# autonomousvision/volsurfs

Hardware: AMD Instinct MI355X
Metric: Mrays/s (fwd+bwd) at 800x800, K=5 shells (higher is better)
Workload: dtype f16 (hash features, MLP on MFMA, composite: as the reference), f32 accumulate and I/O

## Files before the change

include/volsurfs_hip.h:

```cpp
#ifndef VOLSURFS_HIP_H
#define VOLSURFS_HIP_H

#include <stdint.h>

#ifdef __cplusplus
extern "C" {
#endif

#define VSA_OK 0
#define VSA_ERR_ARG (-1)
#define VSA_ERR_UNSUPPORTED (-2)

#define VSA_MAX_SHELLS 16

int vsa_version(void);

int vsa_composite_dense_fwd(const float* surfs_rgb, const float* surfs_alpha,
                            const float* rgb_bg, int bg_is_broadcast, float* out_rgb,
                            float* out_rgb_fg, float* out_bg_transmittance, float* out_weights,
                            float* out_surfs_rgb_h, float* out_surfs_alpha_h, int nr_rays,
                            int nr_shells, int carry_f16, void* stream);

int vsa_composite_dense_bwd(const float* surfs_rgb, const float* surfs_alpha,
                            const float* rgb_bg, int bg_is_broadcast, const float* g_rgb,
                            float* g_surfs_rgb, float* g_surfs_alpha, float* g_rgb_bg,
                            int nr_rays, int nr_shells, int carry_f16, void* stream);

int vsa_composite_dense_bwd_l1(const float* surfs_rgb, const float* surfs_alpha,
                               const float* rgb_bg, int bg_is_broadcast, const float* pred_rgb,
                               const float* gt_rgb, float loss_scale, float* g_surfs_rgb,
                               float* g_surfs_alpha, int nr_rays, int nr_shells, int carry_f16,
                               void* stream);

int vsa_composite_dense_fwd_bwd_l1(const float* surfs_rgb, const float* surfs_alpha,
                                   const float* rgb_bg, int bg_is_broadcast, const float* gt_rgb,
                                   float loss_scale, float* out_rgb, float* g_surfs_rgb,
                                   float* g_surfs_alpha, int nr_rays, int nr_shells, int carry_f16,
                                   void* stream);

long long vsa_reduce_scratch_bytes(void);
int vsa_count_hits(const int32_t* hit_slot, long long n, void* scratch, int64_t* out, void* stream);
int vsa_l1_mean(const float* pred, const float* gt, long long n, void* scratch, float* out, void* stream);

typedef struct vsa_bvh vsa_bvh;
int vsa_bvh_build(const float* verts, const int32_t* faces, int nr_verts, int nr_faces,
                  int leaf_size, vsa_bvh** out_bvh);
int vsa_bvh_sizes(const vsa_bvh* bvh, int* nr_nodes, int* nr_tris, int* max_depth);
int vsa_bvh_export(const vsa_bvh* bvh, float* nodes_out, float* tris_out, int node_base,
                   int tri_base);
int vsa_bvh_export_q(const vsa_bvh* bvh, uint32_t* qnodes_out, float* tris_out, int node_base,
                     int tri_base, float* frame_out);
int vsa_bvh_refit(vsa_bvh* bvh, const float* verts, int nr_verts);
int vsa_bvh_destroy(vsa_bvh* bvh);

typedef struct vsa_bvh_dev vsa_bvh_dev;
int vsa_bvh_dev_build(const float* verts, const int32_t* faces, int nr_verts, int nr_faces, int leaf_size,
                      void* stream, vsa_bvh_dev** out_bvh);
int vsa_bvh_dev_sizes(const vsa_bvh_dev* bvh, int* nr_nodes, int* nr_tris, int* max_depth);
int vsa_bvh_dev_export(const vsa_bvh_dev* bvh, float* nodes_out, uint32_t* qnodes_out, float* tris_out,
                       int node_base, int tri_base, float* frame_out, void* stream);
int vsa_bvh_dev_refit(vsa_bvh_dev* bvh, const float* verts, int nr_verts, void* stream);
int vsa_bvh_dev_destroy(vsa_bvh_dev* bvh);
int vsa_bvh_dev_build_ploc(const float* verts, const int32_t* faces, int nr_verts, int nr_faces, int leaf_size,
                           int radius, void* stream, vsa_bvh_dev** out_bvh);

int vsa_trace(const float* nodes, const float* tris, const int32_t* mesh_roots, int nr_meshes,
              int max_depth, const float* rays_o, const float* rays_d, int nr_rays, float t_min,
              float* hit_t, int32_t* hit_slot, float* hit_uv, void* stream);

int vsa_trace_q(const uint32_t* qnodes, const float* tris, const int32_t* mesh_roots,
                const float* mesh_frames, int nr_meshes, int max_depth, const float* rays_o,
                const float* rays_d, int nr_rays, float t_min, float* hit_t, int32_t* hit_slot,
                float* hit_uv, void* stream);
int vsa_trace_q_narrow(const uint32_t* qnodes, const float* tris, const int32_t* mesh_roots,
                       const float* mesh_frames, int nr_meshes, int max_depth, const float* rays_o,
                       const float* rays_d, int nr_rays, float t_min, float* hit_t, int32_t* hit_slot,
                       float* hit_uv, int rays_per_wave, void* stream);
long long vsa_trace_feedback_bytes(int nr_rays, int nr_meshes);
int vsa_trace_q_fb(const uint32_t* qnodes, const float* tris, const int32_t* mesh_roots,
                   const float* mesh_frames, int nr_meshes, int max_depth, const float* rays_o,
                   const float* rays_d, int nr_rays, float t_min, float* hit_t, int32_t* hit_slot,
                   float* hit_uv, void* feedback, long long feedback_bytes, int phase, void* stream);
int vsa_trace_coop_config(int chunk, int lanes, long long max_waves);
int vsa_trace_q_stats(const uint32_t* qnodes, const float* tris, const int32_t* mesh_roots,
                      const float* mesh_frames, int nr_meshes, int max_depth, const float* rays_o,
                      const float* rays_d, int nr_rays, float t_min, uint64_t* stats, void* stream);
int vsa_hit_attributes(const float* tris, const float* rays_o, const float* rays_d,
                       const float* hit_t, const int32_t* hit_slot, const float* hit_uv,
                       int nr_rays, uint8_t* is_hit, int32_t* tri_id, float* positions,
                       float* normals, float* barycentric, void* stream);

#define VSA_NT_MAX_LEVELS 16
#define VSA_NT_MAX_DEG 4
#define VSA_NT_WEIGHTS_PER_TEX 8192
#define VSA_NT_ROW_QUADS(d) ((d) == 0 ? 2 : ((d) == 1 ? 4 : 8))
#define VSA_NT_ALPHA_QUAD(d) ((d) == 0 ? 1 : ((d) == 1 ? 3 : ((d) == 2 ? 4 : 6)))

typedef struct vsa_nt_plan {
  int32_t nr_shells;
  int32_t rgb_degrees;
  int32_t alpha_degrees;
  int32_t inner_solid;
  int32_t with_alpha_decay;
  int32_t n_levels;
  int32_t tex_res[VSA_NT_MAX_DEG];
  float sh_lo[VSA_NT_MAX_DEG];
  float sh_span[VSA_NT_MAX_DEG];
  float level_scale[VSA_NT_MAX_LEVELS];
  int32_t level_res[VSA_NT_MAX_LEVELS];
  int32_t level_size[VSA_NT_MAX_LEVELS];
  int32_t level_offset[VSA_NT_MAX_LEVELS + 1];
  int64_t dom_off[VSA_MAX_SHELLS * VSA_NT_MAX_DEG + 1];
  int64_t slot_capacity;
  int32_t max_rays;
  int32_t anchor;
  int64_t row_base[VSA_MAX_SHELLS * VSA_NT_MAX_DEG + 1];
  void* balance;
  int32_t row_format;
  int32_t grads_zeroed;
  int32_t shared_rgb;
  int32_t shared_alpha;
} vsa_nt_plan;

long long vsa_nt_balance_bytes(void);
int vsa_nt_rebalance(const vsa_nt_plan* plan, void* stream);

int vsa_nt_mark(const vsa_nt_plan* plan, const int32_t* hit_slot, const float* hit_uv,
                const float* face_uvs, int nr_rays, float* tex_uv, uint8_t* marks, void* stream);

int vsa_nt_compact_frame(const vsa_nt_plan* plan, uint8_t* marks, int32_t* slot_of,
                         int32_t* texel_of_slot, float* slot_xy, int32_t* seg_start,
                         int32_t* block_scratch, void* stream);

int vsa_nt_encode_fwd(const vsa_nt_plan* plan, const void* tables_h, const float* slot_xy,
                      const int32_t* seg_start, void* features, void* stream);

int vsa_nt_mlp_fwd(const vsa_nt_plan* plan, const void* weights_h, const void* features,
                   const int32_t* seg_start, uint8_t* texels, void* pre_out, void* stream);

int vsa_nt_encode_mlp_fwd(const vsa_nt_plan* plan, const void* tables_h, const void* weights_h,
                          const float* slot_xy, const int32_t* seg_start, void* features,
                          uint8_t* texels, void* pre_out, void* stream);

int vsa_nt_mlp_bwd(const vsa_nt_plan* plan, const void* weights_h, void* features,
                   const int32_t* seg_start, uint16_t* grad_rows, float* grad_weights,
                   float* dfeat_abs_sum, float weight_grad_scale, void* stream);

int vsa_nt_shade_fwd(const vsa_nt_plan* plan, const int32_t* hit_slot, const float* tex_uv,
                     const float* rays_d, const float* tris, const int32_t* slot_of,
                     const int32_t* seg_start, const uint8_t* texels, int nr_rays,
                     float* surfs_rgb, float* surfs_alpha,
                     float* surfs_normals, float* coeffs_out, float* act_out, void* stream);

int vsa_nt_shade_bwd(const vsa_nt_plan* plan, const int32_t* hit_slot, const float* tex_uv,
                     const float* rays_d, const float* tris, const int32_t* slot_of,
                     const int32_t* seg_start, const uint8_t* texels, int nr_rays,
                     const float* g_surfs_rgb,
                     const float* g_surfs_alpha, float grad_scale, uint16_t* grad_rows,
                     const float* act_in, void* stream);

long long vsa_nt_planes_bytes(const vsa_nt_plan* plan);
int vsa_nt_export_planes(const vsa_nt_plan* plan, const int32_t* slot_of, const int32_t* seg_start,
                         const uint8_t* texels, uint8_t* planes, long long planes_bytes, void* stream);
int vsa_nt_import_planes(const vsa_nt_plan* plan, const uint8_t* planes, long long planes_bytes,
                         const int32_t* slot_of, const int32_t* seg_start, uint8_t* texels, void* stream);

int vsa_nt_encode_bwd(const vsa_nt_plan* plan, const void* dfeatures, const float* dfeat_abs_sum,
                      float grad_scale, const float* slot_xy, const int32_t* seg_start,
                      float* grad_tables, void* stream);

int vsa_nt_encode_bwd_range(const vsa_nt_plan* plan, const void* dfeatures,
                            const float* dfeat_abs_sum, float grad_scale, const float* slot_xy,
                            const int32_t* seg_start, float* grad_tables, int shell_begin,
                            int shell_end, void* stream);

typedef struct vsa_dp_flags vsa_dp_flags;
int vsa_dp_flags_create(int n, vsa_dp_flags** out);
int vsa_dp_flags_destroy(vsa_dp_flags* flags);
int vsa_dp_flags_read(const vsa_dp_flags* flags, uint32_t* host_out);

int vsa_nt_encode_bwd_phased(const vsa_nt_plan* plan, const void* dfeatures,
                             const float* dfeat_abs_sum, float grad_scale, const float* slot_xy,
                             const int32_t* seg_start, float* grad_tables, int n_phases,
                             const int32_t* phase_shell_end, vsa_dp_flags* flags, uint32_t* counters,
                             const uint32_t* epoch, int reserve_cus, void* stream);

int vsa_dp_signal(vsa_dp_flags* flags, int index, uint32_t* epoch, int advance_epoch, void* stream);

int vsa_dp_stream_wait(vsa_dp_flags* flags, int index, uint32_t value, int mode, void* stream);

#define VSA_GRID_MAX_LEVELS 32
typedef struct vsa_grid_plan {
  int32_t n_dims;
  int32_t n_levels;
  int32_t n_features;
  int32_t reserved0;
  float level_scale[VSA_GRID_MAX_LEVELS];
  int32_t level_res[VSA_GRID_MAX_LEVELS];
  int32_t level_size[VSA_GRID_MAX_LEVELS];
  int32_t level_offset[VSA_GRID_MAX_LEVELS + 1];
} vsa_grid_plan;

int vsa_grid_encode_fwd(const vsa_grid_plan* plan, const float* tables, const float* x,
                        int nr_points, float* out, void* stream);
int vsa_grid_encode_bwd(const vsa_grid_plan* plan, const float* x, const float* g_out,
                        int nr_points, float* grad_tables, void* stream);
int vsa_grid_encode_bwd_sliced(const vsa_grid_plan* plan, const float* x, const float* g_out,
                               int nr_points, float* grad_tables, float* workspace, void* stream);
int vsa_grid_encode_bwd_binned_workspace(const vsa_grid_plan* plan, int nr_points,
                                         long long* workspace_floats);
int vsa_grid_encode_bwd_binned(const vsa_grid_plan* plan, const float* x, const float* g_out,
                               int nr_points, float* grad_tables, float* workspace, void* stream);
int vsa_grid_encode_fwd_ld(const vsa_grid_plan* plan, const float* tables, const float* x,
                           int nr_points, float* out, int out_stride, int append_x, void* stream);
int vsa_grid_encode_bwd_ld(const vsa_grid_plan* plan, const float* x, const float* g_out,
                           int g_stride, int nr_points, float* grad_tables, void* stream);
int vsa_grid_encode_bwd_sliced_ld(const vsa_grid_plan* plan, const float* x, const float* g_out,
                                  int g_stride, int nr_points, float* grad_tables, float* workspace,
                                  void* stream);
int vsa_grid_encode_bwd_binned_ld(const vsa_grid_plan* plan, const float* x, const float* g_out,
                                  int g_stride, int nr_points, float* grad_tables, float* workspace,
                                  void* stream);
int vsa_sh_encode(const float* dirs, int nr_dirs, int degree, float* out, void* stream);

int vsa_field_head_fwd(const float* y1, int y1_stride, const float* dirs_enc, long long nr_points, int nr_feat,
                       int nr_dir, float* x2, float* density, void* stream);
int vsa_field_head_bwd(const float* y1, int y1_stride, const float* dx2, const float* d_density, long long nr_points,
                       int nr_feat, int nr_dir, float* dy1, void* stream);

#define VSA_MLP_MAX_LAYERS 6
typedef struct vsa_mlp_plan {
  int32_t n_layers;
  int32_t dims[VSA_MLP_MAX_LAYERS + 1];
  const float* w[VSA_MLP_MAX_LAYERS];
  const float* b[VSA_MLP_MAX_LAYERS];
} vsa_mlp_plan;
typedef struct vsa_mlp_grads {
  float* dw[VSA_MLP_MAX_LAYERS];
  float* db[VSA_MLP_MAX_LAYERS];
  int32_t accumulate;
} vsa_mlp_grads;

int vsa_mlp_workspace(const vsa_mlp_plan* plan, long long nr_points, long long* packed_floats,
                      long long* act_floats, long long* partial_floats);
int vsa_mlp_bwd_needs_act(const vsa_mlp_plan* plan, int x_stride, int dx_stride);
int vsa_mlp_fwd(const vsa_mlp_plan* plan, const float* x, int x_stride, int nr_points, float* y,
                int y_stride, float* z_ws, float* a_ws, float* packed_ws, void* stream);
int vsa_mlp_bwd(const vsa_mlp_plan* plan, const float* x, int x_stride, int nr_points,
                const float* dy, int dy_stride, const float* z_ws, float* dz_ws, const float* a_ws,
                float* packed_ws, float* partial_ws, float* dx, int dx_stride,
                const vsa_mlp_grads* grads, void* stream);

int vsa_mlp_fwd_grouped(const vsa_mlp_plan* plans, int nr_groups, const int* nr_points,
                        const float* x, int x_stride, float* y, int y_stride, float* z_ws,
                        float* a_ws, float* packed_ws, float* packed_bwd_ws, void* stream);
int vsa_mlp_bwd_grouped(const vsa_mlp_plan* plans, int nr_groups, const int* nr_points,
                        const float* x, int x_stride, const float* dy, int dy_stride,
                        const float* z_ws, float* dz_ws, const float* a_ws, float* packed_ws,
                        int packed_ready, float* partial_ws, float* dx, int dx_stride,
                        const vsa_mlp_grads* grads, void* stream);

typedef struct vsa_adam_tensor {
  float* param;
  float* grad;
  float* exp_avg;
  float* exp_avg_sq;
  void* param_f16;
  int64_t n;
} vsa_adam_tensor;

int vsa_adam_chunk_elems(void);
int vsa_adam_step(const vsa_adam_tensor* tensors_dev, const int32_t* chunks_dev, int nr_chunks,
                  float lr, float beta1, float beta2, float eps, int step, float grad_scale,
                  int zero_grads, void* stream);
int vsa_adam_step_shared(const vsa_adam_tensor* tensors_dev, const int32_t* chunks_dev, int nr_chunks,
                         float lr, float beta1, float beta2, float eps, int step, float grad_scale,
                         int zero_grads, int max_workgroups, void* stream);

int vsa_legacy_hit_prep(const float* rays_o, const float* rays_d, const float* hit_t, const int32_t* hit_slot,
                        const float* tris, const int64_t* hit_shell, const int64_t* hit_ray, int nr_hits, int nr_rays,
                        float* pts, float* dirs, float* normals, void* stream);
int vsa_legacy_shade_out_fwd(const float* y_rgb, int ld_rgb, const float* y_alpha, int ld_alpha, int alpha_first_row,
                             const int64_t* hit_shell, const int64_t* hit_ray, const float* dirs, const float* normals,
                             int nr_hits, int nr_rays,
                             int nr_shells, int with_alpha_decay, float* surfs_rgb, float* surfs_alpha,
                             float* surfs_normals, float* sig_rgb, float* sig_alpha, float* decay, void* stream);
int vsa_legacy_shade_out_bwd(const float* g_surfs_rgb, const float* g_surfs_alpha, const int64_t* hit_shell,
                             const int64_t* hit_ray, const float* sig_rgb, const float* sig_alpha, const float* decay, int nr_hits, int nr_shells,
                             int alpha_first_row, float* dy_rgb, int ld_rgb, float* dy_alpha, int ld_alpha, void* stream);

typedef struct vsa_permuto_plan {
  int32_t pos_dim;
  int32_t n_levels;
  int32_t n_features;
  int32_t capacity;
  float scale_factor[VSA_GRID_MAX_LEVELS][4];
  float random_shift[VSA_GRID_MAX_LEVELS][4];
} vsa_permuto_plan;

int vsa_permuto_encode_fwd(const vsa_permuto_plan* plan, const float* lattice_values,
                           const float* x, const float* window, int nr_points, float* out,
                           int out_stride, void* stream);
int vsa_permuto_encode_bwd(const vsa_permuto_plan* plan, const float* x, const float* window,
                           const float* g_out, int g_stride, int nr_points, float* grad_values,
                           void* stream);

int vsa_permuto_encode_fwd_grouped(const vsa_permuto_plan* plan_host, const vsa_permuto_plan* plans_dev,
                                   const float* const* lattice_values, int nr_groups,
                                   const int* nr_points, const float* x, const float* window,
                                   float* out, int out_stride, void* stream);
int vsa_permuto_encode_bwd_grouped(const vsa_permuto_plan* plan_host, const vsa_permuto_plan* plans_dev,
                                   int nr_groups, const int* nr_points, const float* x,
                                   const float* window, const float* g_out, int g_stride,
                                   float* const* grad_values, void* stream);

int vsa_packed_cumprod_fwd(const int32_t* start_end, const float* one_minus_alpha,
                           float* transmittance, float* bg_transmittance, int nr_rays,
                           void* stream);
int vsa_packed_cumprod_bwd(const int32_t* start_end, const float* g_bg_transmittance,
                           const float* one_minus_alpha, const float* bg_transmittance,
                           const float* cumsum_lv, float* g_one_minus_alpha, int nr_rays,
                           void* stream);
int vsa_packed_cumsum(const int32_t* start_end, const float* values, int inverse, float* out,
                      int nr_rays, void* stream);
int vsa_packed_integrate_fwd(const int32_t* start_end, const float* values, const float* weights,
                             float* out, int nr_rays, int dim, void* stream);
int vsa_packed_integrate_bwd(const int32_t* start_end, const float* g_out, const float* values,
                             const float* weights, float* g_values, float* g_weights,
                             int nr_rays, int dim, int bug_compat, void* stream);
int vsa_packed_composite_fwd(const int32_t* start_end, const float* density, const float* dt,
                             const float* rgb, float* pred_rgb, float* weights, int nr_rays,
                             void* stream);
int vsa_packed_composite_bwd(const int32_t* start_end, const float* density, const float* dt,
                             const float* rgb, const float* g_pred_rgb, float* g_rgb,
                             float* g_density, float* scratch, int nr_rays, int bug_compat,
                             void* stream);
int vsa_nerf_composite_fwd(const int32_t* start_end, const float* density, const float* dt,
                           const float* samples_z, const float* rgb, const float* rgb_bg, int bg_per_ray,
                           float* rgb_fg, float* rgb_out, float* weights_sum, float* depth, float* weights,
                           int nr_rays, void* stream);
int vsa_nerf_composite_bwd(const int32_t* start_end, const float* density, const float* dt,
                           const float* rgb, const float* rgb_bg, int bg_per_ray, const float* weights_sum,
                           const float* g_rgb, const float* g_weights_sum, float* g_density,
                           float* g_rgb_samples, float* g_rgb_bg, float* scratch, int nr_rays,
                           int bug_compat, void* stream);
int vsa_nerf_coarse_cdf(const int32_t* start_end, const float* density, const float* dt, float* cdf,
                        int nr_rays, void* stream);
int vsa_neus_composite_fwd(const int32_t* start_end, const float* sdf, const float* sdf_grad,
                           const float* dirs, const float* dt, const float* samples_z,
                           const float* normals, const float* rgb, const float* rgb_bg, int bg_per_ray,
                           double cos_anneal_ratio, double logistic_beta, float* rgb_fg, float* rgb_out,
                           float* weights_sum, float* depth, float* normals_out, float* weights,
                           float* alpha, int nr_rays, void* stream);
int vsa_neus_composite_bwd(const int32_t* start_end, const float* sdf, const float* sdf_grad,
                           const float* dirs, const float* dt, const float* rgb, const float* rgb_bg,
                           int bg_per_ray, double cos_anneal_ratio, double logistic_beta,
                           const float* weights_sum, const float* g_rgb, const float* g_weights_sum,
                           float* g_sdf, float* g_sdf_grad, float* g_rgb_samples, float* g_rgb_bg,
                           float* scratch, int nr_rays, int bug_compat, void* stream);
int vsa_sdf_coarse_cdf(const int32_t* start_end, const float* sdf, const float* dt, float logistic_beta,
                       float* cdf, int nr_rays, void* stream);
int vsa_offsets_composite_fwd(const int32_t* start_end, int nr_surfs, const float* sdfs, const float* sdfs_grad,
                              const float* normals, const float* rgb, const float* transparency, const float* dirs,
                              const float* dt, const float* samples_z, const float* rgb_bg, int bg_per_ray,
                              double cos_anneal_ratio, double logistic_beta, int with_alpha_decay,
                              double alpha_decay_factor, float* surfs_rgb, float* surfs_normals, float* surfs_depths,
                              float* surfs_weight_sum, float* surfs_alpha, float* surfs_transmittance,
                              float* surfs_blending_weights, float* rgb_fg, float* bg_transmittance, float* rgb_out,
                              float* alpha, int nr_rays, void* stream);
int vsa_offsets_composite_bwd(const int32_t* start_end, int nr_surfs, const float* sdfs, const float* sdfs_grad,
                              const float* normals, const float* rgb, const float* transparency, const float* dirs,
                              const float* dt, const float* rgb_bg, int bg_per_ray, double cos_anneal_ratio,
                              double logistic_beta, int with_alpha_decay, double alpha_decay_factor,
                              const float* surfs_rgb, const float* surfs_alpha, const float* surfs_transmittance,
                              const float* bg_transmittance, const float* g_rgb, float* g_sdfs, float* g_sdfs_grad,
                              float* g_rgb_samples, float* g_transparency, float* g_rgb_bg, float* scratch,
                              int nr_rays, int bug_compat, void* stream);
int vsa_sdfs_coarse_cdf(const int32_t* start_end, int nr_surfs, const float* sdfs, const float* dt,
                        float logistic_beta, float* cdf, int nr_rays, void* stream);
int vsa_packed_median_depth(const int32_t* start_end, const float* samples_z,
                            const float* weights, float threshold, float* out, int nr_rays,
                            int fallback_compat, void* stream);
int vsa_packed_update_dt(const int32_t* start_end, const float* ray_max_dt, const float* ray_exit,
                         const float* samples_z, int is_background, float* samples_dt,
                         int nr_rays, void* stream);
int vsa_sample_bg(const float* rays_o, const float* rays_d, const float* ray_t_start,
                  float ray_t_far, int nr_samples_per_ray, int jitter, uint64_t rng_state,
                  uint64_t rng_inc, float* ray_max_dt, float* samples_3d, float* samples_dirs,
                  float* samples_z, int32_t* ray_start_end_idx, int nr_rays, void* stream);
int vsa_contract_samples(const float* ray_o, const int32_t* start_end, const float* samples_3d,
                         const float* samples_z, float* out_samples_3d, float* out_samples_z,
                         int nr_rays, void* stream);

int vsa_packed_sum_over_rays(const int32_t* start_end, const float* values, float* sum_per_ray,
                             float* sum_per_sample, int nr_rays, int dim, void* stream);
int vsa_packed_sum_over_rays_bwd(const int32_t* start_end, const float* g_sum_per_ray,
                                 const float* g_sum_per_sample, float* g_values, int nr_rays,
                                 int dim, void* stream);
int vsa_packed_sdf2alpha(const int32_t* start_end, const float* samples_dt, const float* samples_sdf,
                         const float* logistic_beta, float* alpha, int nr_rays, void* stream);
int vsa_packed_compute_cdf(const int32_t* start_end, const float* weights, float* cdf, int nr_rays,
                           void* stream);

int vsa_sample_fg(const float* rays_o, const float* rays_d, const float* ray_t_entry,
                  const float* ray_t_exit, float min_dist_between_samples,
                  int min_nr_samples_per_ray, int max_nr_samples_per_ray, int jitter,
                  uint64_t rng_state, uint64_t rng_inc, float* ray_max_dt, int32_t* samples_idx,
                  float* samples_3d, float* samples_dirs, float* samples_z,
                  int32_t* ray_start_end_idx, int nr_rays, void* stream);
int vsa_pack_compact(const int32_t* start_end, const int32_t* out_start, const int32_t* samples_idx,
                     const float* samples_3d, const float* samples_dirs, const float* samples_z,
                     const float* samples_dt, const float* samples_values, int values_dim,
                     int32_t* out_idx, float* out_3d, float* out_dirs, float* out_z, float* out_dt,
                     float* out_values, int32_t* out_start_end, int nr_rays, void* stream);
int vsa_importance_sample(const float* rays_o, const float* rays_d, const int32_t* start_end,
                          const float* samples_z, const float* samples_cdf,
                          int nr_importance_samples, int jitter, uint64_t rng_state,
                          uint64_t rng_inc, float* out_3d, float* out_dirs, float* out_z,
                          int32_t* out_start_end, int nr_rays, void* stream);

int vsa_uncontract_samples(const float* ray_o, const int32_t* start_end, const float* samples_3d,
                           const float* samples_z, float* out_samples_3d, float* out_samples_z,
                           int nr_rays, void* stream);

int vsa_combine_packs(const int32_t* start_end_1, const int32_t* idx_1, const float* s3d_1,
                      const float* dirs_1, const float* z_1, const float* values_1,
                      const int32_t* start_end_2, const int32_t* idx_2, const float* s3d_2,
                      const float* dirs_2, const float* z_2, const float* values_2,
                      const int32_t* out_start, float min_dist_between_samples, int values_dim,
                      int32_t* out_idx, float* out_3d, float* out_dirs, float* out_z,
                      float* out_values, int32_t* out_start_end, int nr_rays, void* stream);

int vsa_intersect_primitive(const float* rays_o, const float* rays_d, int nr_rays, int kind,
                            float size, uint8_t* is_hit, float* t_near, float* t_far,
                            float* points_near, float* points_far, void* stream);

int vsa_camera_rays(const float* c2w, const float* intrinsics_inv, int height, int width,
                    int nr_rays_per_pixel, int jitter_pixels, uint64_t rng_state, uint64_t rng_inc,
                    float* rays_o, float* rays_d, float* points_2d, void* stream);

int vsa_reel_next_rays_batch(const float* c2w_all, const float* intrinsics_inv_all,
                             const float* rgb_all, const float* mask_all, int nr_cameras, int height,
                             int width, int batch_size, int nr_rays_per_pixel, int jitter_pixels,
                             uint64_t rng_state, uint64_t rng_inc, int32_t* camera_idx,
                             float* rays_o, float* rays_d, float* gt_rgb, float* gt_mask,
                             float* points_2d, void* stream);

typedef struct vsa_train_ctl {
  int32_t iter;
  int32_t nr_rays;
  int32_t capacity;
  int32_t adam_step;
  float loss_scale;
  float adam_lr;
  float loss;
  int32_t clamped;
  uint64_t rng_state, rng_inc;
  int64_t nr_hits;
  int32_t target_hits;
  int32_t nr_warmup;
  int32_t nr_milestones;
  int32_t milestone[8];
  float lr_stage[9];
  int32_t adam_pending;
  double lr_base;
  double loss_weight;
  int64_t sum_rays, sum_hits;
} vsa_train_ctl;

int vsa_train_ctl_tick(vsa_train_ctl* ctl, void* stream);

int vsa_reel_next_rays_batch_ctl(const float* c2w_all, const float* intrinsics_inv_all, const float* rgb_all,
                                 const float* mask_all, int nr_cameras, int height, int width, int capacity,
                                 int nr_rays_per_pixel, int jitter_pixels, const vsa_train_ctl* ctl,
                                 const float* dummy_o, const float* dummy_d, const float* dummy_rgb,
                                 int32_t* camera_idx, float* rays_o, float* rays_d, float* gt_rgb,
                                 float* gt_mask, float* points_2d, void* stream);

int vsa_composite_dense_fwd_bwd_l1_ctl(const float* surfs_rgb, const float* surfs_alpha, const float* rgb_bg,
                                       int bg_is_broadcast, const float* gt_rgb, const vsa_train_ctl* ctl,
                                       float* out_rgb, float* g_surfs_rgb, float* g_surfs_alpha, int capacity,
                                       int nr_shells, int carry_f16, void* stream);

int vsa_l1_mean_ctl(const float* pred, const float* gt, int capacity, void* scratch, vsa_train_ctl* ctl, void* stream);

int vsa_adam_step_ctl(const vsa_adam_tensor* tensors_dev, const int32_t* chunks_dev, int nr_chunks, float beta1,
                      float beta2, float eps, float grad_scale, int zero_grads, int max_workgroups,
                      const vsa_train_ctl* ctl, void* stream);

int vsa_tile_order(const float* src, float* dst, int height, int width, int channels, int inverse,
                   void* stream);
int vsa_tile_order_rays(const float* rays_o, const float* rays_d, const float* gt_rgb,
                        float* rays_o_tiled, float* rays_d_tiled, float* gt_rgb_tiled, int height,
                        int width, void* stream);


int vsa_occ_grid_points(const int32_t* point_indices, int nr_points, int nr_voxels_per_dim,
                        float extent_x, float extent_y, float extent_z, int centre_of_voxel, int jitter,
                        uint64_t rng_state, uint64_t rng_inc, float* out_points, void* stream);
int vsa_occ_update_values(const int32_t* point_indices, const float* values, int nr_points, float decay,
                          float* grid_values, void* stream);
int vsa_occ_update_occupancy_density(const int32_t* point_indices, int nr_points, int nr_voxels_per_dim,
                                     float extent_x, float extent_y, float extent_z,
                                     float occupancy_thresh, int check_neighbours,
                                     const float* grid_values, uint8_t* grid_occupancy, void* stream);
int vsa_occ_update_occupancy_sdf(const int32_t* point_indices, const float* logistic_beta, int nr_points,
                                 int nr_voxels_per_dim, float extent_x, float extent_y, float extent_z,
                                 float occupancy_thresh, const float* grid_values,
                                 uint8_t* grid_occupancy, void* stream);
int vsa_occ_check(const float* points, int nr_points, int nr_voxels_per_dim, float extent_x,
                  float extent_y, float extent_z, const float* grid_values,
                  const uint8_t* grid_occupancy, const uint8_t* grid_roi, uint8_t* out_occupancy,
                  float* out_values, void* stream);
int vsa_occ_rays_t_near_t_far(const float* rays_o, const float* rays_d, const float* ray_t_entry,
                              const float* ray_t_exit, int nr_rays, int nr_voxels_per_dim,
                              float extent_x, float extent_y, float extent_z,
                              const uint8_t* grid_occupancy, const uint8_t* grid_roi, float* out_t_near,
                              float* out_t_far, void* stream);
int vsa_occ_first_sample(const float* rays_o, const float* rays_d, const float* ray_t_entry,
                         const float* ray_t_exit, int nr_rays, int nr_voxels_per_dim, float extent_x,
                         float extent_y, float extent_z, const uint8_t* grid_occupancy,
                         const uint8_t* grid_roi, float* samples_3d, float* samples_dirs,
                         float* samples_z, float* samples_dt, int32_t* ray_start_end_idx, void* stream);
int vsa_occ_advance_samples(const float* samples_dirs, const float* samples_3d, int nr_points,
                            int nr_voxels_per_dim, float extent_x, float extent_y, float extent_z,
                            const uint8_t* grid_occupancy, const uint8_t* grid_roi,
                            float* new_samples_3d, uint8_t* is_within_bounds, void* stream);
int vsa_sample_fg_occupied(const float* rays_o, const float* rays_d, const float* ray_t_entry,
                           const float* ray_t_exit, float min_dist_between_samples,
                           int min_nr_samples_per_ray, int max_nr_samples_per_ray, int jitter_samples,
                           uint64_t rng_state, uint64_t rng_inc, int nr_voxels_per_dim, float extent_x,
                           float extent_y, float extent_z, const uint8_t* grid_occupancy,
                           const uint8_t* grid_roi, float* ray_max_dt, int32_t* samples_idx,
                           float* samples_3d, float* samples_dirs, float* samples_z,
                           int32_t* ray_start_end_idx, int nr_rays, void* stream);

long long vsa_image_metrics_workspace_bytes(int B, int H, int W, int pool, int pred_u8, int gt_u8);
int vsa_image_metrics(const void* pred, int pred_u8, const void* gt, int gt_u8, int B, int H, int W, int pool,
                      int quantize_pred, void* workspace, long long workspace_bytes, double* psnr_out,
                      double* ssim_out, void* stream);

long long vsa_isosurface_workspace_bytes(long long nx, long long ny, long long nz, int nr_levels);
int vsa_isosurface_count(const float* grid, long long nx, long long ny, long long nz, const float* levels,
                         int nr_levels, int inside_above, void* workspace, long long workspace_bytes,
                         long long* totals, void* stream);
int vsa_isosurface_emit(const float* grid, long long nx, long long ny, long long nz, const float* levels,
                        int nr_levels, int inside_above, const float* origin, const float* spacing, void* workspace,
                        long long workspace_bytes, const long long* totals, float* const* verts,
                        int32_t* const* faces, void* stream);
int vsa_mc_table(int8_t* out);

long long vsa_simplify_workspace_bytes(long long nr_verts, long long nr_faces);
int vsa_simplify(const float* verts, long long nr_verts, const int32_t* faces, long long nr_faces,
                 long long target_faces, void* workspace, long long workspace_bytes, float* out_verts,
                 int32_t* out_faces, long long* stats, float* stage_ms, void* stream);

#define VSA_ERR_ATLAS_FULL (-3)
long long vsa_atlas_workspace_bytes(long long nr_verts, long long nr_faces, int resolution);
int vsa_atlas(const float* verts, long long nr_verts, const int32_t* faces, long long nr_faces, int resolution,
              int padding, void* workspace, long long workspace_bytes, float* out_faces_uvs, int32_t* out_chart,
              long long* stats, float* scale, float* stage_ms, void* stream);
long long vsa_atlas_rasterize_workspace_bytes(long long nr_faces);
int vsa_atlas_rasterize(const float* faces_uvs, long long nr_faces, int resolution, void* workspace,
                        long long workspace_bytes, int32_t* out_face_id, int32_t* out_count, void* stream);

int vsa_st_begin(const float* points_near, int nr_rays, int nr_slots, float* pts, uint8_t* flags, int32_t* live,
                 float* dense, int32_t* count, void* stream);
int vsa_st_step(const int32_t* live_in, const int32_t* count_in, const float* sdf, int nr_columns,
                const int32_t* slot_cols, int nr_rays, const float* rays_d, float sdf_multiplier, float thresh,
                int kind, float size, float* pts, uint8_t* flags, uint8_t* keep, int32_t* block_counts,
                const float* dense_in, int32_t* live_out, float* dense_out, int32_t* count_out, int bound,
                void* stream);
int vsa_st_finish(const float* pts, const float* rays_o, int nr_rays, int nr_slots, const uint8_t* flags,
                  int unconverged_are_hits, float* z, uint8_t* hit, uint8_t* keep, int32_t* block_counts,
                  int32_t* hit_list, int32_t* hit_count, void* stream);
int vsa_st_scatter(const int32_t* ids, long long nr_ids, const float* src, int nr_channels, int nr_rays,
                   int nr_slots, float* dst, void* stream);
int vsa_st_blend(const float* surfs_rgb, const float* surfs_alpha, int nr_rays, int nr_surfs,
                 float* surfs_transmittance, float* surfs_blending_weights, float* rgb_fg, float* bg_transmittance,
                 void* stream);

long long vsa_tb_workspace_bytes(long long nr_faces, int resolution);
long long vsa_tb_max_chunks(int resolution, int nr_samples, long long chunk_rows);
int vsa_tb_samples(const float* faces_uvs, long long nr_faces, int resolution, int nr_samples,
                   unsigned long long seed, long long chunk_rows, void* workspace, long long workspace_bytes,
                   int32_t* owner, int32_t* ctl, int ctl_len, void* stream);
int vsa_tb_emit(const float* verts, const int32_t* faces, const float* faces_uvs, long long nr_faces, int resolution,
                int nr_samples, unsigned long long seed, const void* workspace, long long workspace_bytes,
                const int32_t* owner, int32_t* row_start, float* points, float* normals, void* stream);
int vsa_tb_resolve(const float* vals, int nr_channels, const int32_t* row_start, int texel_begin, int texel_end,
                   int resolution, float* texture, void* stream);
int vsa_tb_dilate(float* img, int height, int width, int nr_channels, int nr_iterations, int32_t* stamp,
                  int32_t* filled, void* stream);

int vsa_tsdf_fuse_lattice(const float* proj, const float* depth, int nr_views, int height, int width,
                          const float* axis, int n, float sdf_trunc, int uncontract, float* out_tsdf, void* stream);
int vsa_tsdf_fuse_points(const float* proj, const float* depth, const float* rgb_maps, int nr_views, int height,
                         int width, const float* points, long long nr_points, float sdf_trunc, int uncontract,
                         float* out_tsdf, float* out_rgb, void* stream);
int vsa_tsdf_uncontract_points(const float* points, long long nr_points, float max_range, float* out, void* stream);

long long vsa_mesh_clusters_workspace_bytes(long long nr_verts, long long nr_faces);
int vsa_mesh_clusters(const float* verts, long long nr_verts, const int32_t* faces, long long nr_faces,
                      void* workspace, long long workspace_bytes, int32_t* out_triangle_clusters,
                      int32_t* out_cluster_n_triangles, double* out_cluster_area, long long* out_nr_clusters,
                      float* stage_ms, void* stream);
int vsa_mesh_filter(const float* verts, long long nr_verts, const int32_t* faces, long long nr_faces, int mode,
                    const uint8_t* keep_mask, long long cluster_to_keep, long long min_cluster_faces,
                    int drop_unreferenced, int drop_degenerate, void* workspace, long long workspace_bytes,
                    float* out_verts, int32_t* out_faces, int32_t* out_vertex_map, int32_t* out_face_map,
                    long long* stats, float* stage_ms, void* stream);
int vsa_mesh_compact_rows(const void* rows, long long nr_rows, int row_words, const int32_t* map, void* out,
                          void* stream);

int vsa_face_view_counts(const uint32_t* qnodes, const float* tris, const int32_t* mesh_roots,
                         const float* mesh_frames, int nr_meshes, int max_depth,
                         const float* c2w_all, const float* intrinsics_inv_all,
                         int nr_views, int height, int width, int supersample, float t_min,
                         const long long* face_base, uint32_t* counts,
                         void* stream);
int vsa_face_view_counts_tile(int tile);
int vsa_face_ring_dilate(const int32_t* faces, long long nr_faces, long long nr_verts, uint8_t* keep,
                         int rings, uint8_t* vert_scratch, void* stream);

#ifdef __cplusplus
}
#endif
#endif
```

volsurfs_amd/composite.py:

```python
import torch

from . import _lib


class _CompositeDense(torch.autograd.Function):
    @staticmethod
    def forward(ctx, surfs_rgb, surfs_alpha, rgb_bg, carry_f16):
        N, K, _ = surfs_rgb.shape
        surfs_rgb = _lib.check_f32(surfs_rgb.contiguous(), N, K, 3)
        surfs_alpha = _lib.check_f32(surfs_alpha.contiguous().view(N, K), N, K)
        rgb_bg = rgb_bg.contiguous()
        bcast = rgb_bg.shape[0] == 1 and N != 1
        _lib.check_f32(rgb_bg, 1 if bcast else N, 3)
        dev = surfs_rgb.device
        out_rgb = torch.empty(N, 3, device=dev)
        out_fg = torch.empty(N, 3, device=dev)
        out_bgT = torch.empty(N, 1, device=dev)
        out_w = torch.empty(N, K, 1, device=dev)
        out_rgb_h = torch.empty(N, K, 3, device=dev)
        out_alpha_h = torch.empty(N, K, 1, device=dev)
        _lib.call("vsa_composite_dense_fwd", surfs_rgb, surfs_alpha, rgb_bg, bcast, out_rgb,
                  out_fg, out_bgT, out_w, out_rgb_h, out_alpha_h, N, K, int(carry_f16),
                  _lib.stream_ptr())
        ctx.save_for_backward(surfs_rgb, surfs_alpha, rgb_bg)
        ctx.bcast = bcast
        ctx.carry_f16 = int(carry_f16)
        ctx.mark_non_differentiable(out_fg, out_bgT, out_w, out_rgb_h, out_alpha_h)
        return out_rgb, out_fg, out_bgT, out_w, out_rgb_h, out_alpha_h

    @staticmethod
    def backward(ctx, g_rgb, *unused):
        surfs_rgb, surfs_alpha, rgb_bg = ctx.saved_tensors
        N, K, _ = surfs_rgb.shape
        g_rgb = _lib.check_f32(g_rgb.contiguous(), N, 3)
        g_c = torch.empty_like(surfs_rgb)
        g_a = torch.empty_like(surfs_alpha)
        need_bg = ctx.needs_input_grad[2]
        g_bg = torch.empty(N, 3, device=g_rgb.device) if need_bg else None
        _lib.call("vsa_composite_dense_bwd", surfs_rgb, surfs_alpha, rgb_bg, ctx.bcast, g_rgb,
                  g_c, g_a, g_bg, N, K, ctx.carry_f16, _lib.stream_ptr())
        if need_bg and ctx.bcast:
            g_bg = g_bg.sum(0, keepdim=True)
        return g_c, g_a, g_bg, None


def composite_dense(surfs_rgb, surfs_alpha, rgb_bg, carry_f16=False):
    N, K = surfs_rgb.shape[:2]
    alpha2d = surfs_alpha.reshape(N, K)
    rgb, fg, bgT, w, rgb_h, alpha_h = _CompositeDense.apply(surfs_rgb, alpha2d, rgb_bg, carry_f16)
    return {
        "rgb": rgb,
        "rgb_fg": fg,
        "rgb_bg": rgb_bg.expand(N, 3).half().float(),
        "surfs_alpha": alpha_h,
        "surfs_rgb": rgb_h,
        "surfs_blending_weights": w,
        "bg_transmittance": bgT,
    }


class _CompositeL1(torch.autograd.Function):

    @staticmethod
    def forward(ctx, surfs_rgb, surfs_alpha, rgb_bg, gt_rgb):
        N, K = surfs_rgb.shape[:2]
        rgb, g_c, g_a = composite_fwd_bwd_l1_raw(surfs_rgb.contiguous(), surfs_alpha.reshape(N, K).contiguous(),
                                                 rgb_bg.contiguous(), gt_rgb.contiguous(), 1.0 / (3.0 * N))
        ctx.save_for_backward(g_c, g_a)
        ctx.alpha_shape = surfs_alpha.shape
        loss = l1_mean(rgb, gt_rgb)
        ctx.mark_non_differentiable(rgb)
        return loss, rgb

    @staticmethod
    def backward(ctx, g_loss, _g_rgb):
        g_c, g_a = ctx.saved_tensors
        return g_c * g_loss, (g_a * g_loss).reshape(ctx.alpha_shape), None, None


def composite_l1(surfs_rgb, surfs_alpha, rgb_bg, gt_rgb):
    return _CompositeL1.apply(surfs_rgb, surfs_alpha, rgb_bg, gt_rgb)


def composite_fwd_raw(surfs_rgb, surfs_alpha, rgb_bg, carry_f16=False):
    N, K, _ = surfs_rgb.shape
    out = torch.empty(N, 3, device=surfs_rgb.device)
    bcast = rgb_bg.shape[0] == 1 and N != 1
    _lib.call("vsa_composite_dense_fwd", surfs_rgb, surfs_alpha, rgb_bg, bcast, out, None, None,
              None, None, None, N, K, int(carry_f16), _lib.stream_ptr())
    return out


def composite_bwd_raw(surfs_rgb, surfs_alpha, rgb_bg, g_rgb, carry_f16=False):
    N, K, _ = surfs_rgb.shape
    g_c = torch.empty_like(surfs_rgb)
    g_a = torch.empty_like(surfs_alpha)
    bcast = rgb_bg.shape[0] == 1 and N != 1
    _lib.call("vsa_composite_dense_bwd", surfs_rgb, surfs_alpha, rgb_bg, bcast, g_rgb, g_c, g_a,
              None, N, K, int(carry_f16), _lib.stream_ptr())
    return g_c, g_a


def composite_bwd_l1_raw(surfs_rgb, surfs_alpha, rgb_bg, pred_rgb, gt_rgb, loss_scale, carry_f16=False):
    N, K, _ = surfs_rgb.shape
    g_c = torch.empty_like(surfs_rgb)
    g_a = torch.empty_like(surfs_alpha)
    bcast = rgb_bg.shape[0] == 1 and N != 1
    _lib.call("vsa_composite_dense_bwd_l1", surfs_rgb, surfs_alpha, rgb_bg, bcast, pred_rgb, gt_rgb,
              float(loss_scale), g_c, g_a, N, K, int(carry_f16), _lib.stream_ptr())
    return g_c, g_a


def composite_fwd_bwd_l1_raw(surfs_rgb, surfs_alpha, rgb_bg, gt_rgb, loss_scale, carry_f16=False):
    N, K, _ = surfs_rgb.shape
    rgb = torch.empty(N, 3, device=surfs_rgb.device)
    g_c = torch.empty_like(surfs_rgb)
    g_a = torch.empty_like(surfs_alpha)
    bcast = rgb_bg.shape[0] == 1 and N != 1
    _lib.call("vsa_composite_dense_fwd_bwd_l1", surfs_rgb, surfs_alpha, rgb_bg, bcast, gt_rgb,
              float(loss_scale), rgb, g_c, g_a, N, K, int(carry_f16), _lib.stream_ptr())
    return rgb, g_c, g_a


_reduce_scratch = {}


def reduce_scratch(device):
    import ctypes
    dev = torch.device(device)
    dev = torch.device("cuda", torch.cuda.current_device()) if dev.index is None else dev
    key = (dev, torch.cuda.current_stream(dev).cuda_stream)
    sc = _reduce_scratch.get(key)
    if sc is None:
        fn = _lib.lib().vsa_reduce_scratch_bytes
        fn.restype = ctypes.c_longlong
        sc = _reduce_scratch[key] = torch.zeros(int(fn()), dtype=torch.uint8, device=dev)
    return sc


def l1_mean(pred, gt):
    import ctypes
    pred, gt = _lib.check_f32(pred.contiguous()), _lib.check_f32(gt.contiguous(), *pred.shape)
    pred, gt = (x if x.data_ptr() % 16 == 0 else x.clone() for x in (pred, gt))
    out = torch.empty((), device=pred.device)
    _lib.call("vsa_l1_mean", pred, gt, ctypes.c_longlong(pred.numel()), reduce_scratch(pred.device), out,
              _lib.stream_ptr())
    return out


def count_hits(hit_slot):
    import ctypes
    if hit_slot.dtype != torch.int32 or not hit_slot.is_contiguous() or not hit_slot.is_cuda:
        raise _lib.VolsurfsHipError("count_hits: contiguous CUDA int32 tensor expected")
    out = torch.empty((), dtype=torch.int64, device=hit_slot.device)
    _lib.call("vsa_count_hits", hit_slot, ctypes.c_longlong(hit_slot.numel()), reduce_scratch(hit_slot.device), out,
              _lib.stream_ptr())
    return out
```

volsurfs_amd/csrc/composite_dense.hip:

```cpp
#include "common.h"

namespace {

#ifndef VSA_COMP_TILE
#define VSA_COMP_TILE 256
#endif
constexpr int TILE = VSA_COMP_TILE;

template <int K>
struct Lds {
  static constexpr int SC = (3 * K) | 1;
  static constexpr int SA = K | 1;
};

template <int W, int S>
__device__ __forceinline__ void slab_load(const float* __restrict__ g, float* __restrict__ s,
                                          int rows_valid) {
  const int total = rows_valid * W;
  const int nvec = total >> 2;
  const float4* g4 = reinterpret_cast<const float4*>(g);
  if constexpr (W == S) {
    if (rows_valid == TILE && (TILE * W) % 4 == 0) {
      typedef __attribute__((address_space(3))) void* lds_vp;
      typedef __attribute__((address_space(1))) const void* glb_vp;
      const int wave = __builtin_amdgcn_readfirstlane(threadIdx.x >> 6), lane = threadIdx.x & 63;
      constexpr int NV = TILE * W / 4, NC = (NV + 63) / 64;
      for (int c = wave; c < NC; c += TILE / 64)
        if (c * 64 + lane < NV)
          __builtin_amdgcn_global_load_lds((glb_vp)(g4 + c * 64 + lane), (lds_vp)(s + c * 256), 16, 0, 0);
      return;
    }
    float4* s4 = reinterpret_cast<float4*>(s);
    for (int v = threadIdx.x; v < nvec; v += TILE) s4[v] = g4[v];
  } else {
    for (int v = threadIdx.x; v < nvec; v += TILE) {
      float4 x = g4[v];
      int e = v << 2;
      float xs[4] = {x.x, x.y, x.z, x.w};
#pragma unroll
      for (int i = 0; i < 4; ++i) {
        int r = (e + i) / W;
        int j = (e + i) - r * W;
        s[r * S + j] = xs[i];
      }
    }
  }
  for (int e = (nvec << 2) + threadIdx.x; e < total; e += TILE) {
    int r = e / W;
    s[r * S + (e - r * W)] = g[e];
  }
}
__device__ __forceinline__ void slab_load_fence() {
  asm volatile("s_waitcnt vmcnt(0)" ::: "memory");
}

template <int W, int S>
__device__ __forceinline__ void slab_store(float* __restrict__ g, const float* __restrict__ s,
                                           int rows_valid) {
  const int total = rows_valid * W;
  const int nvec = total >> 2;
  float4* g4 = reinterpret_cast<float4*>(g);
  if constexpr (W == S) {
    const float4* s4 = reinterpret_cast<const float4*>(s);
    for (int v = threadIdx.x; v < nvec; v += TILE) g4[v] = s4[v];
  } else {
    for (int v = threadIdx.x; v < nvec; v += TILE) {
      int e = v << 2;
      float xs[4];
#pragma unroll
      for (int i = 0; i < 4; ++i) {
        int r = (e + i) / W;
        int j = (e + i) - r * W;
        xs[i] = s[r * S + j];
      }
      g4[v] = make_float4(xs[0], xs[1], xs[2], xs[3]);
    }
  }
  for (int e = (nvec << 2) + threadIdx.x; e < total; e += TILE) {
    int r = e / W;
    g[e] = s[r * S + (e - r * W)];
  }
}

template <int K, bool CARRY_F16>
struct RayFwd {
  float a[K], c[K][3], T[K], w[K], om[K];
  float bgT, fg[3];
  __device__ __forceinline__ void run(const float* sc, const float* sa) {
#pragma unroll
    for (int k = 0; k < K; ++k) {
      a[k] = vsa_round_f16(sa[k]);
#pragma unroll
      for (int ch = 0; ch < 3; ++ch) c[k][ch] = vsa_round_f16(sc[3 * k + ch]);
      om[k] = vsa_round_f16(1.0f - a[k]);
    }
    float acc = 1.0f, Tp = 1.0f;
    fg[0] = fg[1] = fg[2] = 0.f;
#pragma unroll
    for (int k = K - 1; k >= 0; --k) {
      T[k] = Tp;
      if (CARRY_F16) {
        Tp = vsa_round_f16(Tp * om[k]);
      } else {
        acc = vsa_pin_f32(acc * om[k]);
        Tp = vsa_round_f16(acc);
      }
      w[k] = vsa_round_f16(T[k] * a[k]);
#pragma unroll
      for (int ch = 0; ch < 3; ++ch) fg[ch] += vsa_round_f16(c[k][ch] * w[k]);
    }
    bgT = Tp;
#pragma unroll
    for (int ch = 0; ch < 3; ++ch) fg[ch] = vsa_round_f16(vsa_pin_f32(fg[ch]));
  }
};

template <int K, bool CARRY_F16>
__global__ __launch_bounds__(TILE) void composite_dense_fwd_kernel(
    const float* __restrict__ surfs_rgb, const float* __restrict__ surfs_alpha,
    const float* __restrict__ rgb_bg, int bg_bcast, float* __restrict__ out_rgb,
    float* __restrict__ out_rgb_fg, float* __restrict__ out_bgT, float* __restrict__ out_w,
    float* __restrict__ out_rgb_h, float* __restrict__ out_alpha_h, int N) {
  using L = Lds<K>;
  __shared__ __attribute__((aligned(16))) float s_c[TILE * L::SC];
  __shared__ __attribute__((aligned(16))) float s_a[TILE * L::SA];
  __shared__ __attribute__((aligned(16))) float s_o[TILE * 3];
  const long long ray0 = (long long)blockIdx.x * TILE;
  const int rows = min(TILE, (int)(N - ray0));
  slab_load<3 * K, L::SC>(surfs_rgb + ray0 * 3 * K, s_c, rows);
  slab_load<K, L::SA>(surfs_alpha + ray0 * K, s_a, rows);
  if (!bg_bcast) slab_load<3, 3>(rgb_bg + ray0 * 3, s_o, rows);
  slab_load_fence();
  __syncthreads();
  const int r = threadIdx.x;
  if (r < rows) {
    RayFwd<K, CARRY_F16> f;
    f.run(s_c + r * L::SC, s_a + r * L::SA);
    float bg[3];
#pragma unroll
    for (int ch = 0; ch < 3; ++ch)
      bg[ch] = vsa_round_f16(bg_bcast ? rgb_bg[ch] : s_o[r * 3 + ch]);
#pragma unroll
    for (int ch = 0; ch < 3; ++ch)
      s_o[r * 3 + ch] = vsa_round_f16(f.fg[ch] + vsa_round_f16(f.bgT * bg[ch]));
    const long long n = ray0 + r;
    if (out_rgb_fg) {
#pragma unroll
      for (int ch = 0; ch < 3; ++ch) out_rgb_fg[n * 3 + ch] = f.fg[ch];
    }
    if (out_bgT) out_bgT[n] = f.bgT;
    if (out_w) {
#pragma unroll
      for (int k = 0; k < K; ++k) out_w[n * K + k] = f.w[k];
    }
    if (out_alpha_h) {
#pragma unroll
      for (int k = 0; k < K; ++k) out_alpha_h[n * K + k] = f.a[k];
    }
    if (out_rgb_h) {
#pragma unroll
      for (int k = 0; k < K; ++k)
#pragma unroll
        for (int ch = 0; ch < 3; ++ch) out_rgb_h[(n * K + k) * 3 + ch] = f.c[k][ch];
    }
  }
  __syncthreads();
  slab_store<3, 3>(out_rgb + ray0 * 3, s_o, rows);
}

template <int K, bool CARRY_F16>
__global__ __launch_bounds__(TILE) void composite_dense_bwd_kernel(
    const float* __restrict__ surfs_rgb, const float* __restrict__ surfs_alpha,
    const float* __restrict__ rgb_bg, int bg_bcast, const float* __restrict__ g_rgb,
    float* __restrict__ g_surfs_rgb, float* __restrict__ g_surfs_alpha,
    float* __restrict__ g_rgb_bg, int N, const float* __restrict__ l1_gt, float l1_scale,
    float* __restrict__ pred_out, const vsa_train_ctl* __restrict__ ctl) {
  using L = Lds<K>;
  int n_active = N;
  if (ctl) {
    l1_scale = ctl->loss_scale;
    n_active = ctl->nr_rays;
  }
  __shared__ __attribute__((aligned(16))) float s_c[TILE * L::SC];
  __shared__ __attribute__((aligned(16))) float s_a[TILE * L::SA];
  __shared__ __attribute__((aligned(16))) float s_g[TILE * 3];
  __shared__ __attribute__((aligned(16))) float s_b[TILE * 3];
  __shared__ __attribute__((aligned(16))) float s_t[TILE * 3];
  const long long ray0 = (long long)blockIdx.x * TILE;
  const int rows = min(TILE, (int)(N - ray0));
  slab_load<3 * K, L::SC>(surfs_rgb + ray0 * 3 * K, s_c, rows);
  slab_load<K, L::SA>(surfs_alpha + ray0 * K, s_a, rows);
  if (!pred_out) slab_load<3, 3>(g_rgb + ray0 * 3, s_g, rows);
  if (!bg_bcast) slab_load<3, 3>(rgb_bg + ray0 * 3, s_b, rows);
  if (l1_gt) slab_load<3, 3>(l1_gt + ray0 * 3, s_t, rows);
  slab_load_fence();
  __syncthreads();
  const int r = threadIdx.x;
  if (r < rows) {
    RayFwd<K, CARRY_F16> f;
    float* sc = s_c + r * L::SC;
    float* sa = s_a + r * L::SA;
    f.run(sc, sa);
    float g[3], bg[3];
#pragma unroll
    for (int ch = 0; ch < 3; ++ch) {
      bg[ch] = vsa_round_f16(bg_bcast ? rgb_bg[ch] : s_b[r * 3 + ch]);
      if (pred_out) {
        g[ch] = vsa_round_f16(f.fg[ch] + vsa_round_f16(f.bgT * bg[ch]));
        s_g[r * 3 + ch] = g[ch];
      } else {
        g[ch] = s_g[r * 3 + ch];
      }
      if (l1_gt) {
        const float d = g[ch] - s_t[r * 3 + ch];
        g[ch] = ray0 + r >= n_active ? 0.f : (d > 0.f ? l1_scale : (d < 0.f ? -l1_scale : 0.f));
      }
    }
    float S = g[0] * bg[0] + g[1] * bg[1] + g[2] * bg[2];
#pragma unroll
    for (int k = 0; k < K; ++k) {
      float rk = g[0] * f.c[k][0] + g[1] * f.c[k][1] + g[2] * f.c[k][2];
      sa[k] = f.T[k] * (rk - S);
      S = f.a[k] * rk + f.om[k] * S;
#pragma unroll
      for (int ch = 0; ch < 3; ++ch) sc[3 * k + ch] = g[ch] * f.w[k];
    }
    if (g_rgb_bg) {
#pragma unroll
      for (int ch = 0; ch < 3; ++ch) s_b[r * 3 + ch] = g[ch] * f.bgT;
    }
  }
  __syncthreads();
  slab_store<3 * K, L::SC>(g_surfs_rgb + ray0 * 3 * K, s_c, rows);
  slab_store<K, L::SA>(g_surfs_alpha + ray0 * K, s_a, rows);
  if (g_rgb_bg) slab_store<3, 3>(g_rgb_bg + ray0 * 3, s_b, rows);
  if (pred_out) slab_store<3, 3>(pred_out + ray0 * 3, s_g, rows);
}

}

#define VSA_K_DISPATCH(K_, BODY)              \
  switch (K_) {                               \
    case 1: { constexpr int KK = 1; BODY; } break;   \
    case 2: { constexpr int KK = 2; BODY; } break;   \
    case 3: { constexpr int KK = 3; BODY; } break;   \
    case 4: { constexpr int KK = 4; BODY; } break;   \
    case 5: { constexpr int KK = 5; BODY; } break;   \
    case 6: { constexpr int KK = 6; BODY; } break;   \
    case 7: { constexpr int KK = 7; BODY; } break;   \
    case 8: { constexpr int KK = 8; BODY; } break;   \
    case 9: { constexpr int KK = 9; BODY; } break;   \
    default: return VSA_ERR_UNSUPPORTED;      \
  }

extern "C" int vsa_composite_dense_fwd(const float* surfs_rgb, const float* surfs_alpha,
                                       const float* rgb_bg, int bg_is_broadcast, float* out_rgb,
                                       float* out_rgb_fg, float* out_bg_transmittance,
                                       float* out_weights, float* out_surfs_rgb_h,
                                       float* out_surfs_alpha_h, int nr_rays, int nr_shells,
                                       int carry_f16, void* stream) {
  if (nr_rays < 0 || !out_rgb) return VSA_ERR_ARG;
  if (nr_rays == 0) return VSA_OK;
  if (!surfs_rgb || !surfs_alpha || !rgb_bg) return VSA_ERR_ARG;
  dim3 grid(vsa_div_up(nr_rays, TILE)), block(TILE);
  hipStream_t st = (hipStream_t)stream;
  VSA_K_DISPATCH(nr_shells, {
    if (carry_f16)
      hipLaunchKernelGGL((composite_dense_fwd_kernel<KK, true>), grid, block, 0, st, surfs_rgb,
                         surfs_alpha, rgb_bg, bg_is_broadcast, out_rgb, out_rgb_fg,
                         out_bg_transmittance, out_weights, out_surfs_rgb_h, out_surfs_alpha_h,
                         nr_rays);
    else
      hipLaunchKernelGGL((composite_dense_fwd_kernel<KK, false>), grid, block, 0, st, surfs_rgb,
                         surfs_alpha, rgb_bg, bg_is_broadcast, out_rgb, out_rgb_fg,
                         out_bg_transmittance, out_weights, out_surfs_rgb_h, out_surfs_alpha_h,
                         nr_rays);
  });
  VSA_RETURN_LAUNCH_STATUS();
}

static int composite_bwd_launch(const float* surfs_rgb, const float* surfs_alpha,
                                const float* rgb_bg, int bg_is_broadcast, const float* g_rgb,
                                float* g_surfs_rgb, float* g_surfs_alpha, float* g_rgb_bg,
                                int nr_rays, int nr_shells, int carry_f16, const float* l1_gt,
                                float l1_scale, void* stream, float* pred_out = nullptr,
                                const vsa_train_ctl* ctl = nullptr) {
  if (nr_rays < 0) return VSA_ERR_ARG;
  if (nr_rays == 0) return VSA_OK;
  if (!surfs_rgb || !surfs_alpha || !rgb_bg || (!g_rgb && !pred_out) || !g_surfs_rgb || !g_surfs_alpha)
    return VSA_ERR_ARG;
  dim3 grid(vsa_div_up(nr_rays, TILE)), block(TILE);
  hipStream_t st = (hipStream_t)stream;
  VSA_K_DISPATCH(nr_shells, {
    if (carry_f16)
      hipLaunchKernelGGL((composite_dense_bwd_kernel<KK, true>), grid, block, 0, st, surfs_rgb,
                         surfs_alpha, rgb_bg, bg_is_broadcast, g_rgb, g_surfs_rgb, g_surfs_alpha,
                         g_rgb_bg, nr_rays, l1_gt, l1_scale, pred_out, ctl);
    else
      hipLaunchKernelGGL((composite_dense_bwd_kernel<KK, false>), grid, block, 0, st, surfs_rgb,
                         surfs_alpha, rgb_bg, bg_is_broadcast, g_rgb, g_surfs_rgb, g_surfs_alpha,
                         g_rgb_bg, nr_rays, l1_gt, l1_scale, pred_out, ctl);
  });
  VSA_RETURN_LAUNCH_STATUS();
}

extern "C" int vsa_composite_dense_bwd(const float* surfs_rgb, const float* surfs_alpha,
                                       const float* rgb_bg, int bg_is_broadcast,
                                       const float* g_rgb, float* g_surfs_rgb,
                                       float* g_surfs_alpha, float* g_rgb_bg, int nr_rays,
                                       int nr_shells, int carry_f16, void* stream) {
  return composite_bwd_launch(surfs_rgb, surfs_alpha, rgb_bg, bg_is_broadcast, g_rgb, g_surfs_rgb,
                              g_surfs_alpha, g_rgb_bg, nr_rays, nr_shells, carry_f16, nullptr, 0.f,
                              stream);
}

extern "C" int vsa_composite_dense_bwd_l1(const float* surfs_rgb, const float* surfs_alpha,
                                          const float* rgb_bg, int bg_is_broadcast,
                                          const float* pred_rgb, const float* gt_rgb,
                                          float loss_scale, float* g_surfs_rgb,
                                          float* g_surfs_alpha, int nr_rays, int nr_shells,
                                          int carry_f16, void* stream) {
  if (!gt_rgb) return VSA_ERR_ARG;
  return composite_bwd_launch(surfs_rgb, surfs_alpha, rgb_bg, bg_is_broadcast, pred_rgb,
                              g_surfs_rgb, g_surfs_alpha, nullptr, nr_rays, nr_shells, carry_f16,
                              gt_rgb, loss_scale, stream);
}

extern "C" int vsa_composite_dense_fwd_bwd_l1(const float* surfs_rgb, const float* surfs_alpha,
                                              const float* rgb_bg, int bg_is_broadcast,
                                              const float* gt_rgb, float loss_scale, float* out_rgb,
                                              float* g_surfs_rgb, float* g_surfs_alpha, int nr_rays,
                                              int nr_shells, int carry_f16, void* stream) {
  if (!gt_rgb || (nr_rays > 0 && !out_rgb)) return VSA_ERR_ARG;
  return composite_bwd_launch(surfs_rgb, surfs_alpha, rgb_bg, bg_is_broadcast, nullptr, g_surfs_rgb,
                              g_surfs_alpha, nullptr, nr_rays, nr_shells, carry_f16, gt_rgb,
                              loss_scale, stream, out_rgb);
}

extern "C" int vsa_composite_dense_fwd_bwd_l1_ctl(const float* surfs_rgb, const float* surfs_alpha,
                                                  const float* rgb_bg, int bg_is_broadcast, const float* gt_rgb,
                                                  const vsa_train_ctl* ctl, float* out_rgb, float* g_surfs_rgb,
                                                  float* g_surfs_alpha, int capacity, int nr_shells, int carry_f16,
                                                  void* stream) {
  if (!gt_rgb || !ctl || capacity < 1 || !out_rgb) return VSA_ERR_ARG;
  return composite_bwd_launch(surfs_rgb, surfs_alpha, rgb_bg, bg_is_broadcast, nullptr, g_surfs_rgb, g_surfs_alpha,
                              nullptr, capacity, nr_shells, carry_f16, gt_rgb, 0.f, stream, out_rgb, ctl);
}
```

volsurfs_amd/csrc/nt_common.h:

```cpp
#pragma once
#include "common.h"

typedef _Float16 half2_t __attribute__((ext_vector_type(2)));
typedef _Float16 half4_t __attribute__((ext_vector_type(4)));
typedef _Float16 half8_t __attribute__((ext_vector_type(8)));
typedef float float16_t __attribute__((ext_vector_type(16)));

#define NT_DOM_BLOCK 4096

#define NT_FBLOCK 256
__device__ __forceinline__ long long nt_feat_index(const vsa_nt_plan& p, int type, int level,
                                                   int slot) {
  const long long blocks = p.slot_capacity / NT_FBLOCK;
  return (((long long)type * blocks + (slot >> 8)) * p.n_levels + level) * NT_FBLOCK + (slot & 255);
}
__device__ __forceinline__ long long nt_feat_plane_base(const vsa_nt_plan& p, int type, int level) {
  return ((long long)type * (p.slot_capacity / NT_FBLOCK) * p.n_levels + level) * NT_FBLOCK;
}
__device__ __forceinline__ long long nt_feat_in_plane(int n_levels, int slot) {
  return (long long)(slot >> 8) * (n_levels * NT_FBLOCK) + (slot & 255);
}

__host__ __device__ inline int nt_tex_index(int shell, int type, int deg) {
  return (shell * 2 + type) * VSA_NT_MAX_DEG + deg;
}

__host__ __device__ inline int nt_row_quads(int d) { return VSA_NT_ROW_QUADS(d); }
__host__ __device__ inline int nt_alpha_quad(int d) { return VSA_NT_ALPHA_QUAD(d); }

struct NtFootprint {
  int i0, j0;
  float fx, fy;
};

__device__ __forceinline__ NtFootprint nt_footprint(float u, float v, int R, bool anchor = false) {
  const float Rf = (float)R;
  const float a = u * Rf, b = v * Rf;
  if (anchor) {
    NtFootprint f;
    f.fx = f.fy = 0.f;
    f.i0 = (R - 1) - min(max((int)floorf(b), 0), R - 1);
    f.j0 = min(max((int)floorf(a), 0), R - 1);
    return f;
  }
  const float ap = Rf - b;
  const float bp = a;
  const float fl_x = floorf(ap - 0.5f), fl_y = floorf(bp - 0.5f);
  NtFootprint f;
  f.fx = ap - (fl_x + 0.5f);
  f.fy = bp - (fl_y + 0.5f);
  f.i0 = min(max((int)fl_x, -1), R - 1);
  f.j0 = min(max((int)fl_y, -1), R - 1);
  return f;
}

__device__ __forceinline__ float2 nt_interp_uv(const float* __restrict__ fuv, float bu, float bv) {
  const float b0 = (1.0f - bu) - bv;
  float2 r;
  r.x = (b0 * fuv[0] + bu * fuv[2]) + bv * fuv[4];
  r.y = (b0 * fuv[1] + bu * fuv[3]) + bv * fuv[5];
  return r;
}

__host__ __device__ inline bool nt_shell_has_alpha(const vsa_nt_plan& p, int shell) {
  return !(p.inner_solid && (shell == 0 || p.shared_alpha));
}

__device__ __forceinline__ int nt_param_tex(const vsa_nt_plan& p, int tex) {
  const bool shared = ((tex / VSA_NT_MAX_DEG) & 1) ? p.shared_alpha != 0 : p.shared_rgb != 0;
  return shared ? tex % (2 * VSA_NT_MAX_DEG) : tex;
}

__device__ __forceinline__ bool tex_active(const vsa_nt_plan& p, int tex) {
  const int deg = tex % VSA_NT_MAX_DEG;
  const int type = (tex / VSA_NT_MAX_DEG) & 1;
  const int shell = tex / (2 * VSA_NT_MAX_DEG);
  if (type == 0) return deg < p.rgb_degrees;
  if (!nt_shell_has_alpha(p, shell)) return false;
  return deg < p.alpha_degrees;
}

struct Work {
  int tex, first, last;
  int seg_len;
};

struct NtUnitWeight16 {
  __device__ int operator()(int, int, int) const { return 16; }
};

constexpr int NT_BAL_KERNELS = 6, NT_BAL_MAX_WG = 1024, NT_BAL_ONE = 1 << 24;
enum { NT_BAL_ENC_FWD_D, NT_BAL_ENC_FWD_H, NT_BAL_ENC_BWD_D, NT_BAL_ENC_BWD_H, NT_BAL_MLP_FWD, NT_BAL_MLP_BWD };
struct NtBalance {
  unsigned frac[NT_BAL_KERNELS][NT_BAL_MAX_WG + 1];
  unsigned ticks[NT_BAL_KERNELS][NT_BAL_MAX_WG];
  int frac_wgs[NT_BAL_KERNELS];
  int tick_wgs[NT_BAL_KERNELS];
  float ema[NT_BAL_KERNELS][NT_BAL_MAX_WG];
};

__device__ __forceinline__ void nt_split_range(const vsa_nt_plan& plan, int bal_id, long long total,
                                               long long& lo, long long& hi) {
  const NtBalance* b = static_cast<const NtBalance*>(plan.balance);
  if (b && bal_id >= 0 && b->frac_wgs[bal_id] == (int)gridDim.x) {
    lo = (total * b->frac[bal_id][blockIdx.x]) >> 24;
    hi = (total * b->frac[bal_id][blockIdx.x + 1]) >> 24;
  } else {
    lo = total * blockIdx.x / gridDim.x;
    hi = total * (blockIdx.x + 1) / gridDim.x;
  }
}

__device__ __forceinline__ unsigned long long nt_bal_now() {
  unsigned long long t;
  asm volatile("s_memrealtime %0\n\ts_waitcnt lgkmcnt(0)" : "=s"(t)::"memory");
  return t;
}
#define NT_BAL_BEGIN() const unsigned long long bal_t0__ = plan.balance ? nt_bal_now() : 0ull
#define NT_BAL_END(id)                                                                   \
  if (plan.balance && threadIdx.x == 0 && gridDim.x <= NT_BAL_MAX_WG) {                  \
    NtBalance* b__ = static_cast<NtBalance*>(plan.balance);                              \
    b__->ticks[id][blockIdx.x] = (unsigned)(nt_bal_now() - bal_t0__);                    \
    if (blockIdx.x == 0) b__->tick_wgs[id] = (int)gridDim.x;                             \
  }

template <int UNIT, typename Body, typename Weight = NtUnitWeight16>
__device__ __forceinline__ void nt_for_each_piece_scalar(const vsa_nt_plan& plan,
                                                  const int* __restrict__ seg_start, int n_planes,
                                                  int ovh, Body&& body, int tex_begin = 0,
                                                  int tex_end = 1 << 30, Weight wt = Weight(), int bal_id = -1) {
  const int n_all = plan.nr_shells * 2 * VSA_NT_MAX_DEG;
  const int n_tex = tex_end < n_all ? tex_end : n_all;
  long long units_td[2 * VSA_NT_MAX_DEG] = {0, 0, 0, 0, 0, 0, 0, 0};
  long long pieces = 0;
  for (int tex = tex_begin; tex < n_tex; ++tex) {
    if (!tex_active(plan, tex)) continue;
    const int deg = tex % VSA_NT_MAX_DEG;
    const int sd = (tex / (2 * VSA_NT_MAX_DEG)) * VSA_NT_MAX_DEG + deg;
    const int len = seg_start[sd + 1] - seg_start[sd];
    if (len > 0) {
      const int cls = ((tex / VSA_NT_MAX_DEG) & 1) * VSA_NT_MAX_DEG + deg;
      const long long n_units = (len + UNIT - 1) / UNIT;
#pragma unroll
      for (int c = 0; c < 2 * VSA_NT_MAX_DEG; ++c) units_td[c] += c == cls ? n_units : 0;
      pieces += 1;
    }
  }
  if (pieces == 0) return;
  auto plane_cost = [&](int pl) {
    long long c = pieces * ovh * 16;
#pragma unroll
    for (int d = 0; d < VSA_NT_MAX_DEG; ++d) c += units_td[d] * wt(pl, d, 0) + units_td[VSA_NT_MAX_DEG + d] * wt(pl, d, 1);
    return c;
  };
  long long total = 0;
  for (int pl = 0; pl < n_planes; ++pl) total += plane_cost(pl);
  long long lo, hi;
  nt_split_range(plan, bal_id, total, lo, hi);
  if (hi <= lo) return;
  long long c0 = 0;
  for (int pl = 0; pl < n_planes && c0 < hi; ++pl) {
    const long long pc = plane_cost(pl);
    if (c0 + pc <= lo) {
      c0 += pc;
      continue;
    }
    for (int tex = tex_begin; tex < n_tex; ++tex) {
      if (!tex_active(plan, tex)) continue;
      const int deg = tex % VSA_NT_MAX_DEG;
      const int sd = (tex / (2 * VSA_NT_MAX_DEG)) * VSA_NT_MAX_DEG + deg;
      const int begin = seg_start[sd], end = seg_start[sd + 1];
      if (end <= begin) continue;
      const int units = (end - begin + UNIT - 1) / UNIT, w = wt(pl, deg, (tex / VSA_NT_MAX_DEG) & 1);
      const long long t0 = c0 + (long long)ovh * 16;
      c0 = t0 + (long long)units * w;
      if (t0 >= hi) break;
      const long long a = lo > t0 ? lo - t0 : 0, b = hi - t0 < (long long)units * w ? hi - t0 : (long long)units * w;
      if (b <= a) continue;
      const int ua = (int)((a + w - 1) / w), ub = (int)((b + w - 1) / w);
      if (ub <= ua) continue;
      const int first = begin + ua * UNIT;
      const long long lastl = (long long)begin + (long long)ub * UNIT;
      body(pl, tex, first, lastl < end ? (int)lastl : end, begin, end);
    }
  }
}

__device__ __forceinline__ int nt_wave_incl_scan(int v) {
  v += __builtin_amdgcn_update_dpp(0, v, 0x111, 0xf, 0xf, false);
  v += __builtin_amdgcn_update_dpp(0, v, 0x112, 0xf, 0xf, false);
  v += __builtin_amdgcn_update_dpp(0, v, 0x114, 0xf, 0xf, false);
  v += __builtin_amdgcn_update_dpp(0, v, 0x118, 0xf, 0xf, false);
  v += __builtin_amdgcn_update_dpp(0, v, 0x142, 0xa, 0xf, false);
  v += __builtin_amdgcn_update_dpp(0, v, 0x143, 0xc, 0xf, false);
  return v;
}

__device__ __forceinline__ int nt_pair_partner(const vsa_nt_plan& p, int tex) {
  const int other = tex ^ VSA_NT_MAX_DEG;
  return ((tex / VSA_NT_MAX_DEG) & 1) == 0 && tex_active(p, other) ? other : -1;
}

template <int UNIT, typename Body, typename Weight = NtUnitWeight16>
__device__ __forceinline__ void nt_for_each_piece(const vsa_nt_plan& plan,
                                                  const int* __restrict__ seg_start, int n_planes,
                                                  int ovh, Body&& body, int tex_begin = 0,
                                                  int tex_end = 1 << 30, Weight wt = Weight(), int bal_id = -1,
                                                  bool paired = false) {
  const int n_all = plan.nr_shells * 2 * VSA_NT_MAX_DEG;
  if (n_all > 64) {
    nt_for_each_piece_scalar<UNIT>(plan, seg_start, n_planes, ovh, body, tex_begin, tex_end, wt, bal_id);
    return;
  }
  const int n_tex = tex_end < n_all ? tex_end : n_all;
  const int lane = threadIdx.x & 63;
  const int tex = lane;
  const int deg = tex % VSA_NT_MAX_DEG, type = (tex / VSA_NT_MAX_DEG) & 1, shell = tex / (2 * VSA_NT_MAX_DEG);
  const int rgb_deg = plan.rgb_degrees, alpha_deg = plan.alpha_degrees;
  const bool shell_alpha = nt_shell_has_alpha(plan, shell);
  bool act = tex >= tex_begin && tex < n_tex &&
             (type == 0 ? deg < rgb_deg : (shell_alpha && deg < alpha_deg));
  int wtype = type;
  if (paired) {
    const bool rgb_act = deg < rgb_deg, alpha_act = shell_alpha && deg < alpha_deg;
    if (type == 1 && rgb_act) act = false;
    if (type == 0 && act && alpha_act) wtype = 2;
  }
  const int sd = shell * VSA_NT_MAX_DEG + deg;
  int begin = 0, end = 0;
  if (act) {
    begin = seg_start[sd];
    end = seg_start[sd + 1];
  }
  act = act && end > begin;
  const int units = act ? (end - begin + UNIT - 1) / UNIT : 0;
  const unsigned long long act_mask = __ballot(act);
  const long long pieces = __popcll(act_mask);
  if (pieces == 0) return;
  auto lane_cost = [&](int pl) { return act ? ovh * 16 + units * wt(pl, deg, wtype) : 0; };
  auto plane_cost = [&](int pl) -> long long {
    return (long long)(unsigned)__builtin_amdgcn_readlane(nt_wave_incl_scan(lane_cost(pl)), 63);
  };
  long long total = 0;
  for (int pl = 0; pl < n_planes; ++pl) total += plane_cost(pl);
  long long lo, hi;
  nt_split_range(plan, bal_id, total, lo, hi);
  if (hi <= lo) return;
  long long c0 = 0;
  for (int pl = 0; pl < n_planes && c0 < hi; ++pl) {
    const int cl = lane_cost(pl);
    const int incl = nt_wave_incl_scan(cl);
    const long long pc = (long long)(unsigned)__builtin_amdgcn_readlane(incl, 63);
    if (c0 + pc <= lo) {
      c0 += pc;
      continue;
    }
    const long long t0l = c0 + (long long)(incl - cl) + (long long)ovh * 16;
    const int w = wt(pl, deg, wtype);
    const long long span = (long long)units * w;
    bool hit = act && t0l < hi;
    int ua = 0, ub = 0;
    if (hit) {
      const long long a = lo > t0l ? lo - t0l : 0, b = hi - t0l < span ? hi - t0l : span;
      hit = b > a;
      if (hit) {
        ua = (int)(((unsigned)a + (unsigned)w - 1u) / (unsigned)w);
        ub = (int)(((unsigned)b + (unsigned)w - 1u) / (unsigned)w);
        hit = ub > ua;
      }
    }
    unsigned long long todo = __ballot(hit);
    while (todo) {
      const int j = __ffsll((long long)todo) - 1;
      todo &= todo - 1;
      const int jb = __builtin_amdgcn_readlane(begin, j), je = __builtin_amdgcn_readlane(end, j);
      const int ja = __builtin_amdgcn_readlane(ua, j), jub = __builtin_amdgcn_readlane(ub, j);
      const int first = jb + ja * UNIT;
      const long long lastl = (long long)jb + (long long)jub * UNIT;
      body(pl, j, first, lastl < je ? (int)lastl : je, jb, je);
    }
    c0 += pc;
  }
}

#ifdef NT_SPAN
static __device__ unsigned long long g_span[4][2048][3];
#define NT_SPAN_MARK(id, which)                                                          \
  if (threadIdx.x == 0 && blockIdx.x < 2048) {                                           \
    unsigned long long t__;                                                              \
    asm volatile("s_memrealtime %0\n\ts_waitcnt lgkmcnt(0)" : "=s"(t__)::"memory");     \
    g_span[id][blockIdx.x][which] = t__;                                                 \
    if (which == 0) {                                                                    \
      unsigned hw__, xcc__;                                                              \
      asm volatile("s_getreg_b32 %0, hwreg(HW_REG_HW_ID)" : "=s"(hw__));                 \
      asm volatile("s_getreg_b32 %0, hwreg(HW_REG_XCC_ID)" : "=s"(xcc__));               \
      g_span[id][blockIdx.x][2] = ((unsigned long long)xcc__ << 32) | hw__;             \
    }                                                                                    \
  }
#else
#define NT_SPAN_MARK(id, which)
#endif
```

volsurfs_amd/csrc/nt_encode.hip:

```cpp
#include <type_traits>

#include "nt_common.h"
#include "nt_enc_common.h"

namespace {

#ifndef NT_ENC_OVH_FH
#define NT_ENC_OVH_FH 87
#endif
#ifndef NT_ENC_OVH_FD
#define NT_ENC_OVH_FD 27
#endif
#ifndef NT_ENC_OVH_BH
#define NT_ENC_OVH_BH 145
#endif
#ifndef NT_ENC_OVH_BD
#define NT_ENC_OVH_BD 64
#endif
#ifndef NT_ENC_PAIR_W
#define NT_ENC_PAIR_W 22
#endif
constexpr int ENC_BLOCK = 1024;
constexpr int ENC_UNROLL = 8;
#ifndef ENC_UNROLL_FWD_N
#define ENC_UNROLL_FWD_N 4
#endif
constexpr int ENC_UNROLL_FWD = ENC_UNROLL_FWD_N;
constexpr int ENC_UNIT = 256;
constexpr int LDS_ENTRIES = 32768;


#ifndef NT_ENC_DIAG_FWD
#define NT_ENC_DIAG_FWD 0
#endif
constexpr int ENC_PAIR_OFF = 15360;
template <bool HASHED>
__device__ __forceinline__ void nt_encode_fwd_body(
    const vsa_nt_plan& plan, int level0, int n_levels, const half2_t* __restrict__ tables,
    const float2* __restrict__ slot_xy, const int* __restrict__ seg_start,
    half2_t* __restrict__ features, unsigned char* s_raw) {
  half2_t* s_tab = reinterpret_cast<half2_t*>(s_raw);
  const long long n_entries = plan.level_offset[plan.n_levels];
  const int nl = plan.n_levels;
  NT_SPAN_MARK(HASHED ? 1 : 0, 0);
  NT_BAL_BEGIN();
  const bool pair_mode = !HASHED && plan.nr_shells * 2 * VSA_NT_MAX_DEG <= 64;
  auto unit_weight = [&](int pl, int deg, int wtype) {
    const int w = !HASHED || plan.level_scale[level0 + pl] < (float)plan.tex_res[deg] ? 16 : 15;
    return wtype == 2 ? (w * NT_ENC_PAIR_W) >> 4 : w;
  };
  nt_for_each_piece<ENC_UNIT>(plan, seg_start, n_levels, HASHED ? NT_ENC_OVH_FH : NT_ENC_OVH_FD,
                              [&](int pl, int tex, int first, int last, int, int) {
    const int level = level0 + pl;
    const LevelGeom g = level_geom(plan, level);
    const int partner = pair_mode ? nt_pair_partner(plan, tex) : -1;
    const bool pair_fits = (int)g.size <= ENC_PAIR_OFF && ENC_PAIR_OFF + (int)g.size <= LDS_ENTRIES;
    const int tex2 = pair_fits ? partner : -1;
    for (int pass = 0; pass < (partner >= 0 && !pair_fits ? 2 : 1); ++pass) {
    const int tex_p = pass ? partner : tex;
    __syncthreads();
    auto stage = [&](int t, half2_t* dst_h) {
      typedef unsigned u32x4 __attribute__((ext_vector_type(4)));
      const u32x4* src = reinterpret_cast<const u32x4*>(tables + (long long)nt_param_tex(plan, t) * n_entries + plan.level_offset[level]);
      u32x4* dst = reinterpret_cast<u32x4*>(dst_h);
      constexpr int SB = 8;
      const int nvec = (int)(g.size / 4);
      for (int i0 = threadIdx.x; i0 < nvec; i0 += ENC_BLOCK * SB) {
        u32x4 r[SB];
#pragma unroll
        for (int k = 0; k < SB; ++k) {
          const int i = i0 + k * ENC_BLOCK;
          r[k] = src[i < nvec ? i : nvec - 1];
        }
#pragma unroll
        for (int k = 0; k < SB; ++k)
          if (i0 + k * ENC_BLOCK < nvec) dst[i0 + k * ENC_BLOCK] = r[k];
      }
    };
    stage(tex_p, s_tab);
    if (tex2 >= 0) stage(tex2, s_tab + ENC_PAIR_OFF);
    __syncthreads();
    const int type = (tex_p / VSA_NT_MAX_DEG) & 1;
    half2_t* out = features + nt_feat_plane_base(plan, type, level);
    half2_t* out2 = features + nt_feat_plane_base(plan, 1, level);
    const int a_first = first & ~(ENC_UNROLL_FWD - 1);
    auto run = [&](auto reuse_tag, auto pair_tag) {
      constexpr bool REUSE = decltype(reuse_tag)::value;
      constexpr bool PAIR = decltype(pair_tag)::value;
      for (int s0 = a_first + threadIdx.x * ENC_UNROLL_FWD; s0 < last; s0 += ENC_BLOCK * ENC_UNROLL_FWD) {
        float4 xyv[ENC_UNROLL_FWD / 2];
#if NT_ENC_DIAG_FWD & 1
        const float4* xp = reinterpret_cast<const float4*>(slot_xy + (s0 & 0x1fff));
#else
        const float4* xp = reinterpret_cast<const float4*>(slot_xy + s0);
#endif
#pragma unroll
        for (int i = 0; i < ENC_UNROLL_FWD / 2; ++i) xyv[i] = xp[i];
        CellRefS cr[ENC_UNROLL_FWD];
        bool fresh[ENC_UNROLL_FWD];
#pragma unroll
        for (int u = 0; u < ENC_UNROLL_FWD; ++u) {
          const float x = (u & 1) ? xyv[u >> 1].z : xyv[u >> 1].x;
          const float y = (u & 1) ? xyv[u >> 1].w : xyv[u >> 1].y;
          cr[u] = cell_ref_s(g, x, y);
          fresh[u] = !REUSE || u == 0 || cr[u].cx != cr[u - 1].cx || cr[u].cy != cr[u - 1].cy;
        }
        half2_t v[ENC_UNROLL_FWD][4], v2[PAIR ? ENC_UNROLL_FWD : 1][4];
#pragma unroll
        for (int u = 0; u < ENC_UNROLL_FWD; ++u) {
          if (fresh[u]) {
            unsigned idx[4];
            cell_indices<HASHED>(g, cr[u].cx, cr[u].cy, idx);
#pragma unroll
            for (int k = 0; k < 4; ++k) v[u][k] = s_tab[idx[k]];
            if constexpr (PAIR) {
#pragma unroll
              for (int k = 0; k < 4; ++k) v2[u][k] = s_tab[idx[k] + ENC_PAIR_OFF];
            }
          }
        }
        unsigned outw[ENC_UNROLL_FWD], outw2[PAIR ? ENC_UNROLL_FWD : 1];
#pragma unroll
        for (int u = 0; u < ENC_UNROLL_FWD; ++u) {
          if (REUSE && u > 0 && !fresh[u]) {
#pragma unroll
            for (int k = 0; k < 4; ++k) v[u][k] = v[u - 1][k];
            if constexpr (PAIR) {
#pragma unroll
              for (int k = 0; k < 4; ++k) v2[u][k] = v2[u - 1][k];
            }
          }
          unsigned ew[4];
#pragma unroll
          for (int k = 0; k < 4; ++k) ew[k] = __builtin_bit_cast(unsigned, v[u][k]);
          if constexpr (PAIR) {
            half2_t wh[4];
            enc_weights_h(cr[u].w, wh);
            outw[u] = enc_blend_h(ew, wh);
#pragma unroll
            for (int k = 0; k < 4; ++k) ew[k] = __builtin_bit_cast(unsigned, v2[u][k]);
            outw2[u] = enc_blend_h(ew, wh);
          } else
          {
            outw[u] = enc_blend(ew, cr[u].w);
          }
        }
#if NT_ENC_DIAG_FWD & 2
#pragma unroll
        for (int u = 0; u < ENC_UNROLL_FWD; ++u) asm volatile("" ::"v"(outw[u]));
        continue;
#endif
#if NT_ENC_DIAG_FWD & 4
        const long long o_in = nt_feat_in_plane(nl, s0 & 0x3fff);
#else
        const long long o_in = nt_feat_in_plane(nl, s0);
#endif
        unsigned* op = reinterpret_cast<unsigned*>(out) + o_in;
        unsigned* op2 = reinterpret_cast<unsigned*>(out2) + o_in;
        if (s0 >= first && s0 + ENC_UNROLL_FWD <= last) {
          uint4* o4 = reinterpret_cast<uint4*>(op);
#pragma unroll
          for (int i = 0; i < ENC_UNROLL_FWD / 4; ++i)
            o4[i] = make_uint4(outw[4 * i], outw[4 * i + 1], outw[4 * i + 2], outw[4 * i + 3]);
          if constexpr (PAIR) {
            uint4* p4 = reinterpret_cast<uint4*>(op2);
#pragma unroll
            for (int i = 0; i < ENC_UNROLL_FWD / 4; ++i)
              p4[i] = make_uint4(outw2[4 * i], outw2[4 * i + 1], outw2[4 * i + 2], outw2[4 * i + 3]);
          }
        } else {
#pragma unroll
          for (int u = 0; u < ENC_UNROLL_FWD; ++u)
            if (s0 + u >= first && s0 + u < last) {
              op[u] = outw[u];
              if constexpr (PAIR) op2[u] = outw2[u];
            }
        }
      }
    };
    const bool reuse = g.scale < (float)plan.tex_res[tex % VSA_NT_MAX_DEG];
    if (!HASHED && tex2 >= 0) {
      if (reuse) run(std::true_type{}, std::true_type{});
      else run(std::false_type{}, std::true_type{});
    } else {
      if (reuse) run(std::true_type{}, std::false_type{});
      else run(std::false_type{}, std::false_type{});
    }
    }
  }, 0, 1 << 30, unit_weight, HASHED ? NT_BAL_ENC_FWD_H : NT_BAL_ENC_FWD_D, pair_mode);
  __syncthreads();
  NT_SPAN_MARK(HASHED ? 1 : 0, 1);
  NT_BAL_END(HASHED ? NT_BAL_ENC_FWD_H : NT_BAL_ENC_FWD_D);
}

template <bool HASHED>
__global__ __launch_bounds__(ENC_BLOCK) void nt_encode_fwd_kernel(
    vsa_nt_plan plan, int level0, int n_levels, const half2_t* __restrict__ tables,
    const float2* __restrict__ slot_xy, const int* __restrict__ seg_start,
    half2_t* __restrict__ features) {
  extern __shared__ __attribute__((aligned(16))) unsigned char s_raw[];
  nt_encode_fwd_body<HASHED>(plan, level0, n_levels, tables, slot_xy, seg_start, features, s_raw);
}

__global__ __launch_bounds__(ENC_BLOCK) void nt_encode_fwd_both_kernel(
    vsa_nt_plan plan, int lh, const half2_t* __restrict__ tables,
    const float2* __restrict__ slot_xy, const int* __restrict__ seg_start,
    half2_t* __restrict__ features) {
  extern __shared__ __attribute__((aligned(16))) unsigned char s_raw[];
  nt_encode_fwd_body<false>(plan, 0, lh, tables, slot_xy, seg_start, features, s_raw);
  __syncthreads();
  nt_encode_fwd_body<true>(plan, lh, plan.n_levels - lh, tables, slot_xy, seg_start, features, s_raw);
}

#ifndef NT_ENC_DIAG
#define NT_ENC_DIAG 0
#endif
#ifndef NT_ENC_FLUSH_BATCH
#define NT_ENC_FLUSH_BATCH 8
#endif
#if NT_ENC_DIAG & 64
#define ENC_LDS_ADD(ptr, val) asm volatile("" ::"v"(ptr), "v"(val))
#else
#define ENC_LDS_ADD(ptr, val) atomicAdd(ptr, val)
#endif
template <bool HASHED, int NF, bool MERGE>
__device__ __forceinline__ void enc_bwd_piece(
    const vsa_nt_plan& plan, int* s_g, int level, int feat, int tex, int first, int last,
    bool store, const half2_t* __restrict__ dfeatures, const float* __restrict__ dfeat_abs_sum,
    float dscale_inv, const float2* __restrict__ slot_xy, float* __restrict__ grad_tables) {
  const int nl = plan.n_levels;
  const long long n_entries = plan.level_offset[plan.n_levels];
  const LevelGeom g = level_geom(plan, level);
  float S[NF], S_inv[NF];
  bool any = false;
#pragma unroll
  for (int f = 0; f < NF; ++f) {
    const float total = dfeat_abs_sum[tex * 32 + 2 * level + feat + f] * 1.001f;
    S[f] = 0.f, S_inv[f] = 0.f;
    if (total > 0.f) {
      int e;
      frexpf(total, &e);
      S[f] = ldexpf(1.0f, 30 - e);
      S_inv[f] = ldexpf(1.0f, e - 30) * dscale_inv;
      any = true;
    }
  }
  if (!any) return;
#if NT_ENC_DIAG & 8
  return;
#endif
  int copies = 1;
  if (!HASHED) {
    while (copies < 32 && (long long)g.size * copies * 2 * NF <= LDS_ENTRIES) copies *= 2;
  }
  const int plane = (int)g.size * copies;
  __syncthreads();
#if !(NT_ENC_DIAG & 2)
  for (int i = threadIdx.x; i < plane * NF; i += ENC_BLOCK) s_g[i] = 0;
#endif
  int* my_g = s_g + (threadIdx.x & (copies - 1)) * g.size;
  const int type = (tex / VSA_NT_MAX_DEG) & 1;
  const unsigned* dFw = reinterpret_cast<const unsigned*>(dfeatures + nt_feat_plane_base(plan, type, level));
  __syncthreads();
  const int a_first = first & ~(ENC_UNROLL - 1);
  constexpr int PD = 1;
  const int s_max = (last - 1) & ~(ENC_UNROLL - 1);
  float4 xyn[PD][ENC_UNROLL / 2];
  uint4 dn[PD][ENC_UNROLL / 4];
  auto request = [&](int s, float4 (&xd)[ENC_UNROLL / 2], uint4 (&dd)[ENC_UNROLL / 4]) {
#if NT_ENC_DIAG & 16
    const int sc = (s < s_max ? s : s_max) & 0x1fff;
#else
    const int sc = s < s_max ? s : s_max;
#endif
#if NT_ENC_DIAG & 32
    const float4* xp = reinterpret_cast<const float4*>(slot_xy + (sc & 0x1fff));
#else
    const float4* xp = reinterpret_cast<const float4*>(slot_xy + sc);
#endif
    const uint4* dp = reinterpret_cast<const uint4*>(dFw + nt_feat_in_plane(nl, sc));
#pragma unroll
    for (int i = 0; i < ENC_UNROLL / 2; ++i) xd[i] = xp[i];
#pragma unroll
    for (int i = 0; i < ENC_UNROLL / 4; ++i) dd[i] = dp[i];
  };
#pragma unroll
  for (int d = 0; d < PD; ++d)
    request(a_first + threadIdx.x * ENC_UNROLL + d * ENC_BLOCK * ENC_UNROLL, xyn[d], dn[d]);
  for (int s0 = a_first + threadIdx.x * ENC_UNROLL; s0 < last; s0 += ENC_BLOCK * ENC_UNROLL) {
    float4 xyv[ENC_UNROLL / 2];
    uint4 dv[ENC_UNROLL / 4];
#pragma unroll
    for (int i = 0; i < ENC_UNROLL / 2; ++i) xyv[i] = xyn[0][i];
#pragma unroll
    for (int i = 0; i < ENC_UNROLL / 4; ++i) dv[i] = dn[0][i];
#pragma unroll
    for (int d = 0; d + 1 < PD; ++d) {
#pragma unroll
      for (int i = 0; i < ENC_UNROLL / 2; ++i) xyn[d][i] = xyn[d + 1][i];
#pragma unroll
      for (int i = 0; i < ENC_UNROLL / 4; ++i) dn[d][i] = dn[d + 1][i];
    }
    request(s0 + PD * ENC_BLOCK * ENC_UNROLL, xyn[PD - 1], dn[PD - 1]);
    const unsigned dws[ENC_UNROLL] = {dv[0].x, dv[0].y, dv[0].z, dv[0].w,
                                      dv[1].x, dv[1].y, dv[1].z, dv[1].w};
    unsigned cur_idx[4] = {0, 0, 0, 0};
    int acc[NF][4];
#pragma unroll
    for (int f = 0; f < NF; ++f) acc[f][0] = acc[f][1] = acc[f][2] = acc[f][3] = 0;
    unsigned cur_cx = 0xffffffffu, cur_cy = 0xffffffffu;
#pragma unroll
    for (int u = 0; u < ENC_UNROLL; ++u) {
      const int slot = s0 + u;
      const float x = (u & 1) ? xyv[u >> 1].z : xyv[u >> 1].x;
      const float y = (u & 1) ? xyv[u >> 1].w : xyv[u >> 1].y;
      float gv[NF];
      bool nz = false;
#pragma unroll
      for (int f = 0; f < NF; ++f) {
        gv[f] = NF == 2 ? (f ? enc_mul_mix<1>(dws[u], S[f]) : enc_mul_mix<0>(dws[u], S[f]))
                        : enc_mul_mix<0>(dws[u] >> (16 * feat), S[f]);
        nz |= gv[f] != 0.f;
      }
      if (slot >= first && slot < last && nz) {
        const CellRef cr = cell_ref(g, x, y);
        int v[NF][4];
#pragma unroll
        for (int f = 0; f < NF; ++f) {
          const f32x2 p01 = cr.w01 * gv[f], p23 = cr.w23 * gv[f];
          v[f][0] = enc_round_i(p01.x), v[f][1] = enc_round_i(p01.y);
          v[f][2] = enc_round_i(p23.x), v[f][3] = enc_round_i(p23.y);
        }
        if (!MERGE) {
          unsigned idx[4];
          cell_indices<HASHED>(g, cr.cx, cr.cy, idx);
#pragma unroll
          for (int f = 0; f < NF; ++f)
#pragma unroll
            for (int k = 0; k < 4; ++k) ENC_LDS_ADD(&my_g[f * plane + idx[k]], v[f][k]);
        } else if (cr.cx == cur_cx && cr.cy == cur_cy) {
#pragma unroll
          for (int f = 0; f < NF; ++f)
#pragma unroll
            for (int k = 0; k < 4; ++k) acc[f][k] += v[f][k];
        } else {
          if (cur_cx != 0xffffffffu) {
#pragma unroll
            for (int f = 0; f < NF; ++f)
#pragma unroll
              for (int k = 0; k < 4; ++k) ENC_LDS_ADD(&my_g[f * plane + cur_idx[k]], acc[f][k]);
          }
          cur_cx = cr.cx, cur_cy = cr.cy;
          cell_indices<HASHED>(g, cr.cx, cr.cy, cur_idx);
#pragma unroll
          for (int f = 0; f < NF; ++f)
#pragma unroll
            for (int k = 0; k < 4; ++k) acc[f][k] = v[f][k];
        }
      }
    }
    if (MERGE && cur_cx != 0xffffffffu) {
#pragma unroll
      for (int f = 0; f < NF; ++f)
#pragma unroll
        for (int k = 0; k < 4; ++k) ENC_LDS_ADD(&my_g[f * plane + cur_idx[k]], acc[f][k]);
    }
  }
#pragma unroll
  for (int d = 0; d < PD; ++d) {
#pragma unroll
    for (int i = 0; i < ENC_UNROLL / 2; ++i)
      asm volatile("" ::"v"(xyn[d][i].x), "v"(xyn[d][i].y), "v"(xyn[d][i].z), "v"(xyn[d][i].w));
#pragma unroll
    for (int i = 0; i < ENC_UNROLL / 4; ++i)
      asm volatile("" ::"v"(dn[d][i].x), "v"(dn[d][i].y), "v"(dn[d][i].z), "v"(dn[d][i].w));
  }
  __syncthreads();
#if NT_ENC_DIAG & 1
  return;
#endif
  float* gt = grad_tables + ((long long)nt_param_tex(plan, tex) * n_entries + plan.level_offset[level]) * 2 + feat;
  constexpr int FB = NT_ENC_FLUSH_BATCH;
  auto plane_sums = [&](int i0, int (&vi)[FB][NF]) {
#pragma unroll
    for (int b = 0; b < FB; ++b) {
      const int i = i0 + b * ENC_BLOCK;
#pragma unroll
      for (int f = 0; f < NF; ++f) {
        int acc = 0;
        if (i < (int)g.size)
          for (int cpy = 0; cpy < copies; ++cpy) acc += s_g[f * plane + cpy * g.size + i];
        vi[b][f] = acc;
      }
    }
  };
  if (store) {
    for (int i0 = threadIdx.x; i0 < (int)g.size; i0 += ENC_BLOCK * FB) {
      int vi[FB][NF];
      plane_sums(i0, vi);
#pragma unroll
      for (int b = 0; b < FB; ++b) {
        const long long i = i0 + b * ENC_BLOCK;
        if constexpr (NF == 2) {
          if ((vi[b][0] | vi[b][1]) != 0)
            *reinterpret_cast<float2*>(&gt[2 * i]) = make_float2((float)vi[b][0] * S_inv[0], (float)vi[b][1] * S_inv[1]);
        } else {
          if (vi[b][0] != 0) gt[2 * i] = (float)vi[b][0] * S_inv[0];
        }
      }
    }
  } else {
    for (int i0 = threadIdx.x; i0 < (int)g.size; i0 += ENC_BLOCK * FB) {
      int vi[FB][NF];
      plane_sums(i0, vi);
#pragma unroll
      for (int b = 0; b < FB; ++b)
#pragma unroll
        for (int f = 0; f < NF; ++f)
          if (vi[b][f] != 0) atomicAdd(&gt[2 * (long long)(i0 + b * ENC_BLOCK) + f], (float)vi[b][f] * S_inv[f]);
    }
  }
}

__device__ __host__ inline bool enc_both_features(const vsa_nt_plan& p, int level, bool hashed) {
  return !hashed && (long long)p.level_size[level] * 2 <= LDS_ENTRIES;
}

template <bool HASHED>
__device__ __forceinline__ void nt_encode_bwd_body(
    const vsa_nt_plan& plan, int level0, int n_levels, int n_planes,
    const half2_t* __restrict__ dfeatures, const float* __restrict__ dfeat_abs_sum,
    float dscale_inv, const float2* __restrict__ slot_xy, const int* __restrict__ seg_start,
    float* __restrict__ grad_tables, int tex_begin, int tex_end, unsigned char* s_raw) {
  int* s_g = reinterpret_cast<int*>(s_raw);
  NT_SPAN_MARK(HASHED ? 3 : 2, 0);
  NT_BAL_BEGIN();
  const bool full_range = tex_begin <= 0 && tex_end >= plan.nr_shells * 2 * VSA_NT_MAX_DEG;
  auto unit_weight = [&](int pl, int deg, int) {
    return !HASHED || plan.level_scale[level0 + (pl >> 1)] < (float)plan.tex_res[deg] ? 16 : 14;
  };
  nt_for_each_piece<ENC_UNIT>(plan, seg_start, n_planes, HASHED ? NT_ENC_OVH_BH : NT_ENC_OVH_BD,
                              [&](int pl, int tex, int first, int last, int seg_begin, int seg_end) {
    int level = level0, r = pl;
    bool both = enc_both_features(plan, level, HASHED);
    while (r >= (both ? 1 : 2)) {
      r -= both ? 1 : 2;
      ++level;
      both = enc_both_features(plan, level, HASHED);
    }
    const bool shared_plane = (((tex / VSA_NT_MAX_DEG) & 1) ? plan.shared_alpha : plan.shared_rgb) != 0;
    const bool store = plan.grads_zeroed != 0 && first == seg_begin && last == seg_end && !shared_plane;
    const bool merge = plan.level_scale[level] < (float)plan.tex_res[tex % VSA_NT_MAX_DEG];
    if (both)
      enc_bwd_piece<HASHED, 2, true>(plan, s_g, level, 0, tex, first, last, store, dfeatures,
                                     dfeat_abs_sum, dscale_inv, slot_xy, grad_tables);
    else if (merge)
      enc_bwd_piece<HASHED, 1, true>(plan, s_g, level, r, tex, first, last, store, dfeatures,
                                     dfeat_abs_sum, dscale_inv, slot_xy, grad_tables);
    else
      enc_bwd_piece<HASHED, 1, false>(plan, s_g, level, r, tex, first, last, store, dfeatures,
                                      dfeat_abs_sum, dscale_inv, slot_xy, grad_tables);
  }, tex_begin, tex_end, unit_weight,
     full_range ? (HASHED ? NT_BAL_ENC_BWD_H : NT_BAL_ENC_BWD_D) : -1);
  __syncthreads();
  NT_SPAN_MARK(HASHED ? 3 : 2, 1);
  if (full_range) { NT_BAL_END(HASHED ? NT_BAL_ENC_BWD_H : NT_BAL_ENC_BWD_D); }
}

template <bool HASHED>
__global__ __launch_bounds__(ENC_BLOCK) void nt_encode_bwd_kernel(
    vsa_nt_plan plan, int level0, int n_levels, int n_planes,
    const half2_t* __restrict__ dfeatures, const float* __restrict__ dfeat_abs_sum,
    float dscale_inv, const float2* __restrict__ slot_xy, const int* __restrict__ seg_start,
    float* __restrict__ grad_tables, int tex_begin, int tex_end) {
  extern __shared__ __attribute__((aligned(16))) unsigned char s_raw[];
  nt_encode_bwd_body<HASHED>(plan, level0, n_levels, n_planes, dfeatures, dfeat_abs_sum, dscale_inv, slot_xy,
                             seg_start, grad_tables, tex_begin, tex_end, s_raw);
}

__global__ __launch_bounds__(ENC_BLOCK) void nt_encode_bwd_both_kernel(
    vsa_nt_plan plan, int lh, int n_planes_dense,
    const half2_t* __restrict__ dfeatures, const float* __restrict__ dfeat_abs_sum,
    float dscale_inv, const float2* __restrict__ slot_xy, const int* __restrict__ seg_start,
    float* __restrict__ grad_tables, int tex_begin, int tex_end) {
  extern __shared__ __attribute__((aligned(16))) unsigned char s_raw[];
  nt_encode_bwd_body<false>(plan, 0, lh, n_planes_dense, dfeatures, dfeat_abs_sum, dscale_inv, slot_xy,
                            seg_start, grad_tables, tex_begin, tex_end, s_raw);
  __syncthreads();
  nt_encode_bwd_body<true>(plan, lh, plan.n_levels - lh, 2 * (plan.n_levels - lh), dfeatures, dfeat_abs_sum,
                           dscale_inv, slot_xy, seg_start, grad_tables, tex_begin, tex_end, s_raw);
}

struct EncPhases {
  int n;
  int shell_end[VSA_MAX_SHELLS];
  unsigned* flag[VSA_MAX_SHELLS];
};

__global__ __launch_bounds__(ENC_BLOCK) void nt_encode_bwd_phased_kernel(
    vsa_nt_plan plan, int lh, int n_planes_dense,
    const half2_t* __restrict__ dfeatures, const float* __restrict__ dfeat_abs_sum,
    float dscale_inv, const float2* __restrict__ slot_xy, const int* __restrict__ seg_start,
    float* __restrict__ grad_tables, EncPhases ph,
    unsigned* __restrict__ counters, const unsigned* __restrict__ epoch) {
  extern __shared__ __attribute__((aligned(16))) unsigned char s_raw[];
  if (lh > 0)
    nt_encode_bwd_body<false>(plan, 0, lh, n_planes_dense, dfeatures, dfeat_abs_sum, dscale_inv, slot_xy,
                              seg_start, grad_tables, 0, 1 << 30, s_raw);
  __syncthreads();
  int shell0 = 0;
  for (int p = 0; p < ph.n; ++p) {
    const int tex_begin = shell0 * 2 * VSA_NT_MAX_DEG, tex_end = ph.shell_end[p] * 2 * VSA_NT_MAX_DEG;
    shell0 = ph.shell_end[p];
    if (lh < plan.n_levels)
      nt_encode_bwd_body<true>(plan, lh, plan.n_levels - lh, 2 * (plan.n_levels - lh), dfeatures, dfeat_abs_sum,
                               dscale_inv, slot_xy, seg_start, grad_tables, tex_begin, tex_end, s_raw);
    __builtin_amdgcn_s_waitcnt(0);
    __syncthreads();
    if (threadIdx.x == 0) {
      __builtin_amdgcn_fence(__ATOMIC_RELEASE, "agent");
      const unsigned done = __hip_atomic_fetch_add(&counters[p], 1u, __ATOMIC_ACQ_REL, __HIP_MEMORY_SCOPE_AGENT);
      if (done == gridDim.x - 1) {
        __hip_atomic_store(&counters[p], 0u, __ATOMIC_RELAXED, __HIP_MEMORY_SCOPE_AGENT);
        __hip_atomic_store(ph.flag[p], *epoch, __ATOMIC_RELEASE, __HIP_MEMORY_SCOPE_SYSTEM);
      }
    }
  }
}

__global__ void dp_signal_kernel(unsigned* __restrict__ flag, unsigned* __restrict__ epoch, int advance) {
  unsigned e = *epoch;
  if (advance) *epoch = ++e;
  __hip_atomic_store(flag, e, __ATOMIC_RELEASE, __HIP_MEMORY_SCOPE_SYSTEM);
}

__global__ void dp_spin_wait_kernel(const unsigned* __restrict__ flag, unsigned value) {
  while ((int)(__hip_atomic_load(flag, __ATOMIC_RELAXED, __HIP_MEMORY_SCOPE_SYSTEM) - value) < 0)
    __builtin_amdgcn_s_sleep(64);
  __builtin_amdgcn_fence(__ATOMIC_ACQUIRE, "");
}

}

static bool level_hashed(const vsa_nt_plan* p, int l) {
  const long long res = p->level_res[l], size = p->level_size[l];
  return !(res <= size && res * res <= size);
}

static int first_hashed_level(const vsa_nt_plan* p) {
  int l = 0;
  while (l < p->n_levels && !level_hashed(p, l)) ++l;
  return l;
}

static int check_levels(const vsa_nt_plan* p) {
  const int lh = first_hashed_level(p);
  for (int l = lh; l < p->n_levels; ++l) {
    if (!level_hashed(p, l)) return VSA_ERR_UNSUPPORTED;
    const int sz = p->level_size[l];
    if ((sz & (sz - 1)) != 0 || sz > LDS_ENTRIES) return VSA_ERR_UNSUPPORTED;
  }
  for (int l = 0; l < lh; ++l)
    if (p->level_size[l] > LDS_ENTRIES) return VSA_ERR_UNSUPPORTED;
  return VSA_OK;
}

static int max_level_size(const vsa_nt_plan* p, int l0, int l1) {
  int m = 0;
  for (int l = l0; l < l1; ++l) m = m > p->level_size[l] ? m : p->level_size[l];
  return m;
}

template <typename K>
static int set_lds_attr(K kernel) {
  VSA_HIP_TRY(hipFuncSetAttribute(reinterpret_cast<const void*>(kernel),
                                  hipFuncAttributeMaxDynamicSharedMemorySize, 159 * 1024));
  return VSA_OK;
}

#ifdef NT_SPAN
extern "C" int vsa_span_read_encode(void* dst) {
  VSA_HIP_TRY(hipDeviceSynchronize());
  VSA_HIP_TRY(hipMemcpyFromSymbol(dst, HIP_SYMBOL(g_span), sizeof(g_span)));
  return 0;
}
#endif

extern "C" int vsa_nt_encode_fwd(const vsa_nt_plan* plan, const void* tables_h,
                                 const float* slot_xy, const int32_t* seg_start, void* features,
                                 void* stream) {
  if (!plan || !tables_h || !slot_xy || !seg_start || !features) return VSA_ERR_ARG;
  int rc = check_levels(plan);
  if (rc) return rc;
  static bool attr_set = false;
  if (!attr_set) {
    if ((rc = set_lds_attr(nt_encode_fwd_kernel<false>))) return rc;
    if ((rc = set_lds_attr(nt_encode_fwd_kernel<true>))) return rc;
    if ((rc = set_lds_attr(nt_encode_fwd_both_kernel))) return rc;
    attr_set = true;
  }
  const int lh = first_hashed_level(plan);
  const half2_t* tab = reinterpret_cast<const half2_t*>(tables_h);
  const float2* xy = reinterpret_cast<const float2*>(slot_xy);
  half2_t* out = reinterpret_cast<half2_t*>(features);
  int nr_cus = 0;
  if ((rc = vsa_cu_count(&nr_cus))) return rc;
  if (lh > 0 && lh < plan->n_levels) {
    hipLaunchKernelGGL(nt_encode_fwd_both_kernel, dim3(nr_cus), dim3(ENC_BLOCK), (size_t)LDS_ENTRIES * 4,
                       (hipStream_t)stream, *plan, lh, tab, xy, seg_start, out);
    VSA_RETURN_LAUNCH_STATUS();
  }
  if (lh > 0)
    hipLaunchKernelGGL(nt_encode_fwd_kernel<false>, dim3(nr_cus), dim3(ENC_BLOCK),
                       (size_t)LDS_ENTRIES * 4, (hipStream_t)stream, *plan, 0, lh, tab, xy,
                       seg_start, out);
  if (lh < plan->n_levels)
    hipLaunchKernelGGL(nt_encode_fwd_kernel<true>, dim3(nr_cus), dim3(ENC_BLOCK),
                       (size_t)LDS_ENTRIES * 4, (hipStream_t)stream, *plan, lh, plan->n_levels - lh,
                       tab, xy, seg_start, out);
  VSA_RETURN_LAUNCH_STATUS();
}

extern "C" int vsa_nt_encode_bwd(const vsa_nt_plan* plan, const void* dfeatures,
                                 const float* dfeat_abs_sum, float grad_scale,
                                 const float* slot_xy, const int32_t* seg_start,
                                 float* grad_tables, void* stream) {
  if (!plan) return VSA_ERR_ARG;
  return vsa_nt_encode_bwd_range(plan, dfeatures, dfeat_abs_sum, grad_scale, slot_xy, seg_start,
                                 grad_tables, 0, plan->nr_shells, stream);
}

extern "C" int vsa_nt_encode_bwd_range(const vsa_nt_plan* plan, const void* dfeatures,
                                       const float* dfeat_abs_sum, float grad_scale,
                                       const float* slot_xy, const int32_t* seg_start,
                                       float* grad_tables, int shell_begin, int shell_end,
                                       void* stream) {
  if (!plan || !dfeatures || !dfeat_abs_sum || !slot_xy || !seg_start || !grad_tables)
    return VSA_ERR_ARG;
  if (shell_begin < 0 || shell_end > plan->nr_shells || shell_begin > shell_end) return VSA_ERR_ARG;
  if (shell_begin == shell_end) return VSA_OK;
  if ((plan->shared_rgb || plan->shared_alpha) && !(shell_begin == 0 && shell_end == plan->nr_shells)) return VSA_ERR_UNSUPPORTED;
  const int tex_begin = shell_begin * 2 * VSA_NT_MAX_DEG, tex_end = shell_end * 2 * VSA_NT_MAX_DEG;
  if (!(grad_scale > 0.f)) return VSA_ERR_ARG;
  int rc = check_levels(plan);
  if (rc) return rc;
  static bool attr_set = false;
  if (!attr_set) {
    if ((rc = set_lds_attr(nt_encode_bwd_kernel<false>))) return rc;
    if ((rc = set_lds_attr(nt_encode_bwd_kernel<true>))) return rc;
    if ((rc = set_lds_attr(nt_encode_bwd_both_kernel))) return rc;
    attr_set = true;
  }
  const int lh = first_hashed_level(plan);
  const half2_t* dF = reinterpret_cast<const half2_t*>(dfeatures);
  const float2* xy = reinterpret_cast<const float2*>(slot_xy);
  int nr_cus = 0;
  if ((rc = vsa_cu_count(&nr_cus))) return rc;
  if (lh > 0 && lh < plan->n_levels) {
    int n_planes = 0;
    for (int l = 0; l < lh; ++l) n_planes += enc_both_features(*plan, l, false) ? 1 : 2;
    hipLaunchKernelGGL(nt_encode_bwd_both_kernel, dim3(nr_cus), dim3(ENC_BLOCK), (size_t)LDS_ENTRIES * 4,
                       (hipStream_t)stream, *plan, lh, n_planes, dF, dfeat_abs_sum, 1.0f / grad_scale, xy,
                       seg_start, grad_tables, tex_begin, tex_end);
    VSA_RETURN_LAUNCH_STATUS();
  }
  if (lh > 0) {
    int n_planes = 0;
    for (int l = 0; l < lh; ++l) n_planes += enc_both_features(*plan, l, false) ? 1 : 2;
    hipLaunchKernelGGL(nt_encode_bwd_kernel<false>, dim3(nr_cus), dim3(ENC_BLOCK),
                       (size_t)LDS_ENTRIES * 4, (hipStream_t)stream, *plan, 0, lh, n_planes, dF,
                       dfeat_abs_sum, 1.0f / grad_scale, xy, seg_start, grad_tables, tex_begin,
                       tex_end);
  }
  if (lh < plan->n_levels)
    hipLaunchKernelGGL(nt_encode_bwd_kernel<true>, dim3(nr_cus), dim3(ENC_BLOCK),
                       (size_t)LDS_ENTRIES * 4, (hipStream_t)stream, *plan, lh, plan->n_levels - lh,
                       2 * (plan->n_levels - lh), dF, dfeat_abs_sum, 1.0f / grad_scale, xy,
                       seg_start, grad_tables, tex_begin, tex_end);
  VSA_RETURN_LAUNCH_STATUS();
}

struct vsa_dp_flags {
  int n = 0;
  bool signal_memory = false;
  unsigned* word[VSA_MAX_SHELLS + 1] = {};
};

extern "C" int vsa_dp_flags_create(int n, vsa_dp_flags** out) {
  if (!out || n < 1 || n > VSA_MAX_SHELLS + 1) return VSA_ERR_ARG;
  vsa_dp_flags* f = new vsa_dp_flags();
  f->n = n;
  f->signal_memory = true;
  for (int i = 0; i < n; ++i) {
    void* p = nullptr;
    if (f->signal_memory && hipExtMallocWithFlags(&p, 8, hipMallocSignalMemory) != hipSuccess) {
      (void)hipGetLastError();
      f->signal_memory = false;
      for (int j = 0; j < i; ++j) (void)hipFree(f->word[j]);
      i = -1;
      continue;
    }
    if (!f->signal_memory) VSA_HIP_TRY(hipMalloc(&p, 8));
    VSA_HIP_TRY(hipMemset(p, 0, 8));
    f->word[i] = static_cast<unsigned*>(p);
  }
  *out = f;
  return VSA_OK;
}

extern "C" int vsa_dp_flags_destroy(vsa_dp_flags* f) {
  if (!f) return VSA_OK;
  for (int i = 0; i < f->n; ++i) (void)hipFree(f->word[i]);
  delete f;
  return VSA_OK;
}

extern "C" int vsa_dp_flags_read(const vsa_dp_flags* f, uint32_t* host_out) {
  if (!f || !host_out) return VSA_ERR_ARG;
  VSA_HIP_TRY(hipDeviceSynchronize());
  for (int i = 0; i < f->n; ++i) VSA_HIP_TRY(hipMemcpy(host_out + i, f->word[i], 4, hipMemcpyDeviceToHost));
  return VSA_OK;
}

extern "C" int vsa_nt_encode_bwd_phased(const vsa_nt_plan* plan, const void* dfeatures,
                                        const float* dfeat_abs_sum, float grad_scale,
                                        const float* slot_xy, const int32_t* seg_start,
                                        float* grad_tables, int n_phases, const int32_t* phase_shell_end,
                                        vsa_dp_flags* flags, uint32_t* counters, const uint32_t* epoch,
                                        int reserve_cus, void* stream) {
  if (!plan || !dfeatures || !dfeat_abs_sum || !slot_xy || !seg_start || !grad_tables || !phase_shell_end ||
      !flags || !counters || !epoch)
    return VSA_ERR_ARG;
  if (n_phases < 1 || n_phases > VSA_MAX_SHELLS || flags->n < n_phases || !(grad_scale > 0.f)) return VSA_ERR_ARG;
  if ((plan->shared_rgb || plan->shared_alpha) && n_phases != 1) return VSA_ERR_UNSUPPORTED;
  EncPhases ph;
  int prev = 0;
  for (int p = 0; p < n_phases; ++p) {
    if (phase_shell_end[p] <= prev || phase_shell_end[p] > plan->nr_shells) return VSA_ERR_ARG;
    ph.shell_end[p] = prev = phase_shell_end[p];
    ph.flag[p] = flags->word[p];
  }
  if (prev != plan->nr_shells) return VSA_ERR_ARG;
  ph.n = n_phases;
  int rc = check_levels(plan);
  if (rc) return rc;
  static bool attr_set = false;
  if (!attr_set) {
    if ((rc = set_lds_attr(nt_encode_bwd_phased_kernel))) return rc;
    attr_set = true;
  }
  const int lh = first_hashed_level(plan);
  int n_planes = 0;
  for (int l = 0; l < lh; ++l) n_planes += enc_both_features(*plan, l, false) ? 1 : 2;
  int nr_cus = 0;
  if ((rc = vsa_cu_count(&nr_cus))) return rc;
  if (reserve_cus < 0 || reserve_cus >= nr_cus) return VSA_ERR_ARG;
  nr_cus -= reserve_cus;
  hipLaunchKernelGGL(nt_encode_bwd_phased_kernel, dim3(nr_cus), dim3(ENC_BLOCK), (size_t)LDS_ENTRIES * 4,
                     (hipStream_t)stream, *plan, lh, n_planes, reinterpret_cast<const half2_t*>(dfeatures),
                     dfeat_abs_sum, 1.0f / grad_scale, reinterpret_cast<const float2*>(slot_xy), seg_start,
                     grad_tables, ph, counters, epoch);
  VSA_RETURN_LAUNCH_STATUS();
}

extern "C" int vsa_dp_signal(vsa_dp_flags* flags, int index, uint32_t* epoch, int advance_epoch, void* stream) {
  if (!flags || !epoch || index < 0 || index >= flags->n) return VSA_ERR_ARG;
  hipLaunchKernelGGL(dp_signal_kernel, dim3(1), dim3(1), 0, (hipStream_t)stream, flags->word[index], epoch,
                     advance_epoch);
  VSA_RETURN_LAUNCH_STATUS();
}

extern "C" int vsa_dp_stream_wait(vsa_dp_flags* flags, int index, uint32_t value, int mode, void* stream) {
  if (!flags || index < 0 || index >= flags->n || mode < 0 || mode > 2) return VSA_ERR_ARG;
  if (mode == 0) {
    int dev = 0, can = 0;
    VSA_HIP_TRY(hipGetDevice(&dev));
    VSA_HIP_TRY(hipDeviceGetAttribute(&can, hipDeviceAttributeCanUseStreamWaitValue, dev));
    mode = can && flags->signal_memory ? 1 : 2;
  }
  if (mode == 1) {
    VSA_HIP_TRY(hipStreamWaitValue32((hipStream_t)stream, flags->word[index], value, hipStreamWaitValueGte, 0xffffffffu));
    return VSA_OK;
  }
  hipLaunchKernelGGL(dp_spin_wait_kernel, dim3(1), dim3(1), 0, (hipStream_t)stream, flags->word[index], value);
  VSA_RETURN_LAUNCH_STATUS();
}
```

volsurfs_amd/neural_textures.py:

```python
import ctypes
import math
import os

import numpy as np
import torch

from . import _lib

MAX_SHELLS, MAX_DEG, MAX_LEVELS = 16, 4, 16
DOM_BLOCK = 4096
WEIGHTS_PER_TEX = 8192
REBALANCE = os.environ.get("VSA_NT_REBALANCE", "1") != "0"
FUSED_FORWARD = {"0": False, "1": True}.get(os.environ.get("VSA_NT_FUSED", "auto"), "auto")

class Plan(ctypes.Structure):
    _fields_ = [
        ("nr_shells", ctypes.c_int32), ("rgb_degrees", ctypes.c_int32),
        ("alpha_degrees", ctypes.c_int32), ("inner_solid", ctypes.c_int32),
        ("with_alpha_decay", ctypes.c_int32), ("n_levels", ctypes.c_int32),
        ("tex_res", ctypes.c_int32 * MAX_DEG), ("sh_lo", ctypes.c_float * MAX_DEG),
        ("sh_span", ctypes.c_float * MAX_DEG), ("level_scale", ctypes.c_float * MAX_LEVELS),
        ("level_res", ctypes.c_int32 * MAX_LEVELS), ("level_size", ctypes.c_int32 * MAX_LEVELS),
        ("level_offset", ctypes.c_int32 * (MAX_LEVELS + 1)),
        ("dom_off", ctypes.c_int64 * (MAX_SHELLS * MAX_DEG + 1)),
        ("slot_capacity", ctypes.c_int64),
        ("max_rays", ctypes.c_int32), ("anchor", ctypes.c_int32),
        ("row_base", ctypes.c_int64 * (MAX_SHELLS * MAX_DEG + 1)),
        ("balance", ctypes.c_void_p),
        ("row_format", ctypes.c_int32), ("grads_zeroed", ctypes.c_int32),
        ("shared_rgb", ctypes.c_int32), ("shared_alpha", ctypes.c_int32),
    ]


ROW_QUADS = (2, 4, 8, 8)
ALPHA_QUAD = (1, 3, 4, 6)


def grid_geometry(n_levels=16, log2_hashmap_size=15, base_resolution=16, per_level_scale=1.5):
    log2_pls = np.float32(math.log2(per_level_scale))
    scale, res, size, offset = [], [], [], [0]
    for l in range(n_levels):
        s = np.float32(np.exp2(np.float32(l) * log2_pls)) * np.float32(base_resolution) - np.float32(1.0)
        r = int(np.ceil(s)) + 1
        n = min((r * r + 7) // 8 * 8, 1 << log2_hashmap_size)
        scale.append(float(s))
        res.append(r)
        size.append(n)
        offset.append(offset[-1] + n)
    return scale, res, size, offset


class NeuralTextureBank(torch.nn.Module):
    def __init__(self, nr_shells, max_rays, sh_degree=3, alpha_sh_degree=3,
                 sh_range=(15.0, 15.0, 15.0, 15.0), textures_res=(2048, 1024, 512, 256),
                 inner_solid=False, with_alpha_decay=True, device="cuda", seed=42,
                 training=True, anchor=False, lerp=True, quantize_output=True, squeeze_output=True,
                 grid=None, shared_rgb=False, shared_alpha=False, parameters=True):
        super().__init__()
        if bool(anchor) == bool(lerp):
            raise ValueError("NeuralTexture is either anchor or lerp (neural_texture.py:47-51, 141-147)")
        if quantize_output and not squeeze_output:
            raise ValueError("quantize_output requires squeeze_output (sh_neural_textures.py:32-36)")
        self.row_format = 0 if quantize_output else (1 if squeeze_output else 2)
        self.shared_rgb, self.shared_alpha = bool(shared_rgb), bool(shared_alpha)
        self.anchor = bool(anchor)
        K = nr_shells
        self.K, self.max_rays = K, max_rays
        self.rgb_degrees, self.alpha_degrees = sh_degree + 1, alpha_sh_degree + 1
        self.D = max(self.rgb_degrees, self.alpha_degrees)
        scale, res, size, offset = grid_geometry(**(grid or {}))
        self.n_entries = offset[-1]
        self.n_tex = K * 2 * MAX_DEG
        p = Plan()
        p.nr_shells, p.rgb_degrees, p.alpha_degrees = K, self.rgb_degrees, self.alpha_degrees
        p.inner_solid, p.with_alpha_decay, p.n_levels = int(inner_solid), int(with_alpha_decay), 16
        for d in range(MAX_DEG):
            p.tex_res[d] = int(textures_res[d])
            p.sh_lo[d] = -float(sh_range[d])
            p.sh_span[d] = 2.0 * float(sh_range[d])
        for l in range(16):
            p.level_scale[l], p.level_res[l], p.level_size[l] = scale[l], res[l], size[l]
        for l in range(17):
            p.level_offset[l] = offset[l]
        off, cap, quads = 0, 0, 0
        for s in range(K):
            for d in range(MAX_DEG):
                p.dom_off[s * MAX_DEG + d] = off
                p.row_base[s * MAX_DEG + d] = quads
                if d < self.D:
                    T = (textures_res[d] + 2) ** 2
                    off += (T + DOM_BLOCK - 1) // DOM_BLOCK * DOM_BLOCK
                    cap += min(4 * max_rays, T)
                    quads += (min(4 * max_rays, T) * ROW_QUADS[d] + 7) // 8 * 8
        for i in range(K * MAX_DEG, MAX_SHELLS * MAX_DEG + 1):
            p.dom_off[i] = off
            p.row_base[i] = quads
        self.row_quads_total = quads
        cap = (cap + 255) // 256 * 256 + 256
        p.slot_capacity = cap
        p.max_rays = max_rays
        p.anchor = int(self.anchor)
        p.row_format = int(self.row_format)
        p.shared_rgb, p.shared_alpha = int(self.shared_rgb), int(self.shared_alpha)
        self.plan, self.dom_total, self.slot_capacity = p, off, cap
        self.tex_res = tuple(int(r) for r in textures_res)

        self.has_parameters = bool(parameters)
        if not parameters:
            self.tables = self.weights = None
            self._alloc(device, training=False)
            return
        g = torch.Generator().manual_seed(seed)
        tables = (torch.rand(self.n_tex, self.n_entries, 2, generator=g) * 2 - 1) * 1e-4
        weights = torch.zeros(self.n_tex, WEIGHTS_PER_TEX)
        for x in range(self.n_tex):
            C = self.tex_channels(x)
            if C and self.param_tex(x) != x:
                tables[x] = 0
                continue
            if C == 0:
                continue

            def xav(o, i):
                s_ = math.sqrt(6.0 / (i + o))
                return (torch.rand(o, i, generator=g) * 2 - 1) * s_
            w3 = torch.zeros(32, 64)
            pad = (C + 15) // 16 * 16
            w3[:C] = xav(pad, 64)[:C]
            weights[x] = torch.cat([xav(64, 32).flatten(), xav(64, 64).flatten(), w3.flatten()])
        self.tables = torch.nn.Parameter(tables.to(device))
        self.weights = torch.nn.Parameter(weights.to(device))
        self._alloc(device, training)

    def tex_channels(self, x):
        deg, typ, shell = x % MAX_DEG, (x // MAX_DEG) & 1, x // (2 * MAX_DEG)
        if typ == 0:
            return 3 * (2 * deg + 1) if deg < self.rgb_degrees else 0
        if self.plan.inner_solid and (shell == 0 or self.shared_alpha):
            return 0
        return (2 * deg + 1) if deg < self.alpha_degrees else 0

    def param_tex(self, x):
        typ = (x // MAX_DEG) & 1
        return x % (2 * MAX_DEG) if (self.shared_alpha if typ else self.shared_rgb) else x

    @staticmethod
    def tex_index(shell, typ, deg):
        return (shell * 2 + typ) * MAX_DEG + deg

    def _alloc(self, dev, training):
        i32, u8 = torch.int32, torch.uint8
        cap, K = self.slot_capacity, self.K
        if REBALANCE:
            fn = _lib.lib().vsa_nt_balance_bytes
            fn.restype = ctypes.c_longlong
            self.balance = torch.zeros(int(fn()), dtype=u8, device=dev)
            self.plan.balance = self.balance.data_ptr()
        self.marks = torch.zeros(self.dom_total, dtype=u8, device=dev)
        self.slot_of = torch.full((self.dom_total,), -1, dtype=i32, device=dev)
        self.texel_of_slot = torch.zeros(cap, dtype=i32, device=dev)
        self.slot_xy = torch.zeros(cap, 2, device=dev)
        self.seg_start = torch.zeros(K * MAX_DEG + 1, dtype=i32, device=dev)
        self.block_scratch = torch.zeros(self.dom_total // DOM_BLOCK + 1, dtype=i32, device=dev)
        texel_dtype = u8 if self.row_format == 0 else torch.float16
        if not self.has_parameters:
            self.features = self.tables_h = self.weights_h = self.grad_rows = None
            self.texels = torch.zeros(self.row_quads_total * 4, dtype=texel_dtype, device=dev)
            return
        self.features = torch.empty(2, cap // 256, 16, 256, 2, dtype=torch.float16, device=dev)
        self.tables_h = torch.empty(self.n_tex, self.n_entries, 2, dtype=torch.float16, device=dev)
        self.weights_h = torch.empty(self.n_tex, WEIGHTS_PER_TEX, dtype=torch.float16, device=dev)
        self.texels = torch.zeros(self.row_quads_total * 4, dtype=texel_dtype, device=dev)
        self.grad_rows = torch.zeros(self.row_quads_total * 4, dtype=torch.float16, device=dev) if training else None
        self.refresh_half_params()

    @torch.no_grad()
    def refresh_half_params(self):
        self.wait_params()
        self.tables_h.copy_(self.tables)
        self.weights_h.copy_(self.weights)

    def mark_and_compact(self, hit_slot, hit_uv, face_uvs, want_texel_of_slot=False):
        K, N = hit_slot.shape
        assert K == self.K and N <= self.max_rays
        if getattr(self, "baked", False):
            raise _lib.VolsurfsHipError("this bank holds baked textures: use tex_uv_only + shade")
        st = _lib.stream_ptr()
        tex_uv = torch.empty(K, N, 2, device=hit_slot.device)
        if getattr(self, "_marks_dirty", False):
            self.marks.zero_()
        self._marks_dirty = True
        _lib.call("vsa_nt_mark", ctypes.byref(self.plan), hit_slot, hit_uv, face_uvs, N, tex_uv,
                  self.marks, st)
        _lib.call("vsa_nt_compact_frame", ctypes.byref(self.plan), self.marks, self.slot_of,
                  self.texel_of_slot if want_texel_of_slot else None, self.slot_xy, self.seg_start,
                  self.block_scratch, st)
        self._marks_dirty = False
        return tex_uv

    @staticmethod
    def full_capacity_rays(textures_res):
        return ((max(int(r) for r in textures_res) + 2) ** 2 + 3) // 4

    @torch.no_grad()
    def bake_all(self):
        if self.row_format != 0:
            raise _lib.VolsurfsHipError("baked textures are the 8-bit deploy format: using_sh_quantization=1 only")
        self.compact_all()
        self.evaluate(need_features=False)
        self.baked = True
        return self

    @torch.no_grad()
    def compact_all(self, want_texel_of_slot=True):
        self.marks.zero_()
        for s in range(self.K):
            for d in range(self.D):
                R = self.tex_res[d]
                W = R + 2
                if min(4 * self.max_rays, W * W) < W * W:
                    raise _lib.VolsurfsHipError("bake_all needs a full-capacity bank "
                                                "(max_rays >= NeuralTextureBank.full_capacity_rays)")
                off = int(self.plan.dom_off[s * MAX_DEG + d])
                self.marks[off:off + W * W].view(W, W).fill_(1)
        _lib.call("vsa_nt_compact_frame", ctypes.byref(self.plan), self.marks, self.slot_of,
                  self.texel_of_slot if want_texel_of_slot else None, self.slot_xy, self.seg_start,
                  self.block_scratch, _lib.stream_ptr())

    @torch.no_grad()
    def baked_textures(self):
        dense = self.rows_dense(self.texels)
        out = {}
        for s in range(self.K):
            for d in range(self.D):
                R = self.tex_res[d]
                W, n = R + 2, 2 * d + 1
                off = int(self.plan.dom_off[s * MAX_DEG + d])
                slots = self.slot_of[off:off + W * W].view(W, W)[1:R + 1, 1:R + 1].long()
                rows = dense[slots]
                if self.tex_channels(self.tex_index(s, 0, d)):
                    out[(s, 0, d)] = rows[..., :3 * n].contiguous()
                if self.tex_channels(self.tex_index(s, 1, d)):
                    out[(s, 1, d)] = rows[..., 24:24 + n].contiguous()
        return out

    def tex_uv_only(self, hit_slot, hit_uv, face_uvs):
        K, N = hit_slot.shape
        tex_uv = torch.empty(K, N, 2, device=hit_slot.device)
        _lib.call("vsa_nt_mark", ctypes.byref(self.plan), hit_slot, hit_uv, face_uvs, N, tex_uv,
                  None, _lib.stream_ptr())
        return tex_uv

    def wait_params(self):
        ev = getattr(self, "_params_event", None)
        if ev is not None:
            torch.cuda.current_stream().wait_event(ev)
            self._params_event = None

    def encode(self):
        self.wait_params()
        _lib.call("vsa_nt_encode_fwd", ctypes.byref(self.plan), self.tables_h, self.slot_xy,
                  self.seg_start, self.features, _lib.stream_ptr())
        return self.features

    def features_level_major(self):
        f = self.features.permute(0, 2, 1, 3, 4)
        return f.reshape(2, 16, self.slot_capacity, 2)

    def mlp(self, want_pre=False):
        self.wait_params()
        pre = None
        if want_pre:
            pre = torch.zeros(self.slot_capacity, 32, dtype=torch.float16, device=self.texels.device)
        _lib.call("vsa_nt_mlp_fwd", ctypes.byref(self.plan), self.weights_h, self.features,
                  self.seg_start, self.texels, pre, _lib.stream_ptr())
        return (self.rows_dense(self.texels), pre) if want_pre else self.texels

    def encode_mlp(self, write_features=True, want_pre=False):
        self.wait_params()
        pre = None
        if want_pre:
            pre = torch.zeros(self.slot_capacity, 32, dtype=torch.float16, device=self.texels.device)
        _lib.call("vsa_nt_encode_mlp_fwd", ctypes.byref(self.plan), self.tables_h, self.weights_h,
                  self.slot_xy, self.seg_start, self.features if write_features else None,
                  self.texels, pre, _lib.stream_ptr())
        return (self.rows_dense(self.texels), pre) if want_pre else self.texels

    def evaluate(self, need_features=True):
        if self.row_format == 0 and (FUSED_FORWARD is True or (FUSED_FORWARD == "auto" and not need_features)):
            return self.encode_mlp(write_features=need_features)
        self.encode()
        return self.mlp()

    def rows_dense(self, buf):
        seg = self.seg_start.cpu().tolist()
        dense = torch.zeros(self.slot_capacity, 32, dtype=buf.dtype, device=buf.device)
        for s in range(self.K):
            for d in range(self.D):
                sd, n, q = s * MAX_DEG + d, 2 * d + 1, ROW_QUADS[d]
                a, b = seg[sd], seg[sd + 1]
                r0 = int(self.plan.row_base[sd]) * 4
                rows = buf[r0:r0 + (b - a) * q * 4].view(b - a, q * 4)
                dense[a:b, :3 * n] = rows[:, :3 * n]
                dense[a:b, 24:24 + n] = rows[:, 4 * ALPHA_QUAD[d]:4 * ALPHA_QUAD[d] + n]
        return dense

    def shade(self, hit_slot, tex_uv, rays_d, tris, want_coeffs=False, want_normals=False,
              act_out=None):
        K, N = hit_slot.shape
        dev = hit_slot.device
        rgb = torch.empty(N, K, 3, device=dev)
        alpha = torch.empty(N, K, device=dev)
        normals = torch.empty(N, K, 3, device=dev) if want_normals else None
        coeffs = torch.empty(K, N, 64, device=dev) if want_coeffs else None
        _lib.call("vsa_nt_shade_fwd", ctypes.byref(self.plan), hit_slot, tex_uv, rays_d, tris,
                  self.slot_of, self.seg_start, self.texels, N, rgb, alpha, normals, coeffs,
                  act_out, _lib.stream_ptr())
        return rgb, alpha, normals, coeffs

    def backward(self, hit_slot, tex_uv, rays_d, tris, g_surfs_rgb, g_surfs_alpha, grad_scale,
                 act=None, grads_zeroed=None):
        self.backward_shade(hit_slot, tex_uv, rays_d, tris, g_surfs_rgb, g_surfs_alpha, grad_scale,
                            act)
        self.backward_mlp(grad_scale)
        self.backward_encode(grad_scale, grads_zeroed=grads_zeroed)

    def _ensure_grads(self):
        if self.tables.grad is None:
            self.tables.grad = torch.zeros_like(self.tables)
        if self.weights.grad is None:
            self.weights.grad = torch.zeros_like(self.weights)

    def zero_grads(self):
        flat = getattr(self, "_grad_flat", None)
        nt, nw = self.tables.numel(), self.weights.numel()
        if flat is None:
            flat = torch.zeros(nt + nw + self.n_tex * 32, device=self.tables.device)
            self._grad_flat = flat
            self._flat_t, self._flat_w = flat[:nt].view_as(self.tables), flat[nt:nt + nw].view_as(self.weights)
            self._dfsum = flat[nt + nw:].view(self.n_tex, 32)
        if self.tables.grad is None and self.weights.grad is None:
            self.tables.grad, self.weights.grad = self._flat_t, self._flat_w
        self._tables_grad_zero = True
        if self.tables.grad is self._flat_t and self.weights.grad is self._flat_w:
            flat.zero_()
            self._dfsum_clean = True
            self._tables_grad_sig = (id(self.tables.grad), self.tables.grad._version)
            return True
        self.tables.grad.zero_()
        self.weights.grad.zero_()
        self._tables_grad_sig = (id(self.tables.grad), self.tables.grad._version)
        return False

    def _take_grads_zeroed(self, grads_zeroed):
        z = bool(getattr(self, "_tables_grad_zero", False) if grads_zeroed is None else grads_zeroed)
        if grads_zeroed is None and z:
            g = self.tables.grad
            z = g is not None and getattr(self, "_tables_grad_sig", None) == (id(g), g._version)
        self._tables_grad_zero = False
        self.plan.grads_zeroed = int(z)

    def backward_shade(self, hit_slot, tex_uv, rays_d, tris, g_surfs_rgb, g_surfs_alpha, grad_scale,
                       act=None):
        self._ensure_grads()
        if act is not None:
            _lib.check_f32(act, hit_slot.shape[0], hit_slot.shape[1], 4)
        _lib.call("vsa_nt_shade_bwd", ctypes.byref(self.plan), hit_slot, tex_uv, rays_d, tris,
                  self.slot_of, self.seg_start, self.texels, hit_slot.shape[1],
                  g_surfs_rgb.contiguous(),
                  g_surfs_alpha.contiguous(), float(grad_scale), self.grad_rows, act,
                  _lib.stream_ptr())

    def backward_mlp(self, grad_scale):
        if getattr(self, "_dfsum", None) is None:
            self._dfsum = torch.zeros(self.n_tex, 32, device=self.weights.device)
        elif not getattr(self, "_dfsum_clean", False):
            self._dfsum.zero_()
        self._dfsum_clean = False
        _lib.call("vsa_nt_mlp_bwd", ctypes.byref(self.plan), self.weights_h, self.features,
                  self.seg_start, self.grad_rows, self.weights.grad, self._dfsum,
                  1.0 / float(grad_scale), _lib.stream_ptr())

    def backward_encode(self, grad_scale, shells=None, grads_zeroed=None):
        self._take_grads_zeroed(grads_zeroed)
        if shells is None:
            _lib.call("vsa_nt_encode_bwd", ctypes.byref(self.plan), self.features, self._dfsum,
                      float(grad_scale), self.slot_xy, self.seg_start, self.tables.grad,
                      _lib.stream_ptr())
        else:
            _lib.call("vsa_nt_encode_bwd_range", ctypes.byref(self.plan), self.features,
                      self._dfsum, float(grad_scale), self.slot_xy, self.seg_start,
                      self.tables.grad, int(shells[0]), int(shells[1]), _lib.stream_ptr())

    def backward_encode_phased(self, grad_scale, signals, grads_zeroed=None):
        self._take_grads_zeroed(grads_zeroed)
        _lib.call("vsa_nt_encode_bwd_phased", ctypes.byref(self.plan), self.features, self._dfsum,
                  float(grad_scale), self.slot_xy, self.seg_start, self.tables.grad, signals.n,
                  signals.phase_end_c, signals._flags, signals.counters, signals.epoch, int(signals.reserve_cus),
                  _lib.stream_ptr())


def stage_accounting(bank, nr_rays, nr_hits, tracer_bytes=0):
    N, K, M = nr_rays, bank.K, nr_hits
    P = int(bank.seg_start[K * 4].item())
    seg = bank.seg_start.cpu().tolist()
    fl, row_quads, slot_models = 0, 0, 0
    for s_ in range(K):
        for d in range(4):
            P_sd = seg[s_ * 4 + d + 1] - seg[s_ * 4 + d]
            row_quads += P_sd * ROW_QUADS[d]
            for typ in range(2):
                C = bank.tex_channels(bank.tex_index(s_, typ, d))
                if C:
                    fl += P_sd * 2 * (32 * 64 + 64 * 64 + 64 * C)
                    slot_models += P_sd
    ntex = sum(1 for x in range(bank.n_tex) if bank.tex_channels(x))
    rows_u8, rows_f16 = row_quads * 4, row_quads * 8
    feats = slot_models * 64
    gathers = M * (16 * 4 + 4 * sum(ROW_QUADS) * 4 + 8) + N * 12
    acct = {
        "trace": N * (24 + 16 * K) + tracer_bytes,
        "nt_mark_compact": N * K * 20 + bank.dom_total * (1 + 1) + P * (1 + 1 + 4 + 8),
        "nt_encode_fwd": P * 8 + feats + ntex * bank.n_entries * 4,
        "nt_mlp_fwd": feats + rows_u8 + ntex * 8192 * 2,
        "nt_encode_mlp_fwd": slot_models * 8 + feats + rows_u8 + ntex * (bank.n_entries * 4 + 8192 * 2),
        "nt_shade_fwd": gathers + N * K * 16,
        "nt_shade_bwd": gathers + N * K * 16 + rows_f16,
        "nt_mlp_bwd": 2 * feats + 2 * rows_f16 + ntex * 8192 * (2 + 4),
        "nt_encode_bwd": feats + P * 8 + ntex * bank.n_entries * 8,
    }
    return acct, fl, P
```

volsurfs_amd/pipeline.py:

```python
import torch

from . import _lib
from .camera import pinhole_rays
from .mesh import nested_shells, stress_shells
from .raytrace import RayTracer


GRAD_CHAIN_GAIN = 16.0

_CAPTURE_MODE = "thread_local"


class _no_gc:

    def __enter__(self):
        import gc
        gc.collect()
        self.was = gc.isenabled()
        gc.disable()

    def __exit__(self, *exc):
        import gc
        if self.was:
            gc.enable()


class StageTimer:
    def __init__(self):
        self.records = []
        self.meta = {}

    def run(self, name, fn, record, **meta):
        if not record:
            return fn()
        s = torch.cuda.Event(enable_timing=True)
        e = torch.cuda.Event(enable_timing=True)
        s.record()
        out = fn()
        e.record()
        self.records.append((name, s, e))
        self.meta[name] = meta
        return out

    def report(self):
        torch.cuda.synchronize()
        acc, cnt = {}, {}
        for name, s, e in self.records:
            acc[name] = acc.get(name, 0.0) + s.elapsed_time(e)
            cnt[name] = cnt.get(name, 0) + 1
        return {k: dict(ms=acc[k] / cnt[k], **self.meta[k]) for k in acc}


class KShellPipeline:
    dtype_desc = "f16 (hash features, MLP on MFMA, composite: as the reference), f32 accumulate and I/O"

    def __init__(self, meshes, rays_o, rays_d, gt_rgb, bg_color=(1.0, 1.0, 1.0), seed=42,
                 init="tcnn", image_hw=None, tracer=None, bvh_builder="host"):
        from .neural_textures import NeuralTextureBank
        self.meshes = meshes
        self.K = len(meshes)
        self.tracer = RayTracer(meshes, builder=bvh_builder) if tracer is None else tracer
        self.rays_o, self.rays_d, self.gt = rays_o, rays_d, gt_rgb
        self.nr_rays = rays_o.shape[0]
        self.image_hw = None
        if image_hw is not None and image_hw[0] % 8 == 0 and image_hw[1] % 8 == 0 and \
                image_hw[0] * image_hw[1] == self.nr_rays:
            self.image_hw = (int(image_hw[0]), int(image_hw[1]))
            self._o_t, self._d_t, self._gt_t = (torch.empty_like(x) for x in (rays_o, rays_d, gt_rgb))
            self._rgb_out = torch.empty_like(gt_rgb)
            H, W = self.image_hw
            tiles = torch.arange(H * W, device=rays_o.device).reshape(H // 8, 8, W // 8, 8).permute(0, 2, 1, 3).clone()
            tiles[:, :, 1::2] = tiles[:, :, 1::2].flip(-1)
            self._tile_idx = tiles.reshape(-1)
        dev = rays_o.device
        self.bg = torch.tensor([bg_color], device=dev, dtype=torch.float32)
        self.timer = StageTimer()
        N, K = self.nr_rays, self.K
        fu = []
        for m, off, n in zip(meshes, self.tracer.mesh_tri_offset, self.tracer.mesh_nr_tris):
            ids = self.tracer.slot_face_id[off:off + n].long()
            fu.append(m.faces_uvs.reshape(-1, 6)[ids])
        self.face_uvs = torch.cat(fu, 0).contiguous()
        self.bank = NeuralTextureBank(K, N, device=dev, seed=seed)
        if init == "spread":
            g = torch.Generator().manual_seed(seed)
            with torch.no_grad():
                self.bank.tables.copy_((torch.rand(self.bank.tables.shape, generator=g) * 2 - 1).to(dev))
            self.bank.refresh_half_params()
        self.shading = "neural_textures"
        self.grad_scale = GRAD_CHAIN_GAIN * float(N)
        self.loss_rays = N
        self.surfs_rgb = self.surfs_alpha = None
        self._act = torch.empty(K, N, 4, device=dev)

    def to_ray_order(self, x, dim=0):
        if self.image_hw is None:
            return x
        out = torch.empty_like(x)
        out.index_copy_(dim, self._tile_idx, x)
        return out

    @classmethod
    def synthetic(cls, K=5, subdiv=6, res=800, device="cuda", seed=42, rows=None, gt_seed=None,
                  noise=0.0, atlas_charts=0, stress=False, cam_pos=(0.0, 0.0, -1.5), **kw):
        if stress:
            meshes = stress_shells(K=K, subdiv=subdiv, device=device)
        else:
            meshes = nested_shells(K=K, subdiv=subdiv, device=device, noise=noise, atlas_charts=atlas_charts)
        H, W = (res, res) if isinstance(res, int) else res
        o, d = pinhole_rays(H, W, focal=1111.1 * min(H, W) / 800.0, cam_pos=cam_pos, device=device)
        g = torch.Generator(device=device).manual_seed(seed if gt_seed is None else gt_seed)
        gt = torch.rand(o.shape[0], 3, device=device, generator=g)
        n_frame, h_local = H * W, H
        if rows is not None:
            rows = rows.to(device)
            o, d, gt = (x.view(H, W, 3)[rows].reshape(-1, 3).contiguous() for x in (o, d, gt))
            h_local = int(rows.numel())
        p = cls(meshes, o, d, gt, seed=seed, image_hw=(h_local, W), **kw)
        p.loss_rays = n_frame
        p.grad_scale = GRAD_CHAIN_GAIN * float(n_frame)
        p.res = res
        p.subdiv = subdiv
        p.scene_desc = ("stress shells: 4 lobes of depth 0.3 r across the view axis (non-convex, up to 6 crossings per "
                        "ray), triangle areas spread 12x, 256 randomly packed uv charts per shell, noise 0.05, "
                        f"parameters {kw.get('init', 'tcnn')}-initialised") if stress else \
            (f"noise {noise}, {atlas_charts}x{atlas_charts} randomly packed uv charts per shell, "
             f"parameters {kw.get('init', 'tcnn')}-initialised") if (noise or atlas_charts) else \
            "perfect spheres, one continuous octahedral uv chart, tcnn-initialised parameters"
        return p

    def reset_stage_timers(self):
        self.timer = StageTimer()

    def stage_report(self):
        return self.timer.report()

    @staticmethod
    def stage_roofline(st, hbm_peak, mfma_peak):
        sec = st["ms"] * 1e-3
        out = {}
        if st.get("bytes"):
            out["GB/s"] = round(st["bytes"] / sec / 1e9, 1)
            out["hbm_frac"] = round(st["bytes"] / sec / 1e9 / hbm_peak, 4)
        if st.get("flops"):
            out["TFLOP/s"] = round(st["flops"] / sec / 1e12, 2)
            out["mfma_frac"] = round(st["flops"] / sec / 1e12 / mfma_peak, 4)
        return out

    def config_desc(self, world):
        return {
            "workload": f"synthetic kitten-like: {self.res if isinstance(self.res, int) else self.res[1]}x"
                        f"{self.res if isinstance(self.res, int) else self.res[0]} rays, K={self.K} nested "
                        f"icospheres subdiv {self.subdiv} ({self.tracer.mesh_nr_tris[0]} tris each), "
                        "SH-degree-3 neural textures (rgb + alpha per shell, res 2048/1024/512/256, "
                        "16-level 2-D hash grid + 32-64-64-C MLP, 8-bit quantised, lerp), alpha decay, "
                        "white bg, L1 loss, gradients to all hash tables and MLP weights",
            "rays_per_gpu": self.nr_rays,
            "global_rays": self.loss_rays if self.loss_rays != self.nr_rays else self.nr_rays * world,
            "parallelism": f"tile-parallel x{world}",
            "hits_per_frame": getattr(self, "last_hits", None),
            "unique_texels_per_frame": getattr(self, "last_slots", None),
            "trace_launch_order": "cost feedback from the previous frame (static camera: the previous frame has "
                                  "the same rays; value_cold is the figure without any inter-frame feedback)"
                                  if self.tracer.cost_feedback and
                                  self.tracer.node_format == "q16" else "natural",
        }

    def stats(self):
        from .neural_textures import stage_accounting
        bank, N, K = self.bank, self.nr_rays, self.K
        self.last_hits = M = int((self._hit_slot >= 0).sum().item())
        nodes_b = self.tracer.nodes.numel() * 4 + self.tracer.tris.numel() * 4
        self.acct, self.mlp_flops_fwd, self.last_slots = stage_accounting(bank, N, M, nodes_b)
        return self.last_hits, self.last_slots

    def capture_graph_split(self, **step_kw):
        self._static_rgb = None
        self._graph_dp = dp = step_kw.get("dp")
        s = torch.cuda.Stream()
        s.wait_stream(torch.cuda.current_stream())
        hook, _ = (dp.on_weights_final, setattr(dp, "on_weights_final", None)) if dp is not None else (None, None)
        with torch.cuda.stream(s):
            for _ in range(2):
                self.step(**step_kw)
        if dp is not None:
            dp.on_weights_final = hook
        torch.cuda.current_stream().wait_stream(s)
        self._graph_prefix, self._graph_mid, self._graph_tail = (torch.cuda.CUDAGraph() for _ in range(3))
        with _no_gc():
            with torch.cuda.graph(self._graph_prefix, capture_error_mode=_CAPTURE_MODE):
                self.step(part="prefix", **step_kw)
            with torch.cuda.graph(self._graph_mid, pool=self._graph_prefix.pool(), capture_error_mode=_CAPTURE_MODE):
                self.step(part="mid", **step_kw)
            with torch.cuda.graph(self._graph_tail, pool=self._graph_prefix.pool(), capture_error_mode=_CAPTURE_MODE):
                self._static_rgb = self.step(part="tail", **step_kw)

    def replay_prefix(self):
        self._graph_prefix.replay()

    def _count_replay(self):
        dp = getattr(self, "_graph_dp", None)
        if dp is not None:
            dp.epoch_host += 1

    def replay_mid(self):
        self._graph_mid.replay()
        self._count_replay()

    def replay_tail(self):
        self._graph_tail.replay()
        return self._static_rgb

    def replay_rest(self):
        self._graph_mid.replay()
        self._count_replay()
        self._graph_tail.replay()
        return self._static_rgb

    def capture_graph(self, **step_kw):
        self._static_rgb = None
        self._graph_dp = dp = step_kw.get("dp")
        s = torch.cuda.Stream()
        s.wait_stream(torch.cuda.current_stream())
        hook, _ = (dp.on_weights_final, setattr(dp, "on_weights_final", None)) if dp is not None else (None, None)
        with torch.cuda.stream(s):
            for _ in range(2):
                self.step(**step_kw)
        if dp is not None:
            dp.on_weights_final = hook
        torch.cuda.current_stream().wait_stream(s)
        self._graph = torch.cuda.CUDAGraph()
        with _no_gc(), torch.cuda.graph(self._graph, capture_error_mode=_CAPTURE_MODE):
            self._static_rgb = self.step(**step_kw)
        return self._graph

    def replay(self):
        self._graph.replay()
        self._count_replay()
        return self._static_rgb

    def step(self, record=False, grad_ready=None, dp=None, part=None):
        from .composite import composite_fwd_raw, composite_bwd_raw
        N, K = self.nr_rays, self.K
        T, bank = self.timer, self.bank
        acct = getattr(self, "acct", None) or {}

        if part == "tail":
            return self._step_tail(record, acct, grad_ready, dp, self._mid_out)
        if part in ("rest", "mid"):
            rays_d, gt, hit_slot, tex_uv = self._prefix_out
        else:
            rays_d, gt, hit_slot, tex_uv = self._step_prefix(record, acct)
            if part == "prefix":
                self._prefix_out = (rays_d, gt, hit_slot, tex_uv)
                return None
        T.run("zero_grad", bank.zero_grads, record, bytes=(bank.tables.numel() + bank.weights.numel()) * 4)
        rgb = self._step_rest(record, acct, dp, rays_d, gt, hit_slot, tex_uv)
        if part == "mid":
            self._mid_out = rgb
            return None
        if dp is not None and dp.on_weights_final is not None and not torch.cuda.is_current_stream_capturing():
            dp.on_weights_final()
        return self._step_tail(record, acct, grad_ready, dp, rgb)

    def _step_prefix(self, record, acct):
        N, T, bank = self.nr_rays, self.timer, self.bank
        rays_o, rays_d, gt = self.rays_o, self.rays_d, self.gt
        if self.image_hw is not None:
            H, W = self.image_hw

            T.run("ray_tile_order",
                  lambda: _lib.call("vsa_tile_order_rays", self.rays_o, self.rays_d, self.gt, self._o_t,
                                    self._d_t, self._gt_t, H, W, _lib.stream_ptr()),
                  record, bytes=N * 72)
            rays_o, rays_d, gt = self._o_t, self._d_t, self._gt_t
        hit_t, hit_slot, hit_uv = T.run(
            "trace", lambda: self.tracer.trace_all(rays_o, rays_d), record,
            bytes=acct.get("trace", 0))
        self._hit_slot = hit_slot
        tex_uv = T.run("nt_mark_compact",
                       lambda: bank.mark_and_compact(hit_slot, hit_uv, self.face_uvs), record,
                       bytes=acct.get("nt_mark_compact", 0))
        return rays_d, gt, hit_slot, tex_uv

    def _step_rest(self, record, acct, dp, rays_d, gt, hit_slot, tex_uv):
        N, K = self.nr_rays, self.K
        T, bank = self.timer, self.bank
        mlp_flops = getattr(self, "mlp_flops_fwd", 0)
        from . import neural_textures as _nt
        if _nt.FUSED_FORWARD is True:
            T.run("nt_encode_mlp_fwd", bank.encode_mlp, record, bytes=acct.get("nt_encode_mlp_fwd", 0),
                  flops=mlp_flops, bound="mfma")
        else:
            T.run("nt_encode_fwd", bank.encode, record, bytes=acct.get("nt_encode_fwd", 0))
            T.run("nt_mlp_fwd", bank.mlp, record, bytes=acct.get("nt_mlp_fwd", 0), flops=mlp_flops,
                  bound="mfma")
        rgb_k, alpha_k, _, _ = T.run(
            "nt_shade_fwd", lambda: bank.shade(hit_slot, tex_uv, rays_d, self.tracer.tris,
                                               act_out=self._act),
            record, bytes=acct.get("nt_shade_fwd", 0))
        self.surfs_rgb, self.surfs_alpha = rgb_k, alpha_k
        from .composite import composite_fwd_bwd_l1_raw
        rgb, g_c, g_a = T.run("composite_fwd_bwd",
                              lambda: composite_fwd_bwd_l1_raw(rgb_k, alpha_k, self.bg, gt,
                                                               1.0 / (3.0 * self.loss_rays)),
                              record, bytes=N * (12 + 12 + 32 * K))
        if self.image_hw is not None:
            T.run("rgb_row_order", lambda: _lib.call("vsa_tile_order", rgb, self._rgb_out, self.image_hw[0],
                                                     self.image_hw[1], 3, 1, _lib.stream_ptr()),
                  record, bytes=N * 24)
            rgb = self._rgb_out
        tris = self.tracer.tris
        T.run("nt_shade_bwd", lambda: bank.backward_shade(hit_slot, tex_uv, rays_d, tris, g_c, g_a,
                                                           self.grad_scale, self._act), record,
              bytes=acct.get("nt_shade_bwd", 0), bound="atomic")
        T.run("nt_mlp_bwd", lambda: bank.backward_mlp(self.grad_scale), record,
              bytes=acct.get("nt_mlp_bwd", 0), flops=2 * mlp_flops, bound="mfma")
        if dp is not None:
            dp.signal_weights()
        return rgb

    def _step_tail(self, record, acct, grad_ready, dp, rgb):
        K, T, bank = self.K, self.timer, self.bank
        enc_bytes = acct.get("nt_encode_bwd", 0)
        if dp is not None:
            T.run("nt_encode_bwd", lambda: bank.backward_encode_phased(self.grad_scale, dp), record,
                  bytes=enc_bytes)
        elif grad_ready is None:
            T.run("nt_encode_bwd", lambda: bank.backward_encode(self.grad_scale), record,
                  bytes=enc_bytes)
        else:
            grad_ready(bank.weights.grad)

            def by_shell():
                for s in range(K):
                    bank.backward_encode(self.grad_scale, shells=(s, s + 1))
                    grad_ready(bank.tables.grad[s * 8:(s + 1) * 8])
            T.run("nt_encode_bwd", by_shell, record, bytes=enc_bytes)
        return rgb
```

Baseline: 266.9.

## Fuse row-order scatter into composite and pair dense textures in encode backward

The composite forward+backward+L1 kernel now writes the predicted RGB straight into row-major image order, which removes the separate tile-order kernel launch and its extra pass over the output. Separately, the dense-level encode backward can now walk two textures' features at once (paired levels), sharing the slot coordinate loads and LDS accumulation. Piece overheads become per-piece through a callable, and the balancing constants are retuned. The pairing doubles the LDS planes per piece, which reduces LDS copies and adds register pressure. The row-order output is written with scattered 12-byte stores instead of coalesced ones.

Result: no change. 268.1, median of 6 (+0.5%).

```diff
diff --git a/include/volsurfs_hip.h b/include/volsurfs_hip.h
--- a/include/volsurfs_hip.h
+++ b/include/volsurfs_hip.h
@@ -37,6 +37,12 @@
                                    float loss_scale, float* out_rgb, float* g_surfs_rgb,
                                    float* g_surfs_alpha, int nr_rays, int nr_shells, int carry_f16,
                                    void* stream);
+
+int vsa_composite_dense_fwd_bwd_l1_rm(const float* surfs_rgb, const float* surfs_alpha,
+                                      const float* rgb_bg, int bg_is_broadcast, const float* gt_rgb,
+                                      float loss_scale, float* out_rgb, float* out_rgb_rm, int height,
+                                      int width, float* g_surfs_rgb, float* g_surfs_alpha, int nr_shells,
+                                      int carry_f16, void* stream);
 
 long long vsa_reduce_scratch_bytes(void);
 int vsa_count_hits(const int32_t* hit_slot, long long n, void* scratch, int64_t* out, void* stream);
@@ -173,6 +179,8 @@
                             const float* dfeat_abs_sum, float grad_scale, const float* slot_xy,
                             const int32_t* seg_start, float* grad_tables, int shell_begin,
                             int shell_end, void* stream);
+
+int vsa_nt_encode_bwd_pair_levels(const vsa_nt_plan* plan);
 
 typedef struct vsa_dp_flags vsa_dp_flags;
 int vsa_dp_flags_create(int n, vsa_dp_flags** out);
diff --git a/volsurfs_amd/composite.py b/volsurfs_amd/composite.py
--- a/volsurfs_amd/composite.py
+++ b/volsurfs_amd/composite.py
@@ -122,6 +122,22 @@
     return rgb, g_c, g_a
 
 
+def composite_fwd_bwd_l1_rm_raw(surfs_rgb, surfs_alpha, rgb_bg, gt_rgb, loss_scale, image_hw, out_rm=None,
+                                carry_f16=False, tile_ordered=False):
+    N, K, _ = surfs_rgb.shape
+    H, W = image_hw
+    if H * W != N:
+        raise ValueError("image_hw does not match the ray count")
+    rgb_rm = out_rm if out_rm is not None else torch.empty(N, 3, device=surfs_rgb.device)
+    rgb = torch.empty(N, 3, device=surfs_rgb.device) if tile_ordered else None
+    g_c = torch.empty_like(surfs_rgb)
+    g_a = torch.empty_like(surfs_alpha)
+    bcast = rgb_bg.shape[0] == 1 and N != 1
+    _lib.call("vsa_composite_dense_fwd_bwd_l1_rm", surfs_rgb, surfs_alpha, rgb_bg, bcast, gt_rgb,
+              float(loss_scale), rgb, rgb_rm, int(H), int(W), g_c, g_a, K, int(carry_f16), _lib.stream_ptr())
+    return (rgb_rm, rgb, g_c, g_a) if tile_ordered else (rgb_rm, g_c, g_a)
+
+
 _reduce_scratch = {}
 
 
diff --git a/volsurfs_amd/csrc/composite_dense.hip b/volsurfs_amd/csrc/composite_dense.hip
--- a/volsurfs_amd/csrc/composite_dense.hip
+++ b/volsurfs_amd/csrc/composite_dense.hip
@@ -168,14 +168,20 @@
   slab_store<3, 3>(out_rgb + ray0 * 3, s_o, rows);
 }
 
+struct __attribute__((packed, aligned(4))) F3 {
+  float x, y, z;
+};
+
 template <int K, bool CARRY_F16>
 __global__ __launch_bounds__(TILE) void composite_dense_bwd_kernel(
     const float* __restrict__ surfs_rgb, const float* __restrict__ surfs_alpha,
     const float* __restrict__ rgb_bg, int bg_bcast, const float* __restrict__ g_rgb,
     float* __restrict__ g_surfs_rgb, float* __restrict__ g_surfs_alpha,
     float* __restrict__ g_rgb_bg, int N, const float* __restrict__ l1_gt, float l1_scale,
-    float* __restrict__ pred_out, const vsa_train_ctl* __restrict__ ctl) {
+    float* __restrict__ pred_out, const vsa_train_ctl* __restrict__ ctl,
+    float* __restrict__ pred_rm, int W) {
   using L = Lds<K>;
+  const bool fused_fwd = pred_out || pred_rm;
   int n_active = N;
   if (ctl) {
     l1_scale = ctl->loss_scale;
@@ -190,7 +196,7 @@
   const int rows = min(TILE, (int)(N - ray0));
   slab_load<3 * K, L::SC>(surfs_rgb + ray0 * 3 * K, s_c, rows);
   slab_load<K, L::SA>(surfs_alpha + ray0 * K, s_a, rows);
-  if (!pred_out) slab_load<3, 3>(g_rgb + ray0 * 3, s_g, rows);
+  if (!fused_fwd) slab_load<3, 3>(g_rgb + ray0 * 3, s_g, rows);
   if (!bg_bcast) slab_load<3, 3>(rgb_bg + ray0 * 3, s_b, rows);
   if (l1_gt) slab_load<3, 3>(l1_gt + ray0 * 3, s_t, rows);
   slab_load_fence();
@@ -205,12 +211,21 @@
 #pragma unroll
     for (int ch = 0; ch < 3; ++ch) {
       bg[ch] = vsa_round_f16(bg_bcast ? rgb_bg[ch] : s_b[r * 3 + ch]);
-      if (pred_out) {
+      if (fused_fwd) {
         g[ch] = vsa_round_f16(f.fg[ch] + vsa_round_f16(f.bgT * bg[ch]));
         s_g[r * 3 + ch] = g[ch];
       } else {
         g[ch] = s_g[r * 3 + ch];
       }
+    }
+    if (pred_rm) {
+      const long long i = ray0 + r, t = i >> 6;
+      const int j = (int)(i & 63), tiles_x = W >> 3;
+      const long long px = ((t / tiles_x) * 8 + (j >> 3)) * W + (t % tiles_x) * 8 + ((j & 8) ? 7 - (j & 7) : (j & 7));
+      *reinterpret_cast<F3*>(pred_rm + px * 3) = F3{g[0], g[1], g[2]};
+    }
+#pragma unroll
+    for (int ch = 0; ch < 3; ++ch) {
       if (l1_gt) {
         const float d = g[ch] - s_t[r * 3 + ch];
         g[ch] = ray0 + r >= n_active ? 0.f : (d > 0.f ? l1_scale : (d < 0.f ? -l1_scale : 0.f));
@@ -284,10 +299,10 @@
                                 float* g_surfs_rgb, float* g_surfs_alpha, float* g_rgb_bg,
                                 int nr_rays, int nr_shells, int carry_f16, const float* l1_gt,
                                 float l1_scale, void* stream, float* pred_out = nullptr,
-                                const vsa_train_ctl* ctl = nullptr) {
+                                const vsa_train_ctl* ctl = nullptr, float* pred_rm = nullptr, int width = 0) {
   if (nr_rays < 0) return VSA_ERR_ARG;
   if (nr_rays == 0) return VSA_OK;
-  if (!surfs_rgb || !surfs_alpha || !rgb_bg || (!g_rgb && !pred_out) || !g_surfs_rgb || !g_surfs_alpha)
+  if (!surfs_rgb || !surfs_alpha || !rgb_bg || (!g_rgb && !pred_out && !pred_rm) || !g_surfs_rgb || !g_surfs_alpha)
     return VSA_ERR_ARG;
   dim3 grid(vsa_div_up(nr_rays, TILE)), block(TILE);
   hipStream_t st = (hipStream_t)stream;
@@ -295,11 +310,11 @@
     if (carry_f16)
       hipLaunchKernelGGL((composite_dense_bwd_kernel<KK, true>), grid, block, 0, st, surfs_rgb,
                          surfs_alpha, rgb_bg, bg_is_broadcast, g_rgb, g_surfs_rgb, g_surfs_alpha,
-                         g_rgb_bg, nr_rays, l1_gt, l1_scale, pred_out, ctl);
+                         g_rgb_bg, nr_rays, l1_gt, l1_scale, pred_out, ctl, pred_rm, width);
     else
       hipLaunchKernelGGL((composite_dense_bwd_kernel<KK, false>), grid, block, 0, st, surfs_rgb,
                          surfs_alpha, rgb_bg, bg_is_broadcast, g_rgb, g_surfs_rgb, g_surfs_alpha,
-                         g_rgb_bg, nr_rays, l1_gt, l1_scale, pred_out, ctl);
+                         g_rgb_bg, nr_rays, l1_gt, l1_scale, pred_out, ctl, pred_rm, width);
   });
   VSA_RETURN_LAUNCH_STATUS();
 }
@@ -337,6 +352,21 @@
                               loss_scale, stream, out_rgb);
 }
 
+extern "C" int vsa_composite_dense_fwd_bwd_l1_rm(const float* surfs_rgb, const float* surfs_alpha,
+                                                 const float* rgb_bg, int bg_is_broadcast,
+                                                 const float* gt_rgb, float loss_scale, float* out_rgb,
+                                                 float* out_rgb_rm, int height, int width, float* g_surfs_rgb,
+                                                 float* g_surfs_alpha, int nr_shells, int carry_f16,
+                                                 void* stream) {
+  if (height < 0 || width < 0 || (height & 7) || (width & 7)) return VSA_ERR_ARG;
+  const long long n = (long long)height * width;
+  if (n > 0x7fffffffll) return VSA_ERR_ARG;
+  if (!gt_rgb || (n > 0 && !out_rgb_rm) || (out_rgb && out_rgb == out_rgb_rm)) return VSA_ERR_ARG;
+  return composite_bwd_launch(surfs_rgb, surfs_alpha, rgb_bg, bg_is_broadcast, nullptr, g_surfs_rgb,
+                              g_surfs_alpha, nullptr, (int)n, nr_shells, carry_f16, gt_rgb,
+                              loss_scale, stream, out_rgb, nullptr, out_rgb_rm, width);
+}
+
 extern "C" int vsa_composite_dense_fwd_bwd_l1_ctl(const float* surfs_rgb, const float* surfs_alpha,
                                                   const float* rgb_bg, int bg_is_broadcast, const float* gt_rgb,
                                                   const vsa_train_ctl* ctl, float* out_rgb, float* g_surfs_rgb,
diff --git a/volsurfs_amd/csrc/nt_common.h b/volsurfs_amd/csrc/nt_common.h
--- a/volsurfs_amd/csrc/nt_common.h
+++ b/volsurfs_amd/csrc/nt_common.h
@@ -1,4 +1,6 @@
 #pragma once
+#include <type_traits>
+
 #include "common.h"
 
 typedef _Float16 half2_t __attribute__((ext_vector_type(2)));
@@ -201,15 +203,21 @@
   return ((tex / VSA_NT_MAX_DEG) & 1) == 0 && tex_active(p, other) ? other : -1;
 }
 
-template <int UNIT, typename Body, typename Weight = NtUnitWeight16>
+template <typename Ovh>
+__device__ __forceinline__ int nt_piece_ovh(const Ovh& ovh, int pl, int wtype) {
+  if constexpr (std::is_integral<Ovh>::value) return ovh;
+  else return ovh(pl, wtype);
+}
+
+template <int UNIT, typename Ovh, typename Body, typename Weight = NtUnitWeight16>
 __device__ __forceinline__ void nt_for_each_piece(const vsa_nt_plan& plan,
                                                   const int* __restrict__ seg_start, int n_planes,
-                                                  int ovh, Body&& body, int tex_begin = 0,
+                                                  const Ovh& ovh, Body&& body, int tex_begin = 0,
                                                   int tex_end = 1 << 30, Weight wt = Weight(), int bal_id = -1,
                                                   bool paired = false) {
   const int n_all = plan.nr_shells * 2 * VSA_NT_MAX_DEG;
   if (n_all > 64) {
-    nt_for_each_piece_scalar<UNIT>(plan, seg_start, n_planes, ovh, body, tex_begin, tex_end, wt, bal_id);
+    nt_for_each_piece_scalar<UNIT>(plan, seg_start, n_planes, nt_piece_ovh(ovh, 0, 0), body, tex_begin, tex_end, wt, bal_id);
     return;
   }
   const int n_tex = tex_end < n_all ? tex_end : n_all;
@@ -237,7 +245,7 @@
   const unsigned long long act_mask = __ballot(act);
   const long long pieces = __popcll(act_mask);
   if (pieces == 0) return;
-  auto lane_cost = [&](int pl) { return act ? ovh * 16 + units * wt(pl, deg, wtype) : 0; };
+  auto lane_cost = [&](int pl) { return act ? nt_piece_ovh(ovh, pl, wtype) * 16 + units * wt(pl, deg, wtype) : 0; };
   auto plane_cost = [&](int pl) -> long long {
     return (long long)(unsigned)__builtin_amdgcn_readlane(nt_wave_incl_scan(lane_cost(pl)), 63);
   };
@@ -255,7 +263,7 @@
       c0 += pc;
       continue;
     }
-    const long long t0l = c0 + (long long)(incl - cl) + (long long)ovh * 16;
+    const long long t0l = c0 + (long long)(incl - cl) + (long long)nt_piece_ovh(ovh, pl, wtype) * 16;
     const int w = wt(pl, deg, wtype);
     const long long span = (long long)units * w;
     bool hit = act && t0l < hi;
diff --git a/volsurfs_amd/csrc/nt_encode.hip b/volsurfs_amd/csrc/nt_encode.hip
--- a/volsurfs_amd/csrc/nt_encode.hip
+++ b/volsurfs_amd/csrc/nt_encode.hip
@@ -15,10 +15,16 @@
 #define NT_ENC_OVH_BH 145
 #endif
 #ifndef NT_ENC_OVH_BD
-#define NT_ENC_OVH_BD 64
+#define NT_ENC_OVH_BD 69
 #endif
 #ifndef NT_ENC_PAIR_W
 #define NT_ENC_PAIR_W 22
+#endif
+#ifndef NT_ENC_OVH_BDP
+#define NT_ENC_OVH_BDP 82
+#endif
+#ifndef NT_ENC_PAIR_WB
+#define NT_ENC_PAIR_WB 24
 #endif
 constexpr int ENC_BLOCK = 1024;
 constexpr int ENC_UNROLL = 8;
@@ -223,25 +229,31 @@
 #else
 #define ENC_LDS_ADD(ptr, val) atomicAdd(ptr, val)
 #endif
-template <bool HASHED, int NF, bool MERGE>
+template <bool HASHED, int NF, bool MERGE, bool PAIR = false>
 __device__ __forceinline__ void enc_bwd_piece(
-    const vsa_nt_plan& plan, int* s_g, int level, int feat, int tex, int first, int last,
+    const vsa_nt_plan& plan, int* s_g, int level, int feat, int tex, int tex2, int first, int last,
     bool store, const half2_t* __restrict__ dfeatures, const float* __restrict__ dfeat_abs_sum,
     float dscale_inv, const float2* __restrict__ slot_xy, float* __restrict__ grad_tables) {
   const int nl = plan.n_levels;
   const long long n_entries = plan.level_offset[plan.n_levels];
   const LevelGeom g = level_geom(plan, level);
-  float S[NF], S_inv[NF];
+  static_assert(!PAIR || (NF == 2 && !HASHED), "a pair walks both features of two dense textures");
+  constexpr int NT = PAIR ? 2 : 1;
+  constexpr int NP = NT * NF;
+  const int texs[2] = {tex, PAIR ? tex2 : tex};
+  float S[NT][NF], S_inv[NT][NF];
   bool any = false;
 #pragma unroll
+  for (int t = 0; t < NT; ++t)
+#pragma unroll
   for (int f = 0; f < NF; ++f) {
-    const float total = dfeat_abs_sum[tex * 32 + 2 * level + feat + f] * 1.001f;
-    S[f] = 0.f, S_inv[f] = 0.f;
+    const float total = dfeat_abs_sum[texs[t] * 32 + 2 * level + feat + f] * 1.001f;
+    S[t][f] = 0.f, S_inv[t][f] = 0.f;
     if (total > 0.f) {
       int e;
       frexpf(total, &e);
-      S[f] = ldexpf(1.0f, 30 - e);
-      S_inv[f] = ldexpf(1.0f, e - 30) * dscale_inv;
+      S[t][f] = ldexpf(1.0f, 30 - e);
+      S_inv[t][f] = ldexpf(1.0f, e - 30) * dscale_inv;
       any = true;
     }
   }
@@ -251,23 +263,24 @@
 #endif
   int copies = 1;
   if (!HASHED) {
-    while (copies < 32 && (long long)g.size * copies * 2 * NF <= LDS_ENTRIES) copies *= 2;
+    while (copies < 32 && (long long)g.size * copies * 2 * NP <= LDS_ENTRIES) copies *= 2;
   }
   const int plane = (int)g.size * copies;
   __syncthreads();
 #if !(NT_ENC_DIAG & 2)
-  for (int i = threadIdx.x; i < plane * NF; i += ENC_BLOCK) s_g[i] = 0;
+  for (int i = threadIdx.x; i < plane * NP; i += ENC_BLOCK) s_g[i] = 0;
 #endif
   int* my_g = s_g + (threadIdx.x & (copies - 1)) * g.size;
   const int type = (tex / VSA_NT_MAX_DEG) & 1;
   const unsigned* dFw = reinterpret_cast<const unsigned*>(dfeatures + nt_feat_plane_base(plan, type, level));
+  const unsigned* dFw2 = reinterpret_cast<const unsigned*>(dfeatures + nt_feat_plane_base(plan, 1, level));
   __syncthreads();
   const int a_first = first & ~(ENC_UNROLL - 1);
   constexpr int PD = 1;
   const int s_max = (last - 1) & ~(ENC_UNROLL - 1);
   float4 xyn[PD][ENC_UNROLL / 2];
-  uint4 dn[PD][ENC_UNROLL / 4];
-  auto request = [&](int s, float4 (&xd)[ENC_UNROLL / 2], uint4 (&dd)[ENC_UNROLL / 4]) {
+  uint4 dn[PD][NT * (ENC_UNROLL / 4)];
+  auto request = [&](int s, float4 (&xd)[ENC_UNROLL / 2], uint4 (&dd)[NT * (ENC_UNROLL / 4)]) {
 #if NT_ENC_DIAG & 16
     const int sc = (s < s_max ? s : s_max) & 0x1fff;
 #else
@@ -283,50 +296,61 @@
     for (int i = 0; i < ENC_UNROLL / 2; ++i) xd[i] = xp[i];
 #pragma unroll
     for (int i = 0; i < ENC_UNROLL / 4; ++i) dd[i] = dp[i];
+    if constexpr (PAIR) {
+      const uint4* dp2 = reinterpret_cast<const uint4*>(dFw2 + nt_feat_in_plane(nl, sc));
+#pragma unroll
+      for (int i = 0; i < ENC_UNROLL / 4; ++i) dd[ENC_UNROLL / 4 + i] = dp2[i];
+    }
   };
 #pragma unroll
   for (int d = 0; d < PD; ++d)
     request(a_first + threadIdx.x * ENC_UNROLL + d * ENC_BLOCK * ENC_UNROLL, xyn[d], dn[d]);
   for (int s0 = a_first + threadIdx.x * ENC_UNROLL; s0 < last; s0 += ENC_BLOCK * ENC_UNROLL) {
     float4 xyv[ENC_UNROLL / 2];
-    uint4 dv[ENC_UNROLL / 4];
+    uint4 dv[NT * (ENC_UNROLL / 4)];
 #pragma unroll
     for (int i = 0; i < ENC_UNROLL / 2; ++i) xyv[i] = xyn[0][i];
 #pragma unroll
-    for (int i = 0; i < ENC_UNROLL / 4; ++i) dv[i] = dn[0][i];
+    for (int i = 0; i < NT * (ENC_UNROLL / 4); ++i) dv[i] = dn[0][i];
 #pragma unroll
     for (int d = 0; d + 1 < PD; ++d) {
 #pragma unroll
       for (int i = 0; i < ENC_UNROLL / 2; ++i) xyn[d][i] = xyn[d + 1][i];
 #pragma unroll
-      for (int i = 0; i < ENC_UNROLL / 4; ++i) dn[d][i] = dn[d + 1][i];
+      for (int i = 0; i < NT * (ENC_UNROLL / 4); ++i) dn[d][i] = dn[d + 1][i];
     }
     request(s0 + PD * ENC_BLOCK * ENC_UNROLL, xyn[PD - 1], dn[PD - 1]);
-    const unsigned dws[ENC_UNROLL] = {dv[0].x, dv[0].y, dv[0].z, dv[0].w,
-                                      dv[1].x, dv[1].y, dv[1].z, dv[1].w};
+    unsigned dws[NT][ENC_UNROLL];
+#pragma unroll
+    for (int t = 0; t < NT; ++t) {
+      dws[t][0] = dv[2 * t].x, dws[t][1] = dv[2 * t].y, dws[t][2] = dv[2 * t].z, dws[t][3] = dv[2 * t].w;
+      dws[t][4] = dv[2 * t + 1].x, dws[t][5] = dv[2 * t + 1].y, dws[t][6] = dv[2 * t + 1].z, dws[t][7] = dv[2 * t + 1].w;
+    }
     unsigned cur_idx[4] = {0, 0, 0, 0};
-    int acc[NF][4];
-#pragma unroll
-    for (int f = 0; f < NF; ++f) acc[f][0] = acc[f][1] = acc[f][2] = acc[f][3] = 0;
+    int acc[NP][4];
+#pragma unroll
+    for (int f = 0; f < NP; ++f) acc[f][0] = acc[f][1] = acc[f][2] = acc[f][3] = 0;
     unsigned cur_cx = 0xffffffffu, cur_cy = 0xffffffffu;
 #pragma unroll
     for (int u = 0; u < ENC_UNROLL; ++u) {
       const int slot = s0 + u;
       const float x = (u & 1) ? xyv[u >> 1].z : xyv[u >> 1].x;
       const float y = (u & 1) ? xyv[u >> 1].w : xyv[u >> 1].y;
-      float gv[NF];
+      float gv[NP];
       bool nz = false;
 #pragma unroll
+      for (int t = 0; t < NT; ++t)
+#pragma unroll
       for (int f = 0; f < NF; ++f) {
-        gv[f] = NF == 2 ? (f ? enc_mul_mix<1>(dws[u], S[f]) : enc_mul_mix<0>(dws[u], S[f]))
-                        : enc_mul_mix<0>(dws[u] >> (16 * feat), S[f]);
-        nz |= gv[f] != 0.f;
+        gv[t * NF + f] = NF == 2 ? (f ? enc_mul_mix<1>(dws[t][u], S[t][f]) : enc_mul_mix<0>(dws[t][u], S[t][f]))
+                                 : enc_mul_mix<0>(dws[t][u] >> (16 * feat), S[t][f]);
+        nz |= gv[t * NF + f] != 0.f;
       }
       if (slot >= first && slot < last && nz) {
         const CellRef cr = cell_ref(g, x, y);
-        int v[NF][4];
-#pragma unroll
-        for (int f = 0; f < NF; ++f) {
+        int v[NP][4];
+#pragma unroll
+        for (int f = 0; f < NP; ++f) {
           const f32x2 p01 = cr.w01 * gv[f], p23 = cr.w23 * gv[f];
           v[f][0] = enc_round_i(p01.x), v[f][1] = enc_round_i(p01.y);
           v[f][2] = enc_round_i(p23.x), v[f][3] = enc_round_i(p23.y);
@@ -335,25 +359,25 @@
           unsigned idx[4];
           cell_indices<HASHED>(g, cr.cx, cr.cy, idx);
 #pragma unroll
-          for (int f = 0; f < NF; ++f)
+          for (int f = 0; f < NP; ++f)
 #pragma unroll
             for (int k = 0; k < 4; ++k) ENC_LDS_ADD(&my_g[f * plane + idx[k]], v[f][k]);
         } else if (cr.cx == cur_cx && cr.cy == cur_cy) {
 #pragma unroll
-          for (int f = 0; f < NF; ++f)
+          for (int f = 0; f < NP; ++f)
 #pragma unroll
             for (int k = 0; k < 4; ++k) acc[f][k] += v[f][k];
         } else {
           if (cur_cx != 0xffffffffu) {
 #pragma unroll
-            for (int f = 0; f < NF; ++f)
+            for (int f = 0; f < NP; ++f)
 #pragma unroll
               for (int k = 0; k < 4; ++k) ENC_LDS_ADD(&my_g[f * plane + cur_idx[k]], acc[f][k]);
           }
           cur_cx = cr.cx, cur_cy = cr.cy;
           cell_indices<HASHED>(g, cr.cx, cr.cy, cur_idx);
 #pragma unroll
-          for (int f = 0; f < NF; ++f)
+          for (int f = 0; f < NP; ++f)
 #pragma unroll
             for (int k = 0; k < 4; ++k) acc[f][k] = v[f][k];
         }
@@ -361,7 +385,7 @@
     }
     if (MERGE && cur_cx != 0xffffffffu) {
 #pragma unroll
-      for (int f = 0; f < NF; ++f)
+      for (int f = 0; f < NP; ++f)
 #pragma unroll
         for (int k = 0; k < 4; ++k) ENC_LDS_ADD(&my_g[f * plane + cur_idx[k]], acc[f][k]);
     }
@@ -372,14 +396,17 @@
     for (int i = 0; i < ENC_UNROLL / 2; ++i)
       asm volatile("" ::"v"(xyn[d][i].x), "v"(xyn[d][i].y), "v"(xyn[d][i].z), "v"(xyn[d][i].w));
 #pragma unroll
-    for (int i = 0; i < ENC_UNROLL / 4; ++i)
+    for (int i = 0; i < NT * (ENC_UNROLL / 4); ++i)
       asm volatile("" ::"v"(dn[d][i].x), "v"(dn[d][i].y), "v"(dn[d][i].z), "v"(dn[d][i].w));
   }
   __syncthreads();
 #if NT_ENC_DIAG & 1
   return;
 #endif
-  float* gt = grad_tables + ((long long)nt_param_tex(plan, tex) * n_entries + plan.level_offset[level]) * 2 + feat;
+#pragma unroll
+  for (int t = 0; t < NT; ++t) {
+  const int* s_t = s_g + t * NF * plane;
+  float* gt = grad_tables + ((long long)nt_param_tex(plan, texs[t]) * n_entries + plan.level_offset[level]) * 2 + feat;
   constexpr int FB = NT_ENC_FLUSH_BATCH;
   auto plane_sums = [&](int i0, int (&vi)[FB][NF]) {
 #pragma unroll
@@ -389,7 +416,7 @@
       for (int f = 0; f < NF; ++f) {
         int acc = 0;
         if (i < (int)g.size)
-          for (int cpy = 0; cpy < copies; ++cpy) acc += s_g[f * plane + cpy * g.size + i];
+          for (int cpy = 0; cpy < copies; ++cpy) acc += s_t[f * plane + cpy * g.size + i];
         vi[b][f] = acc;
       }
     }
@@ -403,9 +430,9 @@
         const long long i = i0 + b * ENC_BLOCK;
         if constexpr (NF == 2) {
           if ((vi[b][0] | vi[b][1]) != 0)
-            *reinterpret_cast<float2*>(&gt[2 * i]) = make_float2((float)vi[b][0] * S_inv[0], (float)vi[b][1] * S_inv[1]);
+            *reinterpret_cast<float2*>(&gt[2 * i]) = make_float2((float)vi[b][0] * S_inv[t][0], (float)vi[b][1] * S_inv[t][1]);
         } else {
-          if (vi[b][0] != 0) gt[2 * i] = (float)vi[b][0] * S_inv[0];
+          if (vi[b][0] != 0) gt[2 * i] = (float)vi[b][0] * S_inv[t][0];
         }
       }
     }
@@ -417,13 +444,28 @@
       for (int b = 0; b < FB; ++b)
 #pragma unroll
         for (int f = 0; f < NF; ++f)
-          if (vi[b][f] != 0) atomicAdd(&gt[2 * (long long)(i0 + b * ENC_BLOCK) + f], (float)vi[b][f] * S_inv[f]);
-    }
+          if (vi[b][f] != 0) atomicAdd(&gt[2 * (long long)(i0 + b * ENC_BLOCK) + f], (float)vi[b][f] * S_inv[t][f]);
+    }
+  }
   }
 }
 
 __device__ __host__ inline bool enc_both_features(const vsa_nt_plan& p, int level, bool hashed) {
   return !hashed && (long long)p.level_size[level] * 2 <= LDS_ENTRIES;
+}
+__device__ __forceinline__ int enc_plane_level(const vsa_nt_plan& p, int level0, int pl, bool hashed, int& r) {
+  int level = level0;
+  r = pl;
+  bool both = enc_both_features(p, level, hashed);
+  while (r >= (both ? 1 : 2)) {
+    r -= both ? 1 : 2;
+    ++level;
+    both = enc_both_features(p, level, hashed);
+  }
+  return level;
+}
+__device__ __host__ inline bool enc_pair_level(const vsa_nt_plan& p, int level) {
+  return (long long)p.level_size[level] * 4 <= LDS_ENTRIES;
 }
 
 template <bool HASHED>
@@ -431,37 +473,55 @@
     const vsa_nt_plan& plan, int level0, int n_levels, int n_planes,
     const half2_t* __restrict__ dfeatures, const float* __restrict__ dfeat_abs_sum,
     float dscale_inv, const float2* __restrict__ slot_xy, const int* __restrict__ seg_start,
-    float* __restrict__ grad_tables, int tex_begin, int tex_end, unsigned char* s_raw) {
+    float* __restrict__ grad_tables, int tex_begin, int tex_end, unsigned char* s_raw, unsigned pair_levels = 0) {
   int* s_g = reinterpret_cast<int*>(s_raw);
   NT_SPAN_MARK(HASHED ? 3 : 2, 0);
   NT_BAL_BEGIN();
   const bool full_range = tex_begin <= 0 && tex_end >= plan.nr_shells * 2 * VSA_NT_MAX_DEG;
-  auto unit_weight = [&](int pl, int deg, int) {
-    return !HASHED || plan.level_scale[level0 + (pl >> 1)] < (float)plan.tex_res[deg] ? 16 : 14;
+  const bool pair_mode = !HASHED && pair_levels != 0;
+  auto pairs_at = [&](int pl) {
+    int r;
+    return ((pair_levels >> enc_plane_level(plan, level0, pl, HASHED, r)) & 1u) != 0;
   };
-  nt_for_each_piece<ENC_UNIT>(plan, seg_start, n_planes, HASHED ? NT_ENC_OVH_BH : NT_ENC_OVH_BD,
+  auto unit_weight = [&](int pl, int deg, int wtype) {
+    if (!HASHED) return wtype == 2 ? (pairs_at(pl) ? NT_ENC_PAIR_WB : 32) : 16;
+    return plan.level_scale[level0 + (pl >> 1)] < (float)plan.tex_res[deg] ? 16 : 14;
+  };
+  auto piece_ovh = [&](int pl, int wtype) {
+    if (HASHED) return NT_ENC_OVH_BH;
+    return wtype == 2 ? (pairs_at(pl) ? NT_ENC_OVH_BDP : 2 * NT_ENC_OVH_BD) : NT_ENC_OVH_BD;
+  };
+  nt_for_each_piece<ENC_UNIT>(plan, seg_start, n_planes, piece_ovh,
                               [&](int pl, int tex, int first, int last, int seg_begin, int seg_end) {
-    int level = level0, r = pl;
-    bool both = enc_both_features(plan, level, HASHED);
-    while (r >= (both ? 1 : 2)) {
-      r -= both ? 1 : 2;
-      ++level;
-      both = enc_both_features(plan, level, HASHED);
-    }
-    const bool shared_plane = (((tex / VSA_NT_MAX_DEG) & 1) ? plan.shared_alpha : plan.shared_rgb) != 0;
+    int r;
+    const int level = enc_plane_level(plan, level0, pl, HASHED, r);
+    const bool both = enc_both_features(plan, level, HASHED);
+    const int partner = pair_mode ? nt_pair_partner(plan, tex) : -1;
+    if constexpr (!HASHED) {
+      if (partner >= 0 && ((pair_levels >> level) & 1u)) {
+        const bool store = plan.grads_zeroed != 0 && first == seg_begin && last == seg_end;
+        enc_bwd_piece<false, 2, true, true>(plan, s_g, level, 0, tex, partner, first, last, store, dfeatures,
+                                            dfeat_abs_sum, dscale_inv, slot_xy, grad_tables);
+        return;
+      }
+    }
+    for (int pass = 0; pass < (partner >= 0 ? 2 : 1); ++pass) {
+    const int tex_p = pass ? partner : tex;
+    const bool shared_plane = (((tex_p / VSA_NT_MAX_DEG) & 1) ? plan.shared_alpha : plan.shared_rgb) != 0;
     const bool store = plan.grads_zeroed != 0 && first == seg_begin && last == seg_end && !shared_plane;
-    const bool merge = plan.level_scale[level] < (float)plan.tex_res[tex % VSA_NT_MAX_DEG];
+    const bool merge = plan.level_scale[level] < (float)plan.tex_res[tex_p % VSA_NT_MAX_DEG];
     if (both)
-      enc_bwd_piece<HASHED, 2, true>(plan, s_g, level, 0, tex, first, last, store, dfeatures,
+      enc_bwd_piece<HASHED, 2, true>(plan, s_g, level, 0, tex_p, -1, first, last, store, dfeatures,
                                      dfeat_abs_sum, dscale_inv, slot_xy, grad_tables);
     else if (merge)
-      enc_bwd_piece<HASHED, 1, true>(plan, s_g, level, r, tex, first, last, store, dfeatures,
+      enc_bwd_piece<HASHED, 1, true>(plan, s_g, level, r, tex_p, -1, first, last, store, dfeatures,
                                      dfeat_abs_sum, dscale_inv, slot_xy, grad_tables);
     else
-      enc_bwd_piece<HASHED, 1, false>(plan, s_g, level, r, tex, first, last, store, dfeatures,
+      enc_bwd_piece<HASHED, 1, false>(plan, s_g, level, r, tex_p, -1, first, last, store, dfeatures,
                                       dfeat_abs_sum, dscale_inv, slot_xy, grad_tables);
+    }
   }, tex_begin, tex_end, unit_weight,
-     full_range ? (HASHED ? NT_BAL_ENC_BWD_H : NT_BAL_ENC_BWD_D) : -1);
+     full_range ? (HASHED ? NT_BAL_ENC_BWD_H : NT_BAL_ENC_BWD_D) : -1, pair_mode);
   __syncthreads();
   NT_SPAN_MARK(HASHED ? 3 : 2, 1);
   if (full_range) { NT_BAL_END(HASHED ? NT_BAL_ENC_BWD_H : NT_BAL_ENC_BWD_D); }
@@ -472,20 +532,20 @@
     vsa_nt_plan plan, int level0, int n_levels, int n_planes,
     const half2_t* __restrict__ dfeatures, const float* __restrict__ dfeat_abs_sum,
     float dscale_inv, const float2* __restrict__ slot_xy, const int* __restrict__ seg_start,
-    float* __restrict__ grad_tables, int tex_begin, int tex_end) {
+    float* __restrict__ grad_tables, int tex_begin, int tex_end, unsigned pair_levels) {
   extern __shared__ __attribute__((aligned(16))) unsigned char s_raw[];
   nt_encode_bwd_body<HASHED>(plan, level0, n_levels, n_planes, dfeatures, dfeat_abs_sum, dscale_inv, slot_xy,
-                             seg_start, grad_tables, tex_begin, tex_end, s_raw);
+                             seg_start, grad_tables, tex_begin, tex_end, s_raw, HASHED ? 0u : pair_levels);
 }
 
 __global__ __launch_bounds__(ENC_BLOCK) void nt_encode_bwd_both_kernel(
     vsa_nt_plan plan, int lh, int n_planes_dense,
     const half2_t* __restrict__ dfeatures, const float* __restrict__ dfeat_abs_sum,
     float dscale_inv, const float2* __restrict__ slot_xy, const int* __restrict__ seg_start,
-    float* __restrict__ grad_tables, int tex_begin, int tex_end) {
+    float* __restrict__ grad_tables, int tex_begin, int tex_end, unsigned pair_levels) {
   extern __shared__ __attribute__((aligned(16))) unsigned char s_raw[];
   nt_encode_bwd_body<false>(plan, 0, lh, n_planes_dense, dfeatures, dfeat_abs_sum, dscale_inv, slot_xy,
-                            seg_start, grad_tables, tex_begin, tex_end, s_raw);
+                            seg_start, grad_tables, tex_begin, tex_end, s_raw, pair_levels);
   __syncthreads();
   nt_encode_bwd_body<true>(plan, lh, plan.n_levels - lh, 2 * (plan.n_levels - lh), dfeatures, dfeat_abs_sum,
                            dscale_inv, slot_xy, seg_start, grad_tables, tex_begin, tex_end, s_raw);
@@ -502,11 +562,11 @@
     const half2_t* __restrict__ dfeatures, const float* __restrict__ dfeat_abs_sum,
     float dscale_inv, const float2* __restrict__ slot_xy, const int* __restrict__ seg_start,
     float* __restrict__ grad_tables, EncPhases ph,
-    unsigned* __restrict__ counters, const unsigned* __restrict__ epoch) {
+    unsigned* __restrict__ counters, const unsigned* __restrict__ epoch, unsigned pair_levels) {
   extern __shared__ __attribute__((aligned(16))) unsigned char s_raw[];
   if (lh > 0)
     nt_encode_bwd_body<false>(plan, 0, lh, n_planes_dense, dfeatures, dfeat_abs_sum, dscale_inv, slot_xy,
-                              seg_start, grad_tables, 0, 1 << 30, s_raw);
+                              seg_start, grad_tables, 0, 1 << 30, s_raw, pair_levels);
   __syncthreads();
   int shell0 = 0;
   for (int p = 0; p < ph.n; ++p) {
@@ -563,6 +623,22 @@
   for (int l = 0; l < lh; ++l)
     if (p->level_size[l] > LDS_ENTRIES) return VSA_ERR_UNSUPPORTED;
   return VSA_OK;
+}
+
+static unsigned enc_bwd_pair_levels(const vsa_nt_plan* p) {
+  const char* sw = getenv("VSA_NT_ENC_BWD_PAIR");
+  if (sw && sw[0] == '0') return 0;
+  if (p->nr_shells * 2 * VSA_NT_MAX_DEG > 64 || p->shared_rgb || p->shared_alpha) return 0;
+  unsigned mask = 0;
+  const int lh = first_hashed_level(p);
+  for (int l = 0; l < lh; ++l)
+    if (enc_both_features(*p, l, false) && enc_pair_level(*p, l)) mask |= 1u << l;
+  return mask;
+}
+
+extern "C" int vsa_nt_encode_bwd_pair_levels(const vsa_nt_plan* plan) {
+  if (!plan || check_levels(plan)) return 0;
+  return (int)enc_bwd_pair_levels(plan);
 }
 
 static int max_level_size(const vsa_nt_plan* p, int l0, int l1) {
@@ -661,7 +737,7 @@
     for (int l = 0; l < lh; ++l) n_planes += enc_both_features(*plan, l, false) ? 1 : 2;
     hipLaunchKernelGGL(nt_encode_bwd_both_kernel, dim3(nr_cus), dim3(ENC_BLOCK), (size_t)LDS_ENTRIES * 4,
                        (hipStream_t)stream, *plan, lh, n_planes, dF, dfeat_abs_sum, 1.0f / grad_scale, xy,
-                       seg_start, grad_tables, tex_begin, tex_end);
+                       seg_start, grad_tables, tex_begin, tex_end, enc_bwd_pair_levels(plan));
     VSA_RETURN_LAUNCH_STATUS();
   }
   if (lh > 0) {
@@ -670,13 +746,13 @@
     hipLaunchKernelGGL(nt_encode_bwd_kernel<false>, dim3(nr_cus), dim3(ENC_BLOCK),
                        (size_t)LDS_ENTRIES * 4, (hipStream_t)stream, *plan, 0, lh, n_planes, dF,
                        dfeat_abs_sum, 1.0f / grad_scale, xy, seg_start, grad_tables, tex_begin,
-                       tex_end);
+                       tex_end, enc_bwd_pair_levels(plan));
   }
   if (lh < plan->n_levels)
     hipLaunchKernelGGL(nt_encode_bwd_kernel<true>, dim3(nr_cus), dim3(ENC_BLOCK),
                        (size_t)LDS_ENTRIES * 4, (hipStream_t)stream, *plan, lh, plan->n_levels - lh,
                        2 * (plan->n_levels - lh), dF, dfeat_abs_sum, 1.0f / grad_scale, xy,
-                       seg_start, grad_tables, tex_begin, tex_end);
+                       seg_start, grad_tables, tex_begin, tex_end, 0u);
   VSA_RETURN_LAUNCH_STATUS();
 }
 
@@ -759,7 +835,7 @@
   hipLaunchKernelGGL(nt_encode_bwd_phased_kernel, dim3(nr_cus), dim3(ENC_BLOCK), (size_t)LDS_ENTRIES * 4,
                      (hipStream_t)stream, *plan, lh, n_planes, reinterpret_cast<const half2_t*>(dfeatures),
                      dfeat_abs_sum, 1.0f / grad_scale, reinterpret_cast<const float2*>(slot_xy), seg_start,
-                     grad_tables, ph, counters, epoch);
+                     grad_tables, ph, counters, epoch, enc_bwd_pair_levels(plan));
   VSA_RETURN_LAUNCH_STATUS();
 }
 
diff --git a/volsurfs_amd/neural_textures.py b/volsurfs_amd/neural_textures.py
--- a/volsurfs_amd/neural_textures.py
+++ b/volsurfs_amd/neural_textures.py
@@ -392,6 +392,9 @@
                       self._dfsum, float(grad_scale), self.slot_xy, self.seg_start,
                       self.tables.grad, int(shells[0]), int(shells[1]), _lib.stream_ptr())
 
+    def encode_bwd_pair_levels(self):
+        return int(_lib.lib().vsa_nt_encode_bwd_pair_levels(ctypes.byref(self.plan)))
+
     def backward_encode_phased(self, grad_scale, signals, grads_zeroed=None):
         self._take_grads_zeroed(grads_zeroed)
         _lib.call("vsa_nt_encode_bwd_phased", ctypes.byref(self.plan), self.features, self._dfsum,
diff --git a/volsurfs_amd/pipeline.py b/volsurfs_amd/pipeline.py
--- a/volsurfs_amd/pipeline.py
+++ b/volsurfs_amd/pipeline.py
@@ -300,16 +300,18 @@
                                                act_out=self._act),
             record, bytes=acct.get("nt_shade_fwd", 0))
         self.surfs_rgb, self.surfs_alpha = rgb_k, alpha_k
-        from .composite import composite_fwd_bwd_l1_raw
-        rgb, g_c, g_a = T.run("composite_fwd_bwd",
-                              lambda: composite_fwd_bwd_l1_raw(rgb_k, alpha_k, self.bg, gt,
-                                                               1.0 / (3.0 * self.loss_rays)),
-                              record, bytes=N * (12 + 12 + 32 * K))
+        from .composite import composite_fwd_bwd_l1_raw, composite_fwd_bwd_l1_rm_raw
         if self.image_hw is not None:
-            T.run("rgb_row_order", lambda: _lib.call("vsa_tile_order", rgb, self._rgb_out, self.image_hw[0],
-                                                     self.image_hw[1], 3, 1, _lib.stream_ptr()),
-                  record, bytes=N * 24)
-            rgb = self._rgb_out
+            rgb, g_c, g_a = T.run("composite_fwd_bwd",
+                                  lambda: composite_fwd_bwd_l1_rm_raw(rgb_k, alpha_k, self.bg, gt,
+                                                                      1.0 / (3.0 * self.loss_rays), self.image_hw,
+                                                                      out_rm=self._rgb_out),
+                                  record, bytes=N * (12 + 12 + 32 * K))
+        else:
+            rgb, g_c, g_a = T.run("composite_fwd_bwd",
+                                  lambda: composite_fwd_bwd_l1_raw(rgb_k, alpha_k, self.bg, gt,
+                                                                   1.0 / (3.0 * self.loss_rays)),
+                                  record, bytes=N * (12 + 12 + 32 * K))
         tris = self.tracer.tris
         T.run("nt_shade_bwd", lambda: bank.backward_shade(hit_slot, tex_uv, rays_d, tris, g_c, g_a,
                                                            self.grad_scale, self._act), record,
```
